# mindspore-lab/minddiffusion

Measured on AMD Instinct MI355X. Metric: 512x512 txt2img latents/sec (50-step DDIM), higher is better.
Workload: dtype f16; 1 GPU; SDv2 txt2img 512x512 (64x64 latent), 50-step DDIM, CFG 9.0, batch 1 per GPU (BASELINE.json configs[1]); synthetic seeded weights + synthetic text conditioning; global_batch=1, parallelism=batch-shard x1, hip_graph=True, rccl_world_size=1, broadcast_bytes=0, ddim_steps=50, unet_batch_per_gpu=2, sampler=ddim, cfg_dup_prefix=False

## Files before the change

### minddiffusion_amd/csrc/dense.hip

```cpp
#include "mdx_common.h"
#include "gemm_internal.h"

#include <algorithm>

namespace {

#ifndef MDX_LEAN_EPI
#define MDX_LEAN_EPI 1
#endif
constexpr bool LEAN_EPI = MDX_LEAN_EPI != 0;
constexpr int LNR_MAX = 24;
typedef unsigned u32x2 __attribute__((ext_vector_type(2)));

template <int BM, class Restage>
__device__ __forceinline__ void xattn_tile_epilogue(const GemmParams& p, char* smem, const char* xs, const int m0, const int n0,
                                                    const Restage& restage) {
    constexpr int SLD = 72;
    const int tid = threadIdx.x, lane = tid & 63;
    const int wave = __builtin_amdgcn_readfirstlane(tid >> 6);
    const int ntile = (p.xa_len + 63) >> 6;
    if (wave * 32 >= BM) {
        for (int t0 = 2; t0 < ntile; t0 += 2) {
            __syncthreads();
            restage(t0);
            asm volatile("s_waitcnt vmcnt(0)" ::: "memory");
            __syncthreads();
        }
        return;
    }
    const int hi = lane >> 5, l31 = lane & 31;
    f16* stg = reinterpret_cast<f16*>(smem);
    f16x8 qf[4];
#pragma unroll
    for (int s4 = 0; s4 < 4; ++s4) qf[s4] = *reinterpret_cast<const f16x8*>(&stg[(wave * 32 + l31) * SLD + 16 * s4 + 8 * hi]);
    f32x16 acc_o[2];
#pragma unroll
    for (int d = 0; d < 2; ++d)
#pragma unroll
        for (int r = 0; r < 16; ++r) acc_o[d][r] = 0.f;
    float m_run = -INFINITY, l_run = 0.f;
    const int vswz = (lane >> 1) & 7;
    const int krow_l = (l31 & 0x13) | ((l31 & 4) << 1) | ((l31 & 8) >> 1);
    auto tile = [&](const int t, auto mask_c) {
        constexpr bool MASK = decltype(mask_c)::value;
        const char* sk = xs + (t & 1) * 16384;
        const char* sv = sk + 8192;
        f32x16 acc_s[2];
#pragma unroll
        for (int kt = 0; kt < 2; ++kt) {
#pragma unroll
            for (int r = 0; r < 16; ++r) acc_s[kt][r] = 0.f;
            const int krow = kt * 32 + krow_l;
#pragma unroll
            for (int s4 = 0; s4 < 4; ++s4) {
                const f16x8 kf = *reinterpret_cast<const f16x8*>(sk + krow * 128 + (((2 * s4 + hi) ^ ((krow >> 1) & 7)) << 4));
                acc_s[kt] = __builtin_amdgcn_mfma_f32_32x32x16_f16(kf, qf[s4], acc_s[kt], 0, 0, 0);
            }
        }
        if constexpr (MASK) {
            const int key0 = t * 64, kmax = p.xa_len - 1;
#pragma unroll
            for (int kt = 0; kt < 2; ++kt)
#pragma unroll
                for (int r = 0; r < 16; ++r) {
                    const int key = key0 + kt * 32 + (r & 3) + 4 * ((r >> 2) & 1) + 8 * hi + 16 * (r >> 3);
                    if (key > kmax) acc_s[kt][r] = -INFINITY;
                }
        }
        float mx = acc_s[0][0];
#pragma unroll
        for (int kt = 0; kt < 2; ++kt)
#pragma unroll
            for (int r = 0; r < 16; ++r) mx = fmaxf(mx, acc_s[kt][r]);
        {
            const auto sw = __builtin_amdgcn_permlane32_swap(__float_as_uint(mx), __float_as_uint(mx), false, false);
            mx = fmaxf(__uint_as_float(sw[0]), __uint_as_float(sw[1]));
        }
        const float m_cand = fmaxf(m_run, mx);
        if (__builtin_amdgcn_ballot_w64((m_cand - m_run) * p.xa_scale_log2 > 8.0f)) {
            const float alpha = __builtin_amdgcn_exp2f((m_run - m_cand) * p.xa_scale_log2);
            l_run *= alpha;
#pragma unroll
            for (int d = 0; d < 2; ++d)
#pragma unroll
                for (int r = 0; r < 16; ++r) acc_o[d][r] *= alpha;
            m_run = m_cand;
        }
        const float mb = m_run * p.xa_scale_log2;
        typedef float f32x2 __attribute__((ext_vector_type(2)));
        const f32x2 sc2 = {p.xa_scale_log2, p.xa_scale_log2}, nmb2 = {-mb, -mb};
        f32x2 psum2 = {0.f, 0.f};
        f16x8 pf[4];
#pragma unroll
        for (int kt = 0; kt < 2; ++kt)
#pragma unroll
            for (int r = 0; r < 16; r += 2) {
                const f32x2 x2 = {acc_s[kt][r], acc_s[kt][r + 1]};
                const f32x2 a2 = __builtin_elementwise_fma(x2, sc2, nmb2);
                const f32x2 pv2 = {__builtin_amdgcn_exp2f(a2.x), __builtin_amdgcn_exp2f(a2.y)};
                psum2 += pv2;
                pf[kt * 2 + (r >> 3)][r & 7] = (f16)pv2.x;
                pf[kt * 2 + (r >> 3)][(r & 7) + 1] = (f16)pv2.y;
            }
        l_run += psum2.x + psum2.y;
#pragma unroll
        for (int c = 0; c < 4; ++c)
#pragma unroll
            for (int d = 0; d < 2; ++d) {
                const f16x8 vf = *reinterpret_cast<const f16x8*>(sv + (d * 32 + l31) * 128 + (((2 * c + hi) ^ vswz) << 4));
                acc_o[d] = __builtin_amdgcn_mfma_f32_32x32x16_f16(vf, pf[c], acc_o[d], 0, 0, 0);
            }
    };
    for (int t = 0; t < ntile; ++t) {
        if (t >= 2 && !(t & 1)) {
            __syncthreads();
            restage(t);
            asm volatile("s_waitcnt vmcnt(0)" ::: "memory");
            __syncthreads();
        }
        if ((t + 1) * 64 > p.xa_len) tile(t, std::true_type{}); else tile(t, std::false_type{});
    }
    const float l_tot = l_run + __shfl_xor(l_run, 32, 64);
    const float inv = 1.0f / l_tot;
    f16* og = stg + wave * 32 * SLD;
#pragma unroll
    for (int d = 0; d < 2; ++d)
#pragma unroll
        for (int g = 0; g < 4; ++g) {
            f16x4 v;
#pragma unroll
            for (int e = 0; e < 4; ++e) v[e] = (f16)(acc_o[d][4 * g + e] * inv);
            *reinterpret_cast<f16x4*>(&og[l31 * SLD + d * 32 + 8 * g + 4 * hi]) = v;
        }
    asm volatile("s_waitcnt lgkmcnt(0)" ::: "memory");
    for (int idx = lane; idx < 32 * 8; idx += 64) {
        const int row = idx >> 3, chunk = idx & 7;
        const int m = m0 + wave * 32 + row;
        if (m < p.M) {
            const f16x8 v = *reinterpret_cast<const f16x8*>(&og[row * SLD + chunk * 8]);
            *reinterpret_cast<f16x8*>(p.out + (size_t)m * p.out_ld + n0 + chunk * 8) = v;
        }
    }
}

template <int BM, int BN>
__device__ __forceinline__ void epilogue_w41(const GemmParams& p, f32x16 (&acc)[BN / 32], char* smem, const int m0, const int n0,
                                             const float bias_pre, const float lns_pre) {
    constexpr int NT = 256, TN = BN / 32, SLD = BN + 8;
    const int tid = threadIdx.x, lane = tid & 63;
    const int wave = __builtin_amdgcn_readfirstlane(tid >> 6);
    const int hi = lane >> 5, l31 = lane & 31;
    f16* stg = reinterpret_cast<f16*>(smem);
    float* lnrow = reinterpret_cast<float*>(smem + (size_t)BM * SLD * 2);
    float* lns = lnrow + 2 * BM;
    float* bs = lns + BN;
    if (tid < BN) bs[tid] = bias_pre;
    const int m_l = wave * 32 + l31;
    if (p.ln_stats) {
        for (int r = tid; r < BM; r += NT) {
            float mr[2];
            gemm_ln_row_fold(p, m0 + r, mr);
            lnrow[2 * r] = mr[0];
            lnrow[2 * r + 1] = mr[1];
        }
        if (tid < BN) lns[tid] = lns_pre;
        __syncthreads();
        const float mean = lnrow[2 * m_l], rstd = lnrow[2 * m_l + 1];
#pragma unroll
        for (int j = 0; j < TN; ++j)
#pragma unroll
            for (int r = 0; r < 16; ++r) {
                const int n_l = j * 32 + 8 * (r >> 2) + 4 * hi + (r & 3);
                acc[j][r] = rstd * (acc[j][r] - mean * lns[n_l]);
            }
    }
    const bool geglu = p.epilogue == MDX_EPI_GEGLU;
    constexpr int CH = BN / 8, PASSES = BM * CH / NT;
    static_assert(BM * CH % NT == 0 && BM * (CH / 2) % NT == 0, "store loops: whole passes");
    const __amdgpu_buffer_rsrc_t rs_res = make_rsrc(p.residual, (p.residual && !geglu) ? p.res_bytes : 0u);
    f16x8 lres[PASSES];
#pragma unroll
    for (int pass = 0; pass < PASSES; ++pass) {
        const int idx = tid + pass * NT;
        const int row = idx / CH, c = idx - row * CH;
        const int m = m0 + row, n = n0 + c * 8;
        const unsigned off = (m < p.M && n < p.N) ? ((unsigned)m * (unsigned)p.residual_ld + (unsigned)n) * 2u : MDX_OOB;
        lres[pass] = __builtin_bit_cast(f16x8, __builtin_amdgcn_raw_buffer_load_b128(rs_res, off, 0, 0));
    }
#pragma unroll
    for (int j = 0; j < TN; ++j)
#pragma unroll
        for (int g = 0; g < 4; ++g) {
            const int n_l = j * 32 + 8 * g + 4 * hi;
            *reinterpret_cast<f16x4*>(&stg[m_l * SLD + n_l]) =
                cvt4(acc[j][4 * g], acc[j][4 * g + 1], acc[j][4 * g + 2], acc[j][4 * g + 3]);
        }
    __syncthreads();
    trace_mark(p, 5);
    if (geglu) {
        constexpr int U = BN / 2, GCH = U / 8, GP = BM * GCH / NT;
        const bool has_res = p.residual != nullptr;
        f16x8 va[GP], vg[GP];
        f32x4 ba[GP][2], bg[GP][2];
#pragma unroll
        for (int pass = 0; pass < GP; ++pass) {
            const int idx = tid + pass * NT;
            const int row = idx / GCH, c = idx - row * GCH;
            va[pass] = *reinterpret_cast<const f16x8*>(&stg[row * SLD + c * 8]);
            vg[pass] = *reinterpret_cast<const f16x8*>(&stg[row * SLD + U + c * 8]);
            ba[pass][0] = *reinterpret_cast<const f32x4*>(&bs[c * 8]);
            ba[pass][1] = *reinterpret_cast<const f32x4*>(&bs[c * 8 + 4]);
            bg[pass][0] = *reinterpret_cast<const f32x4*>(&bs[U + c * 8]);
            bg[pass][1] = *reinterpret_cast<const f32x4*>(&bs[U + c * 8 + 4]);
        }
#pragma unroll
        for (int pass = 0; pass < GP; ++pass) {
            const int idx = tid + pass * NT;
            const int row = idx / GCH, c = idx - row * GCH;
            const int m = m0 + row;
            const int pn = n0 + c * 8;
            const int on = (n0 >> 1) + c * 8;
            if (m < p.M && pn < p.N) {
                float f[8];
#pragma unroll
                for (int e = 0; e < 8; ++e)
                    f[e] = ((float)va[pass][e] + ba[pass][e >> 2][e & 3]) * gelu_tanh_f((float)vg[pass][e] + bg[pass][e >> 2][e & 3]);
                if (has_res) {
                    const f16x8 rr = *reinterpret_cast<const f16x8*>(p.residual + (size_t)m * p.residual_ld + on);
#pragma unroll
                    for (int e = 0; e < 8; ++e) f[e] += (float)rr[e];
                }
                f16x8 o;
#pragma unroll
                for (int e = 0; e < 8; ++e) o[e] = (f16)f[e];
                *reinterpret_cast<f16x8*>(p.out + (size_t)m * p.out_ld + on) = o;
            }
        }
        return;
    }
    const bool has_res = p.residual != nullptr;
    f16x8 sv[PASSES];
    f32x4 bb[PASSES][2];
#pragma unroll
    for (int pass = 0; pass < PASSES; ++pass) {
        const int idx = tid + pass * NT;
        const int row = idx / CH, c = idx - row * CH;
        sv[pass] = *reinterpret_cast<const f16x8*>(&stg[row * SLD + c * 8]);
        bb[pass][0] = *reinterpret_cast<const f32x4*>(&bs[c * 8]);
        bb[pass][1] = *reinterpret_cast<const f32x4*>(&bs[c * 8 + 4]);
    }
#pragma unroll
    for (int pass = 0; pass < PASSES; ++pass) {
        const int idx = tid + pass * NT;
        const int row = idx / CH, c = idx - row * CH;
        const int m = m0 + row, n = n0 + c * 8;
        float f[8];
#pragma unroll
        for (int e = 0; e < 8; ++e) f[e] = (float)sv[pass][e] + bb[pass][e >> 2][e & 3];
        if (has_res) {
#pragma unroll
            for (int e = 0; e < 8; ++e) f[e] += (float)lres[pass][e];
        }
        f16x8 o;
#pragma unroll
        for (int e = 0; e < 8; ++e) o[e] = (f16)f[e];
        if (m < p.M && n < p.N) *reinterpret_cast<f16x8*>(p.out + (size_t)m * p.out_ld + n) = o;
    }
}

template <int BM, int BN, int NS, int PF, bool XA = false>
__global__ __launch_bounds__(256, 2) void dense_kernel(const GemmParams p) {
    mdx_kernarg_touch<sizeof(GemmParams)>();
    constexpr int NW = 4;
    constexpr bool W41 = BN % 64 != 0;
    static_assert(!W41 || (BM == 128 && BN % 32 == 0 && !XA && PF <= 1), "4 x 1 wave layout: 128-row tiles, prefetch level 0 / 1");
    constexpr int WROWS = W41 ? BM / 4 : BM / 2;
    constexpr int TM = WROWS / 32;
    constexpr int TN = W41 ? BN / 32 : BN / 64;
    constexpr int ROWB = 128;
    constexpr int KS = 4;
    constexpr int A_BYTES = BM * ROWB;
    constexpr int B_BYTES = BN * ROWB;
    constexpr int STAGE = A_BYTES + B_BYTES;
    constexpr int AJ = BM / 8 / NW;
    constexpr int BJ = BN / 8 / NW;
    constexpr int LPT = AJ + BJ;
    extern __shared__ __attribute__((aligned(16))) char smem[];

    const int tid = threadIdx.x;
    const int lane = tid & 63;
    const int wave = __builtin_amdgcn_readfirstlane(tid >> 6);
    const int wm = W41 ? wave : wave >> 1, wn = W41 ? 0 : wave & 1;
    const int hi = lane >> 5;
    const int l31 = lane & 31;

    const int ntiles = p.tiles_m * p.tiles_n;
    const int tile_id = p.spread ? (int)blockIdx.x : (int)((blockIdx.x & 7) * p.tiles_per_xcd + (blockIdx.x >> 3));
    if (tile_id >= ntiles) return;
    trace_mark(p, 0);
    int tile_m, tile_n;
    if (p.n_fastest) {
        tile_m = p.inv_tiles_n ? (int)__umulhi((unsigned)tile_id, p.inv_tiles_n) : tile_id;
        tile_n = tile_id - tile_m * p.tiles_n;
    } else {
        tile_n = p.inv_tiles_m ? (int)__umulhi((unsigned)tile_id, p.inv_tiles_m) : tile_id;
        tile_m = tile_id - tile_n * p.tiles_m;
    }
    const int m0 = tile_m * BM, n0 = tile_n * BN;
    const int split = (int)blockIdx.y;
    const int kt_begin = split * p.ktiles_per_split;
    const int kt_end = min(p.ktiles, kt_begin + p.ktiles_per_split);
    const int nt = kt_end - kt_begin;

    const __amdgpu_buffer_rsrc_t rs_a = make_rsrc(p.a, p.a_bytes);
    const __amdgpu_buffer_rsrc_t rs_w = make_rsrc(p.w, p.w_bytes);

    const int lrow = lane >> 3, lchk = lane & 7;
    const unsigned row_bytes = (unsigned)p.c1 * 2u;
    unsigned a_voff[AJ], b_off[BJ];
#pragma unroll
    for (int j = 0; j < AJ; ++j) {
        const int row = (wave * AJ + j) * 8 + lrow;
        const int m = m0 + row;
        a_voff[j] = m < p.M ? (unsigned)m * row_bytes + (unsigned)((lchk ^ ((row >> 1) & 7)) * 16) : MDX_OOB;
    }
#pragma unroll
    for (int j = 0; j < BJ; ++j) {
        const int row = (wave * BJ + j) * 8 + lrow;
        if constexpr (W41) {
            const int grow = n0 + row;
            b_off[j] = (unsigned)(grow >> 6) * (unsigned)p.kt64 * 8192u + (unsigned)(((grow & 63) * 8 + lchk) * 16);
        } else {
            const int panel = (n0 >> 6) + (row >> 6);
            b_off[j] = (unsigned)panel * (unsigned)p.kt64 * 8192u + (unsigned)(((row & 63) * 8 + lchk) * 16);
        }
    }
    auto stage_tile = [&](int kt, int buf) {
        char* sbase = smem + buf * STAGE;
#pragma unroll
        for (int j = 0; j < AJ; ++j) dma16s(rs_a, sbase + (wave * AJ + j) * 1024, a_voff[j], (unsigned)kt * 128u);
#pragma unroll
        for (int j = 0; j < BJ; ++j) dma16s(rs_w, sbase + A_BYTES + (wave * BJ + j) * 1024, b_off[j], (unsigned)kt * 8192u);
    };
#pragma unroll
    for (int i = 0; i < NS - 1; ++i)
        if (i < nt) stage_tile(kt_begin + i, i);
    __builtin_amdgcn_sched_barrier(0);
    trace_mark(p, 1);

    constexpr int CPR = BN / 8, RPP = 256 / CPR, PASSES = BM / RPP;
    constexpr int NX = (PF >= 2 && !W41) ? (PASSES < 4 ? PASSES : 4) : 0;
    constexpr int LNR = PF >= 3 ? LNR_MAX : 0;
    constexpr int NT = PF == 1 || PF == 2 ? 2 : 0;
    constexpr int NB = BN == 128 ? 4 : 2;
    constexpr int E = NB + NX + LNR + (PF >= 2 ? 1 : 0) + NT;
    const bool geglu = p.epilogue == MDX_EPI_GEGLU;
    const __amdgpu_buffer_rsrc_t rs_bias = make_rsrc(p.bias, p.bias ? (unsigned)p.N * 4u : 0u);
    const __amdgpu_buffer_rsrc_t rs_res = make_rsrc(p.residual, (p.residual && !geglu) ? p.res_bytes : 0u);
    const bool ln_regs = PF >= 3 && p.ln_stats != nullptr && p.ln_nt <= LNR;
    const bool lns_regs = PF >= 2 && p.ln_stats != nullptr;
    const __amdgpu_buffer_rsrc_t rs_ln = make_rsrc(p.ln_stats, p.ln_stats ? (unsigned)p.M * (unsigned)p.ln_nt * 8u : 0u);
    const __amdgpu_buffer_rsrc_t rs_lns = make_rsrc(p.ln_s, p.ln_stats ? (unsigned)p.N * 4u : 0u);
    u32x4 braw[4] = {};
    if constexpr (W41) {
        const unsigned off = (tid < BN && n0 + tid < p.N) ? (unsigned)(n0 + tid) * 4u : MDX_OOB;
        braw[0][0] = __builtin_amdgcn_raw_buffer_load_b32(rs_bias, off, 0, 0);
        braw[1][0] = __builtin_amdgcn_raw_buffer_load_b32(rs_lns, off, 0, 0);
    } else {
        const int n = n0 + (geglu ? (tid & 7) : (tid % CPR)) * 8;
        const unsigned off = n < p.N ? (unsigned)n * 4u : MDX_OOB;
        braw[0] = __builtin_amdgcn_raw_buffer_load_b128(rs_bias, off, 0, 0);
        braw[1] = __builtin_amdgcn_raw_buffer_load_b128(rs_bias, off, 16, 0);
        if constexpr (NB == 4) {
            const unsigned goff = geglu ? off : MDX_OOB;
            braw[2] = __builtin_amdgcn_raw_buffer_load_b128(rs_bias, goff, 256, 0);
            braw[3] = __builtin_amdgcn_raw_buffer_load_b128(rs_bias, goff, 272, 0);
        }
    }
    u32x4 xraw[NX > 0 ? NX : 1];
    if constexpr (NX > 0) {
        const int n = n0 + (tid % CPR) * 8;
#pragma unroll
        for (int q = 0; q < NX; ++q) {
            const int m = m0 + tid / CPR + q * RPP;
            const unsigned off = (m < p.M && n < p.N) ? ((unsigned)m * (unsigned)p.residual_ld + (unsigned)n) * 2u : MDX_OOB;
            xraw[q] = __builtin_amdgcn_raw_buffer_load_b128(rs_res, off, 0, 0);
        }
    }
    u32x2 lnraw[LNR > 0 ? LNR : 1];
    if constexpr (LNR > 0) {
        const unsigned base = (tid < BM && m0 + tid < p.M) ? (unsigned)(m0 + tid) * (unsigned)p.ln_nt * 8u : MDX_OOB;
#pragma unroll
        for (int j = 0; j < LNR; ++j)
            lnraw[j] = __builtin_amdgcn_raw_buffer_load_b64(rs_ln, (base != MDX_OOB && j < p.ln_nt) ? base : MDX_OOB, j * 8, 0);
    }
    unsigned lns_raw = 0u;
    if constexpr (PF >= 2)
        lns_raw = __builtin_amdgcn_raw_buffer_load_b32(rs_lns, (tid < BN && n0 + tid < p.N) ? (unsigned)(n0 + tid) * 4u : MDX_OOB, 0, 0);
    unsigned touch[2] = {0u, 0u};
    if constexpr (NT > 0) {
        const int rows = min(BM, p.M - m0);
        const unsigned bytes = (unsigned)rows * (unsigned)p.ln_nt * 8u;
        const unsigned base = (unsigned)m0 * (unsigned)p.ln_nt * 8u;
        touch[0] = __builtin_amdgcn_raw_buffer_load_b32(rs_ln, (unsigned)tid * 128u < bytes ? base + (unsigned)tid * 128u : MDX_OOB, 0, 0);
        touch[1] = __builtin_amdgcn_raw_buffer_load_b32(rs_lns, (PF < 2 && tid < BN / 32 && n0 + tid * 32 < p.N) ? (unsigned)(n0 + tid * 32) * 4u : MDX_OOB, 0, 0);
    }
    __builtin_amdgcn_sched_barrier(0);

    f32x16 acc[TM][TN];
#pragma unroll
    for (int i = 0; i < TM; ++i)
#pragma unroll
        for (int j = 0; j < TN; ++j)
#pragma unroll
            for (int r = 0; r < 16; ++r) acc[i][j][r] = 0.f;

    const int swz = (l31 >> 1) & 7;
    const int a_row_off = (wm * WROWS + l31) * ROWB;
    const int b_row_off = A_BYTES + (wn * (BN / 2) + l31) * ROWB;

    int rd = 0, wr = NS - 1;
    for (int t = 0; t < nt; ++t) {
        const int ahead = min(NS - 2, nt - 1 - t);
        if (t == 0) {
            if (NS >= 6 && ahead >= 4)
                asm volatile("s_waitcnt vmcnt(%0)" ::"n"(4 * LPT + E) : "memory");
            else if (NS >= 5 && ahead == 3)
                asm volatile("s_waitcnt vmcnt(%0)" ::"n"(3 * LPT + E) : "memory");
            else if (NS >= 4 && ahead == 2)
                asm volatile("s_waitcnt vmcnt(%0)" ::"n"(2 * LPT + E) : "memory");
            else if (NS >= 3 && ahead == 1)
                asm volatile("s_waitcnt vmcnt(%0)" ::"n"(LPT + E) : "memory");
            else
                asm volatile("s_waitcnt vmcnt(%0)" ::"n"(E) : "memory");
        } else if (NS >= 6 && ahead >= 4)
            asm volatile("s_waitcnt vmcnt(%0)" ::"n"(4 * LPT) : "memory");
        else if (NS >= 5 && ahead == 3)
            asm volatile("s_waitcnt vmcnt(%0)" ::"n"(3 * LPT) : "memory");
        else if (NS >= 4 && ahead == 2)
            asm volatile("s_waitcnt vmcnt(%0)" ::"n"(2 * LPT) : "memory");
        else if (NS >= 3 && ahead == 1)
            asm volatile("s_waitcnt vmcnt(%0)" ::"n"(LPT) : "memory");
        else
            asm volatile("s_waitcnt vmcnt(0)" ::: "memory");
        __builtin_amdgcn_s_barrier();
        if (t == 0) trace_mark(p, 2);
        const char* sb = smem + rd * STAGE;
        constexpr bool ALLK = TM * TN <= 2;
        constexpr int FD = ALLK ? KS : 2;
        f16x8 af[FD][TM], bf[FD][TN];
        auto rdfrag = [&](auto slot_c, const int ks) {
            constexpr int slot = decltype(slot_c)::value;
            const int coff = (((2 * ks + hi) ^ swz) << 4);
#pragma unroll
            for (int i = 0; i < TM; ++i) af[slot][i] = *reinterpret_cast<const f16x8*>(sb + a_row_off + i * 32 * ROWB + coff);
#pragma unroll
            for (int j = 0; j < TN; ++j) bf[slot][j] = *reinterpret_cast<const f16x8*>(sb + b_row_off + j * 32 * ROWB + coff);
        };
        auto mfmas = [&](auto slot_c) {
            constexpr int slot = decltype(slot_c)::value;
#pragma unroll
            for (int i = 0; i < TM; ++i)
#pragma unroll
                for (int j = 0; j < TN; ++j)
                    acc[i][j] = __builtin_amdgcn_mfma_f32_32x32x16_f16(bf[slot][j], af[slot][i], acc[i][j], 0, 0, 0);
        };
        using I0 = std::integral_constant<int, 0>;
        using I1 = std::integral_constant<int, 1>;
        if (t + NS - 1 < nt) stage_tile(kt_begin + t + NS - 1, wr);
        __builtin_amdgcn_sched_barrier(0);
        if constexpr (ALLK) {
            using I2 = std::integral_constant<int, 2>;
            using I3 = std::integral_constant<int, 3>;
            rdfrag(I0{}, 0); rdfrag(I1{}, 1); rdfrag(I2{}, 2); rdfrag(I3{}, 3);
            __builtin_amdgcn_sched_barrier(0);
            mfmas(I0{}); mfmas(I1{}); mfmas(I2{}); mfmas(I3{});
        } else {
            rdfrag(I0{}, 0);
            __builtin_amdgcn_sched_barrier(0);
#pragma unroll
            for (int ks = 0; ks < KS; ks += 2) {
                rdfrag(I1{}, ks + 1);
                __builtin_amdgcn_sched_barrier(0);
                mfmas(I0{});
                __builtin_amdgcn_sched_barrier(0);
                if (ks + 2 < KS) {
                    rdfrag(I0{}, ks + 2);
                    __builtin_amdgcn_sched_barrier(0);
                }
                mfmas(I1{});
                __builtin_amdgcn_sched_barrier(0);
            }
        }
        rd = (rd + 1 == NS) ? 0 : rd + 1;
        wr = (wr + 1 == NS) ? 0 : wr + 1;
    }

    __syncthreads();
    trace_mark(p, 3);
#pragma unroll
    for (int q = 0; q < NB; ++q) asm volatile("" ::"v"(braw[q]));
#pragma unroll
    for (int q = 0; q < NX; ++q) asm volatile("" ::"v"(xraw[q]));
#pragma unroll
    for (int j = 0; j < LNR; ++j) asm volatile("" ::"v"(lnraw[j]));
    if constexpr (PF >= 2) asm volatile("" ::"v"(lns_raw));
#pragma unroll
    for (int q = 0; q < NT; ++q) asm volatile("" ::"v"(touch[q]));
    float bpre[16];
#pragma unroll
    for (int q = 0; q < 4; ++q) {
        const f32x4 f = __builtin_bit_cast(f32x4, braw[q]);
        bpre[4 * q] = f[0]; bpre[4 * q + 1] = f[1]; bpre[4 * q + 2] = f[2]; bpre[4 * q + 3] = f[3];
    }
    Row8Extras xpre[NX > 0 ? NX : 1];
#pragma unroll
    for (int q = 0; q < NX; ++q) xpre[q].res = __builtin_bit_cast(f16x8, xraw[q]);
    float ln_pre[2];
    {
        float su = 0.f, sq = 0.f;
#pragma unroll
        for (int j = 0; j < LNR; ++j) {
            const float2 v = __builtin_bit_cast(float2, lnraw[j]);
            su += v.x;
            sq += v.y;
        }
        const float inv = 1.0f / (float)p.K;
        const float mean = su * inv;
        float var = sq * inv - mean * mean;
        var = var < 0.f ? 0.f : var;
        ln_pre[0] = mean;
        ln_pre[1] = rsqrtf(var + p.ln_eps);
    }
    const float lns_pre = __builtin_bit_cast(float, lns_raw);
    if constexpr (XA) {
        static_assert(BN == 64, "cross-attention epilogue: one 64-wide head per tile");
        constexpr int XOFF = ((BM * 72 * 2 + 2 * BM * 4 + BN * 4 + 1023) / 1024) * 1024;
        char* xs = smem + XOFF;
        const int bsamp = m0 / p.HoWo, head = n0 >> 6;
        const f16* kb = p.xa_k + (size_t)bsamp * p.xa_cap * p.N + head * 64;
        const f16* vb = p.xa_vt + ((size_t)bsamp * p.N + head * 64) * p.xa_cap;
        const __amdgpu_buffer_rsrc_t rs_k = make_rsrc(kb, (unsigned)(((size_t)(p.xa_len - 1) * p.N + 64) * 2));
        const __amdgpu_buffer_rsrc_t rs_v = make_rsrc(vb, (unsigned)((size_t)64 * p.xa_cap * 2));
        const int ntile = (p.xa_len + 63) >> 6;
        auto stage_pair = [&](const int t0) {
            const int t1 = t0 + 2 < ntile ? t0 + 2 : ntile;
            for (int t = t0; t < t1; ++t) {
                char* slot = xs + (t & 1) * 16384;
#pragma unroll
                for (int j = 0; j < 2; ++j) {
                    const int inst = wave * 2 + j;
                    const int krow = inst * 8 + (lane >> 3);
                    const int kchunk = (lane & 7) ^ ((krow >> 1) & 7);
                    const int key = t * 64 + krow;
                    dma16(rs_k, slot + inst * 1024, key < p.xa_len ? (unsigned)(((size_t)key * p.N + kchunk * 8) * 2) : MDX_OOB);
                    const int vrow = inst * 8 + (lane >> 3);
                    const unsigned vchunk = (unsigned)((lane & 7) ^ ((vrow >> 1) & 7));
                    const int kc = t * 64 + (int)vchunk * 8;
                    dma16(rs_v, slot + 8192 + inst * 1024, kc < p.xa_cap ? (unsigned)(((size_t)vrow * p.xa_cap + kc) * 2) : MDX_OOB);
                }
            }
        };
        stage_pair(0);
        gemm_epilogue<BM, BN, true, NW, LinearRows, NX, 3>(p, acc, smem, LinearRows{m0}, n0, split, bpre, tile_m, tile_id, ln_pre, &lns_pre, xpre,
                                                           ln_regs, lns_regs);
        asm volatile("s_waitcnt vmcnt(0)" ::: "memory");
        __syncthreads();
        xattn_tile_epilogue<BM>(p, smem, xs, m0, n0, stage_pair);
    } else if constexpr (W41) {
        epilogue_w41<BM, BN>(p, acc[0], smem, m0, n0, bpre[0], bpre[4]);
    } else {
        gemm_epilogue<BM, BN, true, NW, LinearRows, NX, LEAN_EPI ? 1 : 0>(p, acc, smem, LinearRows{m0}, n0, split, bpre, tile_m, tile_id, ln_pre,
                                                                  &lns_pre, xpre, ln_regs, lns_regs);
    }
    trace_mark(p, 4);
}

template <int BM, int BN, int NS, int PF>
void launch_dense_one(const GemmParams& p, dim3 grid, hipStream_t st) {
    constexpr size_t ring = (size_t)NS * (BM + BN) * 64 * 2;
    constexpr size_t epi = (size_t)(BM > BN ? BM : BN) * ((BM > BN ? BN : BM) + 8) * 2 + 4096;
    constexpr size_t lds = ring > epi ? ring : epi;
    static MdxPerDeviceOnce attr_once;
    if (attr_once.first())
        (void)hipFuncSetAttribute(reinterpret_cast<const void*>(&dense_kernel<BM, BN, NS, PF>),
                                  hipFuncAttributeMaxDynamicSharedMemorySize, (int)lds);
    hipLaunchKernelGGL((dense_kernel<BM, BN, NS, PF>), grid, dim3(256), lds, st, p);
}

template <int BM, int NS>
void launch_dense_xa(const GemmParams& p, dim3 grid, hipStream_t st) {
    constexpr size_t ring = (size_t)NS * (BM + 64) * 64 * 2;
    constexpr size_t xa = (size_t)((BM * 72 * 2 + 2 * BM * 4 + 64 * 4 + 1023) / 1024) * 1024 + 2 * 16384;
    constexpr size_t lds = ring > xa ? ring : xa;
    static MdxPerDeviceOnce attr_once;
    if (attr_once.first())
        (void)hipFuncSetAttribute(reinterpret_cast<const void*>(&dense_kernel<BM, 64, NS, 1, true>),
                                  hipFuncAttributeMaxDynamicSharedMemorySize, (int)lds);
    hipLaunchKernelGGL((dense_kernel<BM, 64, NS, 1, true>), grid, dim3(256), lds, st, p);
}

template <int BM, int BN, int NS>
void launch_dense_pf(const GemmParams& p, int pf, dim3 grid, hipStream_t st) {
    if constexpr (BM * BN < 128 * 128) {
        if (pf >= 3) return launch_dense_one<BM, BN, NS, 3>(p, grid, st);
        if (pf == 2) return launch_dense_one<BM, BN, NS, 2>(p, grid, st);
    }
    if (pf >= 1) return launch_dense_one<BM, BN, NS, 1>(p, grid, st);
    launch_dense_one<BM, BN, NS, 0>(p, grid, st);
}

template <int BM, int BN>
bool launch_dense_ns(const GemmParams& p, int ns, int pf, dim3 grid, hipStream_t st) {
    switch (ns) {
        case 2: launch_dense_pf<BM, BN, 2>(p, pf, grid, st); return true;
        case 3: launch_dense_pf<BM, BN, 3>(p, pf, grid, st); return true;
        case 4: if constexpr (BM == 64 || BN == 64) { launch_dense_pf<BM, BN, 4>(p, pf, grid, st); return true; } return false;
        case 5: if constexpr (BM == 64) { launch_dense_pf<BM, BN, 5>(p, pf, grid, st); return true; } return false;
        case 6: if constexpr (BM == 64) { launch_dense_pf<BM, BN, 6>(p, pf, grid, st); return true; } return false;
        default: return false;
    }
}

}

bool mdx_dense_takes_desc(const GemmParams& p, int bn) {
    if (!mdx_opt(MDX_OPT_GEMM_LEAN_DENSE) || !p.dense_issue) return false;
    if (!(p.ksize == 1 && p.stride == 1 && !p.upsample && p.c2 == 0 && p.cin % 64 == 0 && p.out_mode == MDX_OUT_ROWMAJOR)) return false;
    if (p.gn_cs || p.rowbias || p.out_bs || p.skip_w || p.d2s_c) return false;
    if (p.epilogue != MDX_EPI_NONE && p.epilogue != MDX_EPI_GEGLU) return false;
    if (p.xa_k && bn != 64) return false;
    if (bn == 160) {
        if (p.stats_out || p.colstats_out || p.n_split || p.xa_k) return false;
        if (p.epilogue == MDX_EPI_GEGLU && p.geglu_unit != 80) return false;
    }
    return true;
}

bool mdx_dense_takes(const GemmParams& p, int bm, int bn, int ring, int nsplit, bool fixup, bool nw8) {
    if (!mdx_dense_takes_desc(p, bn)) return false;
    if (!(nsplit == 1 || (fixup && bn != 160)) || nw8) return false;
    int built = (bm == 64 && (bn == 64 || bn == 128)) ? 6 : (bm == 128 && bn == 64) ? 4 : (bm == 128 && (bn == 128 || bn == 160)) ? 3 : 0;
    if (p.xa_k) built = std::min(built, 4);
    if (ring < 2 || ring > built) return false;
    if ((size_t)p.M * (size_t)(p.residual ? p.residual_ld : 0) * 2 >= 0x80000000ull) return false;
    if (p.ln_stats && (size_t)p.M * (size_t)p.ln_nt * 8 >= 0x80000000ull) return false;
    return (long)((p.M + bm - 1) / bm) * ((p.N + bn - 1) / bn) < 65536;
}

int mdx_dense_launch(const GemmParams& p, const GemmPlan& pl, hipStream_t st) {
    const int bm = pl.bm, bn = pl.bn, ns = pl.ring;
    const dim3 g = p.spread ? dim3((unsigned)(p.tiles_m * p.tiles_n), (unsigned)p.nsplit) : pl.grid;
    const int opt = mdx_opt(MDX_OPT_GEMM_LEAN_DENSE);
    const bool small = (long)g.x * g.y <= 512;
    const int pf = opt == 2 ? 0 : (opt == 3 && small ? 2 : (opt == 4 && small ? 3 : 1));
    bool ok = false;
    if (pl.form == GEMM_LEAN_XA) {
        ok = bn == 64 && ns >= 2 && ns <= 4 && (bm == 64 || bm == 128);
        if (ok && bm == 64) { if (ns == 2) launch_dense_xa<64, 2>(p, g, st); else if (ns == 3) launch_dense_xa<64, 3>(p, g, st); else launch_dense_xa<64, 4>(p, g, st); }
        if (ok && bm == 128) { if (ns == 2) launch_dense_xa<128, 2>(p, g, st); else if (ns == 3) launch_dense_xa<128, 3>(p, g, st); else launch_dense_xa<128, 4>(p, g, st); }
    }
    else if (bm == 64 && bn == 64) ok = launch_dense_ns<64, 64>(p, ns, pf, g, st);
    else if (bm == 64 && bn == 128) ok = launch_dense_ns<64, 128>(p, ns, pf, g, st);
    else if (bm == 128 && bn == 64) ok = launch_dense_ns<128, 64>(p, ns, pf, g, st);
    else if (bm == 128 && bn == 128) ok = launch_dense_ns<128, 128>(p, ns, pf, g, st);
    else if (bm == 128 && bn == 160) ok = launch_dense_ns<128, 160>(p, ns, pf, g, st);
    MDX_REQUIRE(ok, "mdx_gemm_f16: internal error: the plan names a lean dense tile %d x %d at ring depth %d that is not built", bm, bn, ns);
    return MDX_OK;
}
```

### minddiffusion_amd/csrc/gemm_tuned.inc

```
    {160, 320, 1024, 1, 64, 0, 8},
    {512, 1280, 2560, 1, 64, 0, 3},
    {512, 1280, 5120, 1, 128, 0, 6},
    {512, 1280, 5760, 3, 128, 0, 10},
    {2048, 640, 2560, 1, 128, 0, 3},
    {2048, 640, 2880, 3, 128, 0, 5},
    {2048, 640, 17280, 3, 128, 0, 6},
    {8192, 320, 72, 3, 64, 0, 1},
    {8192, 320, 320, 1, 64, 0, 1},
    {8192, 320, 640, 1, 64, 0, 1},
    {1024, 1280, 2560, 1, 128, 0, 3},
    {1024, 1280, 11520, 3, 128, 0, 6},
    {16384, 640, 320, 1, 64, 0, 1},
    {16384, 640, 960, 1, 64, 0, 1},
    {16384, 640, 1280, 1, 64, 0, 1},
    {16384, 640, 1920, 1, 64, 0, 1},
    {16384, 640, 2560, 1, 64, 0, 1},
    {640, 320, 1024, 1, 64, 0, 4},
    {1152, 1280, 5120, 1, 128, 0, 5},
    {1152, 3840, 1280, 1, 64, 0, 1},
    {4608, 1280, 1280, 1, 64, 0, 1},
    {4608, 3840, 1280, 1, 64, 0, 1},
    {18432, 640, 640, 1, 64, 0, 1},
    {73728, 8, 2880, 3, 128, 0, 2},
    {128, 1280, 1280, 1, 64, 64, 4},
// ... 56 lines not shown
    {16384, 640, 8640, 3, 128, 128, 1},
    {16384, 640, 11520, 3, 128, 128, 1},
    {65536, 960, 320, 1, 64, 128, 1},
    {640, 640, 1024, 1, 64, 64, 1},
    {640, 1280, 1024, 1, 64, 64, 1},
    {4608, 1280, 5760, 3, 64, 128, 1},
    {4608, 1280, 11520, 3, 64, 128, 1},
    {18432, 640, 320, 1, 64, 128, 1},
    {18432, 640, 960, 1, 64, 128, 1},
    {18432, 640, 2560, 1, 64, 128, 1},
    {18432, 640, 11520, 3, 128, 128, 1},
    {73728, 320, 72, 3, 64, 128, 1},
    {73728, 320, 8640, 3, 128, 128, 1},
    {128, 1280, 11520, 3, 128, 64, 20},
    {128, 1280, 23040, 3, 128, 64, 20},
    {160, 1280, 1024, 1, 64, 64, 1, 65},
    {8192, 320, 960, 1, 64, 64, 1, 2},
    {640, 320, 1024, 1, 64, 64, 1, 65},
    {18432, 640, 8640, 3, 128, 128, 2, 641},
    {18432, 640, 11520, 3, 128, 128, 2, 641},
    {1024, 768, 512, 1, 64, 64, 1, 1},
    {1024, 768, 512, 1, 64, 64, 1, 65},
    {1024, 768, 576, 1, 64, 64, 1, 1},
    {2048, 384, 512, 1, 64, 64, 1, 1},
    {2048, 384, 512, 1, 64, 64, 1, 65},
    {8192, 384, 384, 1, 64, 64, 1, 1},
    {8192, 384, 384, 1, 64, 64, 1, 65},
    {8192, 384, 384, 1, 64, 64, 1, 257},
    {8192, 384, 768, 1, 64, 64, 1, 2},
    {128, 1280, 11520, 3, 128, 64, 14, 257, 3},
    {512, 1280, 1920, 1, 64, 64, 3, 2, 3},
    {2048, 640, 320, 1, 64, 64, 1, 1, 3},
    {2048, 640, 640, 1, 64, 64, 1, 17, 3},
    {2048, 640, 640, 1, 64, 64, 1, 33, 3},
    {2048, 640, 640, 1, 64, 64, 1, 257, 3},
    {2048, 640, 640, 1, 64, 64, 1, 289, 3},
    {2048, 640, 640, 1, 64, 64, 1, 385, 3},
    {2048, 640, 960, 1, 64, 64, 1, 2, 3},
    {2048, 640, 1280, 1, 64, 64, 1, 2, 3},
    {2048, 640, 1920, 1, 64, 64, 1, 2, 3},
    {2048, 640, 2560, 1, 128, 64, 2, 257, 3},
    {2048, 640, 8640, 3, 128, 64, 3, 641, 3},
    {2048, 1920, 640, 1, 64, 128, 1, 25, 3},
    {8192, 8, 2880, 3, 128, 64, 5, 1, 3},
    {8192, 320, 320, 1, 64, 64, 1, 385, 3},
    {8192, 320, 1280, 1, 64, 128, 1, 257, 3},
    {8192, 320, 2880, 3, 128, 64, 1, 641, 3},
    {8192, 320, 8640, 3, 128, 64, 3, 641, 3},
    {1024, 1280, 1280, 1, 64, 64, 1, 33, 3},
    {1024, 1280, 1280, 1, 64, 64, 1, 257, 3},
    {1024, 1280, 1280, 1, 64, 64, 1, 289, 3},
    {1024, 1280, 2560, 1, 64, 128, 2, 2, 3},
    {1024, 1280, 11520, 3, 128, 64, 3, 257, 3},
    {1024, 1280, 11520, 3, 128, 64, 3, 513, 3},
    {16384, 640, 2880, 3, 128, 64, 1, 641, 3},
    {16384, 640, 5760, 3, 128, 64, 1, 385, 3},
    {16384, 640, 5760, 3, 128, 64, 1, 641, 3},
    {16384, 640, 8640, 3, 128, 64, 1, 641, 3},
    {16384, 640, 11520, 3, 128, 64, 1, 641, 3},
    {16384, 640, 17280, 3, 128, 64, 1, 641, 3},
    {16384, 1920, 640, 1, 64, 128, 1, 25, 2},
    {65536, 8, 2880, 3, 128, 64, 1, 1, 3},
    {65536, 320, 1280, 1, 128, 64, 1, 257, 2},
    {65536, 320, 2880, 3, 128, 64, 1, 641, 3},
    {1152, 1280, 1280, 1, 64, 64, 1, 257, 3},
    {1152, 1280, 2560, 1, 64, 128, 2, 2, 3},
    {4608, 1280, 17280, 3, 128, 128, 4, 513, 2},
    {18432, 640, 1920, 1, 64, 128, 1, 2, 2},
    {18432, 640, 5760, 3, 128, 64, 1, 385, 3},
    {18432, 640, 5760, 3, 128, 64, 1, 641, 3},
    {73728, 320, 2880, 3, 128, 64, 1, 257, 3},
    {73728, 320, 2880, 3, 128, 64, 1, 513, 3},
    {73728, 320, 5760, 3, 128, 64, 1, 513, 3},
    {512, 768, 1536, 1, 64, 64, 3, 2, 3},
    {512, 768, 6912, 3, 128, 64, 8, 1, 3},
    {512, 768, 6912, 3, 128, 64, 8, 257, 3},
    {512, 768, 13824, 3, 128, 64, 10, 1, 3},
    {1024, 768, 1536, 1, 64, 64, 3, 2, 3},
    {1024, 768, 5184, 3, 128, 64, 6, 1, 3},
    {1024, 768, 6912, 3, 128, 64, 5, 1, 3},
    {1024, 768, 6912, 3, 128, 64, 5, 257, 3},
    {1024, 768, 12096, 3, 128, 64, 6, 1, 3},
    {2048, 576, 512, 1, 64, 64, 1, 1, 3},
    {2048, 576, 512, 1, 64, 64, 1, 65, 3},
    {2048, 768, 384, 1, 64, 64, 1, 1, 3},
    {2048, 768, 512, 1, 64, 64, 1, 65, 3},
    {2048, 768, 768, 1, 64, 64, 1, 1, 3},
    {2048, 768, 768, 1, 64, 64, 1, 65, 3},
    {2048, 768, 768, 1, 64, 64, 1, 257, 3},
    {2048, 768, 3456, 3, 128, 64, 2, 1, 3},
    {2048, 768, 6912, 3, 128, 64, 2, 257, 3},
    {4096, 384, 3456, 3, 128, 64, 2, 257, 3},
    {4096, 576, 576, 1, 64, 64, 1, 257, 3},
    {4096, 576, 576, 1, 64, 64, 1, 385, 3},
    {4096, 576, 960, 1, 128, 64, 1, 2, 3},
    {4096, 576, 1152, 1, 128, 64, 1, 2, 3},
    {4096, 576, 1344, 1, 128, 64, 1, 2, 3},
    {8192, 384, 384, 1, 64, 64, 1, 385, 3},
    {8192, 384, 3456, 3, 128, 64, 1, 257, 3},
    {8192, 384, 6912, 3, 128, 64, 1, 1, 3},
    {16384, 384, 1728, 3, 128, 64, 1, 1, 3},
    {16384, 384, 3456, 3, 128, 64, 1, 1, 3},
    {16384, 384, 5184, 3, 128, 64, 1, 1, 3},
    {16384, 384, 8640, 3, 128, 64, 1, 1, 3},
    {16384, 576, 5184, 3, 128, 64, 1, 385, 3},
    {32768, 192, 1728, 3, 128, 64, 1, 385, 3},
    {32768, 384, 3456, 3, 128, 64, 1, 129, 3},
    {32768, 384, 3456, 3, 128, 64, 1, 385, 3},
    {32768, 384, 5184, 3, 128, 64, 1, 129, 3},
    {32768, 384, 6912, 3, 128, 64, 1, 129, 3},
    {65536, 8, 1728, 3, 128, 64, 1, 1, 3},
    {65536, 192, 1728, 3, 128, 64, 1, 129, 3},
    {65536, 192, 1728, 3, 128, 64, 1, 385, 3},
    {65536, 192, 3456, 3, 128, 64, 1, 129, 3},
    {65536, 192, 5184, 3, 128, 64, 1, 129, 3},
    {131072, 192, 1728, 3, 128, 64, 1, 257, 3},
    {131072, 192, 3456, 3, 128, 64, 1, 1, 3},
    {131072, 192, 5184, 3, 128, 64, 1, 1, 3},
    {524288, 192, 1728, 3, 128, 64, 1, 1, 3},
    {524288, 192, 1728, 3, 128, 64, 1, 257, 3},
    {524288, 192, 3456, 3, 128, 64, 1, 1, 3},
    {128, 1280, 11520, 3, 128, 64, 14, 513, 3},
    {512, 1280, 2560, 1, 64, 64, 3, 2, 3},
    {8192, 960, 320, 1, 128, 128, 1, 25, 2},
    {1024, 1280, 1280, 1, 64, 64, 1, 17, 3},
    {4096, 1280, 640, 1, 64, 128, 1, 1, 2},
    {4096, 1280, 1920, 1, 64, 128, 1, 2, 2},
    {4096, 1280, 2560, 1, 64, 128, 1, 2, 2},
    {16384, 640, 320, 1, 64, 128, 1, 1, 2},
    {16384, 640, 640, 1, 64, 128, 1, 289, 2},
    {65536, 320, 320, 1, 128, 64, 1, 17, 2},
    {65536, 320, 320, 1, 64, 64, 1, 33, 2},
    {65536, 320, 320, 1, 128, 64, 1, 289, 2},
    {65536, 320, 320, 1, 128, 64, 1, 385, 2},
    {65536, 320, 2880, 3, 128, 64, 1, 385, 3},
    {65536, 320, 5760, 3, 128, 64, 1, 641, 3},
    {65536, 960, 320, 1, 64, 128, 1, 25, 2},
    {1152, 3840, 1280, 1, 64, 128, 1, 25, 2},
    {4608, 1280, 1280, 1, 64, 128, 1, 33, 2},
    {4608, 1280, 1280, 1, 64, 128, 1, 385, 2},
    {4608, 1280, 2560, 1, 128, 128, 1, 2, 2},
    {4608, 1280, 5760, 3, 64, 128, 1, 513, 2},
    {4608, 1280, 11520, 3, 64, 128, 1, 257, 2},
    {4608, 1280, 11520, 3, 64, 128, 1, 513, 2},
    {18432, 640, 320, 1, 64, 128, 1, 1, 2},
    {18432, 640, 960, 1, 64, 128, 1, 2, 2},
    {18432, 640, 1280, 1, 64, 128, 1, 2, 2},
    {73728, 320, 320, 1, 128, 64, 1, 17, 2},
    {73728, 320, 320, 1, 128, 64, 1, 257, 2},
    {73728, 320, 320, 1, 128, 64, 1, 289, 2},
    {73728, 320, 640, 1, 128, 64, 1, 2, 2},
    {73728, 320, 1280, 1, 128, 64, 1, 257, 2},
    {73728, 960, 320, 1, 128, 64, 1, 25, 2},
    {1024, 768, 1344, 1, 64, 64, 3, 2, 3},
    {16384, 384, 192, 1, 64, 128, 1, 1, 2},
    {16384, 384, 384, 1, 64, 128, 1, 1, 2},
    {16384, 384, 384, 1, 128, 64, 1, 65, 2},
    {16384, 384, 384, 1, 64, 128, 1, 257, 2},
    {16384, 384, 384, 1, 128, 64, 1, 385, 2},
    {16384, 384, 576, 1, 64, 128, 1, 2, 2},
    {16384, 384, 768, 1, 64, 128, 1, 2, 2},
    {16384, 384, 960, 1, 64, 128, 1, 2, 2},
    {32768, 384, 576, 1, 64, 128, 1, 2, 2},
    {32768, 384, 1728, 3, 128, 64, 1, 129, 3},
    {65536, 192, 384, 1, 128, 64, 1, 2, 2},
    {131072, 192, 384, 1, 128, 64, 1, 2, 2},
    {524288, 192, 384, 1, 128, 64, 1, 2, 2},
    {128, 1280, 23040, 3, 128, 64, 10, 513, 3},
    {512, 1280, 11520, 3, 256, 64, 6, 513, 3},
    {512, 1280, 17280, 3, 256, 64, 6, 513, 3},
    {512, 1280, 23040, 3, 256, 64, 6, 513, 3},
    {8192, 320, 640, 1, 128, 128, 1, 2, 11},
    {4096, 1280, 5760, 3, 256, 128, 1, 513, 3},
    {4096, 1280, 11520, 3, 256, 128, 3, 257, 3},
    {4096, 1280, 11520, 3, 256, 128, 1, 513, 3},
    {4096, 1280, 17280, 3, 256, 128, 3, 513, 3},
    {4096, 1280, 23040, 3, 256, 128, 3, 513, 3},
    {16384, 640, 640, 1, 64, 128, 1, 17, 2},
    {65536, 320, 72, 3, 128, 128, 1, 129, 10},
    {65536, 320, 640, 1, 128, 128, 1, 2, 10},
    {65536, 320, 960, 1, 128, 128, 1, 2, 10},
    {65536, 320, 8640, 3, 256, 128, 1, 641, 2},
    {18432, 640, 640, 1, 128, 64, 1, 257, 2},
    {18432, 640, 640, 1, 128, 64, 1, 385, 2},
    {73728, 320, 72, 3, 128, 128, 1, 1, 10},
    {73728, 320, 320, 1, 64, 64, 1, 33, 2},
    {2048, 768, 512, 1, 64, 64, 1, 1, 3},
    {2048, 768, 1152, 1, 128, 64, 1, 2, 11},
    {2048, 768, 13824, 3, 256, 128, 5, 1, 3},
    {2048, 2048, 512, 1, 128, 128, 1, 5, 11},
    {4096, 384, 3456, 3, 128, 64, 2, 1, 3},
    {8192, 384, 1152, 1, 128, 128, 1, 2, 11},
    {8192, 768, 6912, 3, 256, 128, 1, 385, 3},
    {16384, 384, 6912, 3, 256, 128, 1, 1, 3},
    {32768, 384, 192, 1, 128, 128, 1, 1, 10},
    {32768, 384, 768, 1, 128, 128, 1, 2, 10},
    {65536, 192, 72, 3, 128, 128, 1, 129, 10},
    {65536, 192, 576, 1, 128, 64, 1, 2, 11},
    {65536, 384, 3456, 3, 256, 128, 1, 385, 3},
    {1024, 1280, 5120, 1, 128, 128, 3, 257, 11},
    {1024, 1280, 11520, 3, 128, 64, 3, 1, 3},
    {1280, 640, 768, 1, 64, 64, 1, 1, 4},
    {1280, 1280, 768, 1, 64, 64, 1, 1, 3},
    {4096, 1280, 1280, 1, 64, 128, 1, 33, 2},
    {4096, 10240, 1280, 1, 128, 128, 1, 19, 10},
    {16384, 640, 640, 1, 64, 128, 1, 33, 2},
    {640, 1280, 1024, 1, 64, 64, 1, 65, 4},
    {1152, 1280, 1280, 1, 64, 64, 1, 33, 3},
    {1152, 1280, 1280, 1, 64, 64, 1, 289, 3},
    {512, 1280, 11520, 3, 256, 64, 6, 1, 3},
    {512, 1280, 11520, 3, 256, 64, 5, 257, 3},
    {2048, 5120, 640, 1, 64, 128, 1, 19, 2},
    {160, 1280, 1024, 1, 64, 64, 3, 1, 4},
    {512, 1280, 1280, 1, 64, 64, 1, 257, 4},
    {512, 1280, 1280, 1, 64, 64, 1, 289, 4},
    {512, 10240, 1280, 1, 64, 128, 1, 19, 2},
    {1024, 3840, 1280, 1, 128, 128, 1, 25, 11},
    {1024, 10240, 1280, 1, 64, 128, 1, 19, 2},
    {1280, 1280, 768, 1, 64, 64, 1, 65, 3},
    {16384, 640, 2560, 1, 64, 128, 1, 257, 2},
    {640, 320, 1024, 1, 64, 64, 3, 1, 4},
    {640, 640, 1024, 1, 64, 64, 2, 1, 4},
    {1152, 1280, 1280, 1, 64, 64, 1, 17, 3},
    {1152, 1280, 11520, 3, 128, 128, 5, 257, 2},
    {4608, 1280, 1280, 1, 128, 128, 1, 289, 10},
    {4608, 1280, 5120, 1, 128, 128, 1, 257, 10},
    {18432, 640, 640, 1, 64, 128, 1, 289, 2},
    {18432, 640, 2560, 1, 128, 128, 1, 257, 10},
    {512, 768, 768, 1, 64, 64, 3, 1, 4},
    {512, 768, 768, 1, 64, 64, 1, 65, 3},
    {1024, 768, 768, 1, 64, 64, 1, 1, 3},
    {1024, 768, 768, 1, 64, 64, 1, 65, 3},
    {1024, 768, 13824, 3, 128, 128, 5, 1, 3},
    {1024, 2048, 512, 1, 128, 64, 1, 5, 11},
    {2048, 384, 3456, 3, 128, 64, 3, 1, 3},
    {2048, 384, 3456, 3, 128, 64, 5, 257, 3},
    {2048, 512, 512, 1, 64, 64, 1, 257, 4},
    {2048, 512, 2048, 1, 64, 64, 1, 257, 6},
    {4096, 576, 576, 1, 128, 64, 1, 1, 11},
    {4096, 576, 8640, 3, 256, 128, 3, 1, 3},
    {524288, 192, 72, 3, 128, 128, 1, 1, 10},
    {1024, 1280, 23040, 3, 128, 128, 3, 513, 4},
    {4096, 1280, 1280, 1, 128, 128, 1, 17, 2},
    {4096, 1280, 1280, 1, 128, 128, 1, 257, 2},
    {4096, 1280, 1280, 1, 128, 128, 1, 289, 2},
    {4096, 1280, 5120, 1, 128, 128, 3, 257, 2},
    {16384, 640, 640, 1, 128, 64, 1, 257, 2},
    {16384, 640, 640, 1, 64, 128, 1, 385, 2},
    {640, 1280, 1024, 1, 64, 64, 1, 1, 3},
    {4608, 1280, 640, 1, 128, 128, 1, 1, 2},
    {4608, 1280, 1280, 1, 128, 128, 1, 17, 2},
    {4608, 1280, 1280, 1, 128, 128, 1, 257, 2},
    {4608, 3840, 1280, 1, 128, 128, 1, 25, 2},
    {18432, 640, 640, 1, 128, 128, 1, 17, 2},
    {18432, 640, 640, 1, 128, 128, 1, 33, 2},
    {18432, 640, 2880, 3, 128, 128, 1, 641, 2},
    {18432, 1920, 640, 1, 128, 128, 1, 25, 2},
    {73728, 8, 2880, 3, 128, 64, 1, 1, 4},
    {512, 2304, 768, 1, 64, 64, 1, 9, 3},
    {1024, 512, 2048, 1, 64, 64, 2, 257, 6},
    {1024, 576, 5184, 3, 128, 64, 6, 1, 3},
    {1024, 576, 5184, 3, 128, 64, 6, 257, 3},
    {1024, 2304, 768, 1, 64, 64, 1, 9, 3},
    {2048, 768, 6912, 3, 128, 64, 2, 1, 4},
    {2048, 768, 10368, 3, 128, 64, 2, 1, 4},
    {2048, 2304, 768, 1, 64, 128, 1, 9, 2},
    {4096, 576, 3456, 3, 128, 64, 1, 1, 4},
    {4096, 576, 5184, 3, 128, 64, 1, 1, 4},
    {4096, 576, 5184, 3, 128, 64, 1, 257, 4},
    {4096, 576, 10368, 3, 256, 128, 3, 1, 3},
    {4096, 576, 12096, 3, 256, 128, 3, 1, 3},
    {4096, 768, 6912, 3, 128, 64, 1, 385, 4},
    {4096, 1728, 576, 1, 128, 128, 1, 9, 10},
    {8192, 384, 3456, 3, 128, 64, 1, 1, 4},
    {8192, 384, 10368, 3, 256, 128, 2, 1, 3},
    {8192, 1152, 384, 1, 64, 128, 1, 9, 2},
    {16384, 192, 1728, 3, 128, 64, 1, 1, 4},
    {16384, 192, 1728, 3, 128, 64, 1, 385, 4},
    {16384, 384, 3456, 3, 256, 128, 1, 257, 3},
    {16384, 1152, 384, 1, 64, 128, 1, 9, 2},
    {131072, 384, 3456, 3, 256, 128, 1, 385, 3},
    {524288, 8, 1728, 3, 128, 64, 1, 1, 4},
    {128, 1280, 1280, 1, 64, 64, 3, 257, 5},
    {128, 1280, 5120, 1, 64, 64, 4, 257, 5},
    {128, 1280, 11520, 3, 128, 64, 16, 1, 4},
    {128, 3840, 1280, 1, 64, 64, 2, 25, 5},
    {160, 320, 1024, 1, 64, 64, 3, 1, 5},
    {160, 640, 1024, 1, 64, 64, 3, 1, 4},
    {160, 640, 1024, 1, 64, 64, 1, 65, 4},
    {512, 1280, 1280, 1, 64, 64, 1, 17, 4},
    {512, 1280, 1280, 1, 64, 64, 1, 33, 5},
    {512, 1280, 5120, 1, 128, 64, 3, 257, 4},
    {512, 1280, 5760, 3, 128, 64, 4, 513, 4},
    {512, 3840, 1280, 1, 64, 128, 1, 25, 4},
    {2048, 640, 2880, 3, 128, 64, 3, 641, 4},
    {2048, 640, 5760, 3, 128, 64, 3, 129, 4},
    {2048, 640, 5760, 3, 128, 64, 3, 385, 4},
    {2048, 640, 5760, 3, 128, 64, 3, 641, 4},
    {2048, 640, 11520, 3, 128, 64, 3, 641, 4},
    {2048, 640, 17280, 3, 128, 64, 3, 641, 4},
    {8192, 320, 2880, 3, 128, 64, 1, 129, 4},
    {8192, 320, 2880, 3, 128, 64, 1, 385, 4},
    {8192, 320, 5760, 3, 128, 64, 1, 641, 4},
```

### minddiffusion_amd/ldm/modules/diffusionmodules/openaimodel.py

```python
import ctypes
import math
import os
import re
import weakref

import torch

from .... import ops
from ...._lib import MdxError
from ....planner import PlanBuilder, round_up, capture_or_eager
from ....loader import WeightLoader, named_layers

f16, f32 = torch.float16, torch.float32

LORA_PREFIXES = ("tk_delta_", "mindpet_delta_")
_LORA_KEY = re.compile(r"^(.*)\.(" + "|".join(LORA_PREFIXES) + r")lora_([ab])$")
_LORA_TARGETS = ("to_q", "to_k", "to_v", "to_out.0")


def is_lora_key(name):
    return _LORA_KEY.match(name) is not None


class UNetModel:
# ... 6 lines not shown
                 max_context_len=80, device="cuda:0"):
        if use_spatial_transformer:
            assert context_dim is not None, "context_dim is required with use_spatial_transformer"
        if context_dim is not None:
            assert use_spatial_transformer, "context_dim requires use_spatial_transformer"
        if num_heads == -1:
            assert num_head_channels != -1, "Either num_heads or num_head_channels has to be set"
        if num_head_channels == -1:
            assert num_heads != -1, "Either num_heads or num_head_channels has to be set"
        if not use_spatial_transformer:
            raise NotImplementedError("AttentionBlock is an empty stub in the reference (openaimodel.py:208-242)")
        if dims != 2:
            raise NotImplementedError("dims != 2: the image UNet is the only instantiation on the denoising path")
        self.conv_resample = bool(conv_resample)
        self.num_classes = num_classes
        self.use_scale_shift_norm = bool(use_scale_shift_norm)
        self.resblock_updown = bool(resblock_updown)
        self.transformer_depth = int(transformer_depth)
        self.n_embed = n_embed
        assert self.transformer_depth >= 1
        self.image_size = image_size
        self.in_channels = in_channels
        self.model_channels = model_channels
        self.out_channels = out_channels
        self.num_res_blocks = num_res_blocks
        self.attention_resolutions = list(attention_resolutions)
        self.channel_mult = list(channel_mult)
        self.num_heads = num_heads
        self.num_head_channels = num_head_channels
        self.context_dim = int(context_dim)
        self.legacy = legacy
        self.use_linear = use_linear_in_transformer
        self.use_fp16 = use_fp16
        self.device = torch.device(device)
        self.time_embed_dim = model_channels * 4
        self.input_blocks, self.middle_block, self.output_blocks = self._structure()
        self.cin_pad = round_up(in_channels, 8)
        self.final_channels = out_channels if n_embed is None else int(n_embed)
        self.cout_pad = round_up(self.final_channels, 8)
        self.w = None
        self._plans = {}
        self._ctx_key = None
        self._ctx_ref = None
        self.use_graph = True
        self.max_context_len = self._check_context_cap(max_context_len)
        self.last_launch_count = 0
        self.enable_lora = bool(enable_lora)
        self.lora_rank = int(lora_rank)
        self.lora_alpha = float(lora_alpha)
        if self.enable_lora and not (1 <= self.lora_rank <= 64 and self.lora_alpha != 0):
            raise ValueError(f"UNetModel: lora_rank must be in [1, 64] and lora_alpha non-zero (got {lora_rank}, {lora_alpha})")
        self._lora_base = {}
        self._lora_sites = {}
        self._lora = None
        self._lora_mult = 1.0

    @staticmethod
    def _check_context_cap(n):
        n = int(n)
        if not 1 <= n <= 1024:
            raise MdxError(f"UNetModel: max_context_len must be in [1, 1024] (got {n})")
        return round_up(n, 8)

    def set_max_context_len(self, n):
        n = self._check_context_cap(n)
        if n != self.max_context_len:
            self.max_context_len = n
            self._plans = {}
            self._ctx_key = None
            self._ctx_ref = None
        return self

    def _heads(self, ch, num_heads):
        if self.num_head_channels == -1:
            dim_head = ch // num_heads
        else:
            num_heads = ch // self.num_head_channels
            dim_head = self.num_head_channels
        if self.legacy:
            dim_head = ch // num_heads
        return num_heads, dim_head

    def _structure(self):
        mc = self.model_channels
        nh = self.num_heads
        inb = [[("conv", self.in_channels, mc)]]
        chans = [mc]
        ch, ds = mc, 1
        for level, mult in enumerate(self.channel_mult):
            for _ in range(self.num_res_blocks):
                layers = [("res", ch, mult * mc)]
                ch = mult * mc
                if ds in self.attention_resolutions:
                    nh, dh = self._heads(ch, nh)
                    layers.append(("st", ch, nh, dh))
                inb.append(layers)
                chans.append(ch)
            if level != len(self.channel_mult) - 1:
                inb.append([("resdown", ch, ch) if self.resblock_updown else ("down", ch)])
                chans.append(ch)
                ds *= 2
        nh, dh = self._heads(ch, nh)
        mid = [("res", ch, ch), ("st", ch, nh, dh), ("res", ch, ch)]
        outb = []
        for level, mult in list(enumerate(self.channel_mult))[::-1]:
            for i in range(self.num_res_blocks + 1):
                ich = chans.pop()
                layers = [("res", ch + ich, mc * mult)]
                ch = mc * mult
                if ds in self.attention_resolutions:
                    nh, dh = self._heads(ch, nh)
                    layers.append(("st", ch, nh, dh))
                if level and i == self.num_res_blocks:
                    layers.append(("resup", ch, ch) if self.resblock_updown else ("up", ch))
                    ds //= 2
                outb.append(layers)
        return inb, mid, outb

    def parameter_shapes(self):
        mc, ted, ctx = self.model_channels, self.time_embed_dim, self.context_dim
        s = {"time_embed.0.weight": (ted, mc), "time_embed.0.bias": (ted,),
             "time_embed.2.weight": (ted, ted), "time_embed.2.bias": (ted,)}
        if self.num_classes is not None:
            s["label_emb.embedding_table"] = (self.num_classes, ted)
        ssn = 2 if self.use_scale_shift_norm else 1
        for pre, layer in named_layers(self):
            kind = layer[0]
            if kind == "conv":
                s[pre + "conv.weight"] = (layer[2], layer[1], 3, 3)
                s[pre + "conv.bias"] = (layer[2],)
            elif kind in ("res", "resdown", "resup"):
                cin, cout = layer[1], layer[2]
                s[pre + "in_layers_norm.gamma"] = (cin,)
                s[pre + "in_layers_norm.beta"] = (cin,)
                s[pre + "in_layers_conv.conv.weight"] = (cout, cin, 3, 3)
                s[pre + "in_layers_conv.conv.bias"] = (cout,)
                s[pre + "emb_layers.1.weight"] = (ssn * cout, ted)
                s[pre + "emb_layers.1.bias"] = (ssn * cout,)
                s[pre + "out_layers_norm.gamma"] = (cout,)
                s[pre + "out_layers_norm.beta"] = (cout,)
                s[pre + "out_layers_conv.conv.weight"] = (cout, cout, 3, 3)
                s[pre + "out_layers_conv.conv.bias"] = (cout,)
                if cin != cout:
                    s[pre + "skip_connection.conv.weight"] = (cout, cin, 1, 1)
                    s[pre + "skip_connection.conv.bias"] = (cout,)
            elif kind == "st":
                ch, inner = layer[1], layer[2] * layer[3]
                s[pre + "norm.gamma"] = (ch,)
                s[pre + "norm.beta"] = (ch,)
                s[pre + "proj_in.weight"] = (inner, ch) if self.use_linear else (inner, ch, 1, 1)
                s[pre + "proj_in.bias"] = (inner,)
                s[pre + "proj_out.weight"] = (ch, inner) if self.use_linear else (ch, inner, 1, 1)
                s[pre + "proj_out.bias"] = (ch,)
                for k in range(self.transformer_depth):
                    t = pre + f"transformer_blocks.{k}."
                    for a, cd in (("attn1.", inner), ("attn2.", ctx)):
                        s[t + a + "to_q.weight"] = (inner, inner)
                        s[t + a + "to_k.weight"] = (inner, cd)
                        s[t + a + "to_v.weight"] = (inner, cd)
                        s[t + a + "to_out.0.weight"] = (inner, inner)
                        s[t + a + "to_out.0.bias"] = (inner,)
                    s[t + "ff.net.0.proj.weight"] = (inner * 8, inner)
                    s[t + "ff.net.0.proj.bias"] = (inner * 8,)
                    s[t + "ff.net.2.weight"] = (inner, inner * 4)
                    s[t + "ff.net.2.bias"] = (inner,)
                    for n in ("norm1", "norm2", "norm3"):
                        s[t + n + ".gamma"] = (inner,)
                        s[t + n + ".beta"] = (inner,)
            elif kind == "down" and self.conv_resample:
                s[pre + "op.conv.weight"] = (layer[1], layer[1], 3, 3)
                s[pre + "op.conv.bias"] = (layer[1],)
            elif kind == "up" and self.conv_resample:
                s[pre + "conv.conv.weight"] = (layer[1], layer[1], 3, 3)
                s[pre + "conv.conv.bias"] = (layer[1],)
        s["out.0.gamma"] = (mc,)
        s["out.0.beta"] = (mc,)
        s["out.2.conv.weight"] = (self.out_channels, mc, 3, 3)
        s["out.2.conv.bias"] = (self.out_channels,)
        if self.n_embed is not None:
            s["id_predictor.0.gamma"] = (mc,)
            s["id_predictor.0.beta"] = (mc,)
            s["id_predictor.1.conv.weight"] = (self.n_embed, mc, 1, 1)
            s["id_predictor.1.conv.bias"] = (self.n_embed,)
        return s

    def _lora_targets(self):
        for pre, layer in named_layers(self):
            if layer[0] != "st":
                continue
            inner = layer[2] * layer[3]
            for k in range(self.transformer_depth):
                t = pre + f"transformer_blocks.{k}."
                for a, cd in (("attn1.", inner), ("attn2.", self.context_dim)):
                    for n in _LORA_TARGETS:
                        yield t + a + n, inner, (inner if n in ("to_q", "to_out.0") else cd)

    def lora_parameter_shapes(self, prefix=LORA_PREFIXES[0]):
        if prefix not in LORA_PREFIXES:
            raise ValueError(f"lora_parameter_shapes: prefix must be one of {LORA_PREFIXES}")
        s = {}
        for name, nout, nin in self._lora_targets():
            s[f"{name}.{prefix}lora_a"] = (self.lora_rank, nin)
            s[f"{name}.{prefix}lora_b"] = (nout, self.lora_rank)
        return s

    def load_state_dict(self, params, strict=True):
        shapes = self.parameter_shapes()
        who = "UNetModel.load_state_dict"
        lora_params = {}
        if self.enable_lora:
            lora_params = {k: v for k, v in params.items() if is_lora_key(k)}
            params = {k: v for k, v in params.items() if k not in lora_params}
        L = WeightLoader(params, self.device, who)
        L.check(shapes, unexpected=strict)
        if lora_params:
            lora_params = self._check_lora(lora_params, strict, who)
        ln_fold = os.environ.get("MDX_UNET_LN_FOLD", "1") != "0"
        qkv_merge = os.environ.get("MDX_UNET_QKV_MERGE", "1") != "0"
        w = L.w
        w["te0.w"], w["te0.b"] = L.raw("time_embed.0.weight", f16), L.vec("time_embed.0.bias")
        w["te2.w"], w["te2.b"] = L.raw("time_embed.2.weight", f16), L.vec("time_embed.2.bias")
        if self.num_classes is not None:
            w["label_emb"] = L.raw("label_emb.embedding_table", f32)
        emb_w, emb_b, self._emb_off = [], [], {}
        off = 0
        for pre, layer in named_layers(self):
            kind = layer[0]
            if kind == "conv":
                w[pre + "w"], w[pre + "b"] = L.conv(pre + "conv.weight", cin_pad=self.cin_pad), L.vec(pre + "conv.bias")
            elif kind in ("res", "resdown", "resup"):
                cin, cout = layer[1], layer[2]
                for n in ("in_layers_norm", "out_layers_norm"):
                    L.norm(pre + n, pre + n)
                w[pre + "conv1.w"], w[pre + "conv1.b"] = L.conv(pre + "in_layers_conv.conv.weight"), L.vec(pre + "in_layers_conv.conv.bias")
                w[pre + "conv2.w"], w[pre + "conv2.b"] = L.conv(pre + "out_layers_conv.conv.weight"), L.vec(pre + "out_layers_conv.conv.bias")
                if cin != cout:
                    w[pre + "skip.w"], w[pre + "skip.b"] = L.conv(pre + "skip_connection.conv.weight"), L.vec(pre + "skip_connection.conv.bias")
                emb_w.append(L.raw(pre + "emb_layers.1.weight", f16))
                emb_b.append(L.vec(pre + "emb_layers.1.bias"))
                self._emb_off[pre] = off
                off += cout * (2 if self.use_scale_shift_norm else 1)
            elif kind == "st":
                inner = layer[2] * layer[3]
                L.norm(pre + "norm", pre + "norm")
                proj = {}
                for n in ("proj_in", "proj_out"):
                    wt = L.raw(pre + n + ".weight", f16)
                    proj[n] = wt.reshape(wt.shape[0], wt.shape[1])
                    w[pre + n + ".w"], w[pre + n + ".b"] = L.dense(proj[n]), L.vec(pre + n + ".bias")
                for k in range(self.transformer_depth):
                    t = pre + f"transformer_blocks.{k}."
                    wq, wk, wv = (L.raw(t + f"attn1.to_{n}.weight", f16) for n in "qkv")
                    for n in ("norm1", "norm2", "norm3"):
                        L.norm(t + n, t + n)
                    fold = inner % 64 == 0 and ln_fold

                    def put(name, wt, norm, bias=None):
                        if fold:
                            wt, w[name + ".s"], w[name + ".cb"] = ops.fold_layernorm(wt, w[t + norm + ".g"], w[t + norm + ".b"], bias)
                        w[name + ".w"] = L.dense(wt)
                    if (2 * wq.shape[0]) % 128 == 0 and qkv_merge:
                        put(t + "attn1.qkv", torch.cat([wq, wk, wv], 0), "norm1")
                    else:
                        w[t + "attn1.qk.w"] = L.dense(torch.cat([wq, wk], 0))
                        w[t + "attn1.v.w"] = L.dense(wv)
                    wq2 = L.raw(t + "attn2.to_q.weight", f16)
                    put(t + "attn2.q", wq2, "norm2")
                    w[t + "attn2.k.w"] = L.dense(t + "attn2.to_k.weight")
                    w[t + "attn2.v.w"] = L.dense(t + "attn2.to_v.weight")
                    wo = {a: L.raw(t + a + ".to_out.0.weight", f16) for a in ("attn1", "attn2")}
                    for a in ("attn1", "attn2"):
                        w[t + a + ".o.w"], w[t + a + ".o.b"] = L.dense(wo[a]), L.vec(t + a + ".to_out.0.bias")
                    gw, gb = L.raw(t + "ff.net.0.proj.weight", f16), L.vec(t + "ff.net.0.proj.bias")
                    half = 4 * inner
                    w[t + "ff1.b"] = ops.geglu_interleave(gb[:half], gb[half:], 64)
                    put(t + "ff1", ops.geglu_interleave(gw[:half], gw[half:], 64), "norm3", w[t + "ff1.b"])
                    w2 = L.raw(t + "ff.net.2.weight", f16)
                    w[t + "ff2.w"], w[t + "ff2.b"] = L.dense(w2), L.vec(t + "ff.net.2.bias")
                    if (self.transformer_depth == 1 and inner == layer[1]
                            and ops.st_tail_supported(inner, layer[2], layer[3], 64, 64)):
                        w[t + "tail.stream"], w[t + "tail.vec"] = ops.pack_st_tail(
                            wo["attn1"], wq2, wo["attn2"], gw, w2, proj["proj_out"],
                            w[t + "attn1.o.b"], w[t + "norm2.g"], w[t + "norm2.b"], w[t + "attn2.o.b"], w[t + "norm3.g"],
                            w[t + "norm3.b"], gb, w[t + "ff2.b"], w[pre + "proj_out.b"])
                        if ops.st_head_supported(inner, 64, 64):
                            w[t + "head.stream"], w[t + "head.vec"] = ops.pack_st_head(
                                proj["proj_in"], wq, wk, wv, w[pre + "norm.g"], w[pre + "norm.b"],
                                w[pre + "proj_in.b"], w[t + "norm1.g"], w[t + "norm1.b"])
            elif kind == "down" and self.conv_resample:
                w[pre + "w"], w[pre + "b"] = L.conv(pre + "op.conv.weight"), L.vec(pre + "op.conv.bias")
            elif kind == "up" and self.conv_resample:
                w[pre + "w"], w[pre + "b"] = L.conv(pre + "conv.conv.weight"), L.vec(pre + "conv.conv.bias")
                if layer[1] % 64 == 0 and ops.get_option("unet_subpixel_upsample"):
                    w[pre + "wsub"] = ops.pack_subpixel_conv_weight(L.raw(pre + "conv.conv.weight", f32))
        w["emb.w"] = torch.cat(emb_w, 0).contiguous()
        w["emb.b"] = torch.cat(emb_b, 0).contiguous()
        self._emb_total = off
        norm, conv = ("out.0", "out.2.conv") if self.n_embed is None else ("id_predictor.0", "id_predictor.1.conv")
        w["out.g"], w["out.b"] = L.vec(norm + ".gamma"), L.vec(norm + ".beta")
        w["out.w"] = L.conv(conv + ".weight", cout_pad=self.cout_pad)
        w["out.cb"] = L.vec(conv + ".bias", pad=self.cout_pad)
        self._frag_w = {}
        self._geglu80 = {}
        self._plans = {}
        self._ctx_key = None
        self._ctx_ref = None
        self._lora = None
        self._lora_base, self._lora_sites = {}, {}
        if self.enable_lora:
            for name, _, _ in self._lora_targets():
                self._lora_base[name] = L.own(name + ".weight", f32)
        self.w = L.finish(shapes, unused=() if self.n_embed is None else [k for k in shapes if k.startswith("out.")])
        if self.enable_lora:
            self._lora_sites = self._find_lora_sites()
            if lora_params:
                self._set_lora(lora_params)
        return self

    def weight_bytes(self):
        n = sum(t.numel() * t.element_size() for t in self.w.values())
        n += sum(t.numel() * t.element_size() for t in self._lora_base.values())
        if self._lora:
            n += sum(a.numel() * 4 + b.numel() * 4 for a, b in self._lora.values())
        return n

    def _find_lora_sites(self):
        w = self.w
        T, F = ops.LORA_TILED, ops.LORA_FRAG
        sites = {}
        for pre, layer in named_layers(self):
            if layer[0] != "st":
                continue
            inner = layer[2] * layer[3]
            ks = inner // 16
            for k in range(self.transformer_depth):
                t = pre + f"transformer_blocks.{k}."

                def tiled(key, n0=0, dst_n=inner, norm=None):
                    kw = dict(dst=w[key + ".w"], layout=T, dst_n0=n0, dst_N=dst_n)
                    if norm is not None and (key + ".s") in w:
                        kw.update(gamma=w[t + norm + ".g"], beta=w[t + norm + ".b"], S=w[key + ".s"][n0:], cb=w[key + ".cb"][n0:])
                    return kw

                def frag(key, slot, per_wave):
                    return dict(dst=w[t + key], layout=F, dst_N=inner, piece_stride=per_wave * ks, piece_offset=slot * ks)
                merged = (t + "attn1.qkv.w") in w
                for i, n in enumerate("qkv"):
                    if merged:
                        here = [tiled(t + "attn1.qkv", i * inner, 3 * inner, "norm1")]
                    elif n == "v":
                        here = [tiled(t + "attn1.v")]
                    else:
                        here = [tiled(t + "attn1.qk", i * inner, 2 * inner)]
                    if (t + "head.stream") in w:
                        here.append(frag("head.stream", 1 + i, 4))
                    sites[t + f"attn1.to_{n}"] = here
                sites[t + "attn2.to_q"] = [tiled(t + "attn2.q", norm="norm2")]
                sites[t + "attn2.to_k"] = [tiled(t + "attn2.k")]
                sites[t + "attn2.to_v"] = [tiled(t + "attn2.v")]
                sites[t + "attn1.to_out.0"] = [tiled(t + "attn1.o")]
                sites[t + "attn2.to_out.0"] = [tiled(t + "attn2.o")]
                if (t + "tail.stream") in w:
                    for slot, name in enumerate(("attn1.to_out.0", "attn2.to_q", "attn2.to_out.0")):
                        sites[t + name].append(frag("tail.stream", slot, 16))
        assert set(sites) == set(self._lora_base)
        return sites

    def _check_lora(self, params, strict, who):
        found = {m.group(2) for m in map(_LORA_KEY.match, params) if m}
        if len(found) > 1:
            raise KeyError(f"{who}: adapter keys mix the prefixes {sorted(found)}")
        prefix = found.pop() if found else LORA_PREFIXES[0]
        shapes = self.lora_parameter_shapes(prefix)
        WeightLoader(params, self.device, who).check(shapes, unexpected=strict)
        return {k.replace("." + prefix, "." + LORA_PREFIXES[0]): params[k] for k in shapes}

    def _set_lora(self, checked):
        p, L = LORA_PREFIXES[0], WeightLoader(checked, self.device, "UNetModel.load_lora_state_dict")
        self._lora = {name: (L.own(f"{name}.{p}lora_a", f32), L.own(f"{name}.{p}lora_b", f32)) for name in self._lora_base}
        self._merge_lora()

    def _merge_lora(self):
        scale = self._lora_mult * self.lora_alpha / self.lora_rank
        for name, base in self._lora_base.items():
            a, b = self._lora[name] if self._lora else (None, None)
            for site in self._lora_sites[name]:
                ops.lora_merge(base, A=a, B=b, scale=scale, **site)
        self._ctx_key = None
        self._ctx_ref = None

    def _need_lora(self, who):
        if not self.enable_lora:
            raise MdxError(f"UNetModel.{who}: the model was built without enable_lora=True")
        if self.w is None:
            raise MdxError(f"UNetModel.{who}: load_state_dict() must be called first (the adapter is merged into the base weights)")

    def load_lora_state_dict(self, params, strict=True):
        self._need_lora("load_lora_state_dict")
        self._set_lora(self._check_lora(dict(params), strict, "UNetModel.load_lora_state_dict"))
        return self

    def set_lora_scale(self, m=1.0):
        self._need_lora("set_lora_scale")
        m = float(m)
        if not math.isfinite(m):
            raise ValueError("set_lora_scale: the multiplier must be finite")
        self._lora_mult = m
        if self._lora:
            self._merge_lora()
        return self

    def unload_lora(self):
        self._need_lora("unload_lora")
        if self._lora:
            self._lora = None
            self._merge_lora()
        return self

    @property
    def lora_loaded(self):
        return self._lora is not None

    class _Plan:
        pass

    def _plan(self, B, H, W, _selfctx=False):
        key = (B, H, W, "selfctx") if _selfctx else (B, H, W)
        if key in self._plans:
            return self._plans[key]
        if self.w is None:
            raise MdxError("UNetModel: load_state_dict() must be called before the first forward")
        for lvl in range(len(self.channel_mult) - 1):
            if (H >> lvl) % 2 or (W >> lvl) % 2:
                raise MdxError(f"UNetModel: latent {H}x{W} is not divisible by 2^{len(self.channel_mult) - 1}")
        try:
            P = _UNetPlanner(self, B, H, W, True, _selfctx).build()
        except _HeadNotWired:
            P = _UNetPlanner(self, B, H, W, False, _selfctx).build()
        self._plans[key] = P
        return P

    def _ensure_context(self, P, context):
        key = (context.data_ptr(), context._version, tuple(context.shape), context.dtype, id(P))
        alive = self._ctx_ref() if self._ctx_ref is not None else None
        if key == self._ctx_key and alive is context:
            return
        Bc, T, Dc = context.shape
        if Bc != P.B or Dc != self.context_dim:
            raise MdxError(f"context shape {tuple(context.shape)} does not match batch {P.B} / context_dim {self.context_dim}")
        if T > self.max_context_len:
            raise MdxError(f"context length {T} > max_context_len={self.max_context_len}")
        P.ctx_pad.zero_()
        P.ctx_pad[:, :T].copy_(context)
        P.ctx_len = T
        for d in getattr(P, "xattn_descs", ()):
            d.xattn_len = T
        for op in P.ctxops:
            op()
        self._ctx_key = key
        self._ctx_ref = weakref.ref(context)
        if getattr(P, "graph_ctx_len", None) != T:
            P.graph = None
            P.dup_graph = None

    def time_embedding_table(self, t):
        if self.w is None:
            raise MdxError("UNetModel: load_state_dict() must be called before time_embedding_table()")
        if self.num_classes is not None:
            raise MdxError("UNetModel: a class-conditional UNet adds label_emb(y) before the ResBlock projections; "
                           "there is no timestep-only table")
        t = torch.as_tensor(t, dtype=f32).to(self.device).reshape(-1).contiguous()
        w = self.w
        e0 = ops.timestep_embedding(t, self.model_channels)
        e1 = ops.dense_small(e0, w["te0.w"], w["te0.b"], act_out=True)
        e2 = ops.dense_small(e1, w["te2.w"], w["te2.b"])
        return ops.dense_small(e2, w["emb.w"], w["emb.b"], act_in=True)

    def forward_nhwc(self, x, timesteps, context=None, temb=None, y=None, cfg_dup=False):
        if (y is not None) != (self.num_classes is not None):
            raise MdxError("UNetModel: must specify y if and only if the model is class-conditional")
        if y is not None and temb is not None:
            raise MdxError("UNetModel: time_embedding_table() rows do not carry the label embedding; pass timesteps with y")
        if not (isinstance(x, torch.Tensor) and x.is_cuda):
            raise MdxError("UNetModel: x must be a CUDA(HIP) tensor (no CPU fallback)")
        B, C, H, W = x.shape
        if C != self.in_channels:
            raise MdxError(f"UNetModel: expected {self.in_channels} input channels, got {C}")
        if context is None:
            if getattr(self, "_selfctx_bad", None) is None:
                self._selfctx_bad = sorted({l[2] * l[3] for _, l in named_layers(self)
                                            if l[0] == "st" and l[2] * l[3] != self.context_dim})
            bad = self._selfctx_bad
            if bad:
                raise MdxError(f"UNetModel: context=None makes attn2 attend to its own input (attention.py:133), which needs "
                               f"context_dim == transformer width; context_dim={self.context_dim}, widths {bad}")
            P = self._plan(B, H, W, _selfctx=True)
        else:
            P = self._plan(B, H, W)
            self._ensure_context(P, context)
        P.x_static.copy_(x)
        if temb is not None:
            if temb.shape[-1] != self._emb_total or temb.dtype != f32:
                raise MdxError(f"UNetModel: temb must be fp32 [.., {self._emb_total}] rows of time_embedding_table()")
            P.emb_all.copy_(temb)
        else:
            P.t_static.copy_(timesteps.to(device=self.device, dtype=f32) if isinstance(timesteps, torch.Tensor)
                             else torch.as_tensor(timesteps, dtype=f32, device=self.device))
            if y is not None:
                yy = torch.as_tensor(y).to(device=self.device, dtype=torch.long).reshape(-1)
                if yy.shape[0] != B:
                    raise MdxError(f"UNetModel: y has {yy.shape[0]} labels for a batch of {B}")
                if int(yy.min()) < 0 or int(yy.max()) >= self.num_classes:
                    raise MdxError(f"UNetModel: class label outside [0, {self.num_classes})")
                P.y_static.copy_(yy)
            for op in P.main[:P.temb_ops]:
                op()
        dup = self._dup_body(P) if (cfg_dup and context is not None and y is None) else None
        if dup is not None and ops.get_option("unet_cfg_dup_check"):
            hb = B // 2
            same = torch.equal(P.x_static[:hb], P.x_static[hb:]) and torch.equal(P.emb_all[:hb], P.emb_all[hb:])
            if not same:
                raise MdxError("UNetModel: cfg_dup=True, but the two halves of the batch do not carry the same x / timesteps")
        if self.use_graph and not P.graph_failed:
            if dup is not None:
                if P.dup_graph is None:
                    self._capture(P, dup)
                if P.dup_graph is not None:
                    P.dup_graph.replay()
                    return P.eps_nhwc
            if P.graph is None:
                self._capture(P)
            if P.graph is not None:
                P.graph.replay()
                return P.eps_nhwc
        body = dup if dup is not None else P.main[P.temb_ops:]
        for op in body:
            op()
        self.last_launch_count = P.temb_ops + len(body)
        return P.eps_nhwc

    def _dup_body(self, P):
        mn = ops.get_option("unet_cfg_dup")
        if not mn or P.B < mn or P.B % 2 or P.ck is None:
            return None
        if hasattr(P, "dup_body"):
            return P.dup_body
        P.dup_body = None
        h = P.B // 2
        PA = self._plan(h, P.H, P.W)
        if PA.ck is None:
            return None
        late = "op2" in P.ck and "op2" in PA.ck and len(P.ck["live2"]) == len(PA.ck["live2"])
        ko, kl = ("op2", "live2") if late else ("op", "live")
        ib, ic = P.main.index(P.ck[ko]), P.main.index(P.ck["conv_in"])
        ja, jc = PA.main.index(PA.ck[ko]), PA.main.index(PA.ck["conv_in"])
        xin_a, xin_b = PA.ck["xin"], P.ck["xin"]
        copies = [lambda: xin_a.copy_(xin_b[:h]), lambda: PA.emb_all.copy_(P.emb_all[:h])]
        spread = []
        for src, dst in zip(PA.ck[kl], P.ck[kl]):
            if not (dst.shape[0] == 2 * src.shape[0] and dst.shape[1:] == src.shape[1:] and dst.dtype == src.dtype):
                raise MdxError(f"UNetModel: guidance-duplicate prefix: live tensors of the two plans do not pair up "
                               f"({tuple(src.shape)} vs {tuple(dst.shape)})")
            spread.append(lambda src=src, dst=dst, k=src.shape[0]: (dst[:k].copy_(src), dst[k:].copy_(src)))
        P.dup_half = PA
        P.dup_body = P.main[P.temb_ops:ic + 1] + copies + PA.main[jc:ja + 1] + spread + P.main[ib + 1:]
        small = {"kind": "small", "flops": 0, "launches": 1, "info": "guidance-duplicate prefix: copy"}
        P.dup_meta = (P.meta[P.temb_ops:ic + 1] + [dict(small) for _ in copies] + PA.meta[jc:ja + 1]
                      + [dict(small, launches=2) for _ in spread] + P.meta[ib + 1:])
        return P.dup_body

    def _capture(self, P, dup=None):
        body = dup if dup is not None else P.main[P.temb_ops:]
        graphs = capture_or_eager([body])
        if graphs is None:
            P.graph, P.graph_failed = None, True
        elif dup is not None:
            P.dup_graph = graphs[0]
        else:
            P.graph = graphs[0]
        if graphs is not None:
            P.graph_ctx_len = P.ctx_len

    def construct(self, x, timesteps=None, context=None, y=None):
        eps = self.forward_nhwc(x, timesteps, context, y=y)
        B, _, H, W = x.shape
        return ops.nhwc_to_nchw(eps, self.final_channels, H, W)

    __call__ = construct
    forward = construct


class _HeadNotWired(Exception):
    """A fused SpatialTransformer head / GroupNorm-in-conv launch did not get its column statistics (UNetModel._plan)."""


class _UNetPlanner(PlanBuilder):

    def __init__(self, net, B, H, W, fuse_head, selfctx):
        super().__init__(net.device, B, track_producers=True)
        self.net, self.w, self.H, self.W = net, net.w, H, W
        self.fuse_head, self.selfctx = fuse_head, selfctx
        self.TC = net.max_context_len
        self.ctx_flops = 77 if self.TC == 80 else self.TC
        self.mod_ld = net._emb_total
        self.P = UNetModel._Plan()
        self.ctxops = []
        self.ck = {}
        self.hs = []
        self.ctx_kv = {}
        self.xattn_descs, self.ln_stats, self.tails, self.heads_fused, self.ragged_vt = [], {}, [], [], []

    def build(self):
        P, net, B = self.P, self.net, self.B
        dev = self.dev
        P.B, P.H, P.W = B, self.H, self.W
        P.x_static = torch.zeros((B, net.in_channels, self.H, self.W), dtype=f32, device=dev)
        P.t_static = torch.zeros((B,), dtype=f32, device=dev)
        self.time_embedding()
        xin = self.get((B, self.H * self.W, net.cin_pad))
        self.emit(lambda: ops.nchw_to_nhwc(P.x_static, net.cin_pad, out=xin), "small")
        self.ck["xin"] = xin
        P.ctx_pad = torch.zeros((B, self.TC, net.context_dim), dtype=f16, device=dev)
        P.ctx_len = 0
        self.walk(xin)
        for t, (kc, vtc) in self.ctx_kv.items():
            inner = kc.shape[2]
            self.dense(P.ctx_pad, B, self.TC, net.context_dim, inner, self.w[t + "attn2.k.w"], out=kc, out_ld=inner,
                       oplist=self.ctxops)
            self.dense(P.ctx_pad, B, self.TC, net.context_dim, inner, self.w[t + "attn2.v.w"], out=vtc, out_ld=self.TC,
                       out_mode=ops.OUT_TRANSPOSED, oplist=self.ctxops)
        self.finish(P)
        P.ctxops, P.attn_ws, P.colstats = self.ctxops, self.attn_ws, self.colstats
        P.arena_bytes = self.A.total
        P.ln_stats = self.ln_stats
        P.tails = self.tails
        P.ragged_vt = self.ragged_vt
        P.heads_fused = self.heads_fused
        P.ctx_kv = self.ctx_kv
        P.xattn_descs = self.xattn_descs
        P.ck = self.ck if (self.ck.get("op") is not None and not self.selfctx) else None
        P.graph = None
        P.dup_graph = None
        P.graph_failed = False
        return P

    def time_embedding(self):
        P, net, w, B, dev = self.P, self.net, self.w, self.B, self.dev
        mc, ted = net.model_channels, net.time_embed_dim
        t_emb = torch.empty((B, mc), dtype=f32, device=dev)
        e1 = torch.empty((B, ted), dtype=f32, device=dev)
        emb = torch.empty((B, ted), dtype=f32, device=dev)
        P.emb_all = torch.empty((B, net._emb_total), dtype=f32, device=dev)
        self.emit(lambda: ops.timestep_embedding(P.t_static, mc, out=t_emb), "small")
        self.emit(lambda: ops.dense_small(t_emb, w["te0.w"], w["te0.b"], act_out=True, out=e1), "small", 2 * B * mc * ted)
        self.emit(lambda: ops.dense_small(e1, w["te2.w"], w["te2.b"], out=emb), "small", 2 * B * ted * ted)
        if net.num_classes is not None:
            P.y_static = torch.zeros((B,), dtype=torch.long, device=dev)
            self.emit(lambda: emb.add_(w["label_emb"].index_select(0, P.y_static)), "small")
        self.emit(lambda: ops.dense_small(emb, w["emb.w"], w["emb.b"], act_in=True, out=P.emb_all), "small",
                  2 * B * ted * net._emb_total)
        P.temb_ops = len(self.main)

    def held(self, t):
        return any(t is s_[0] for s_ in self.hs)

    def walk(self, xin):
        net, w, B = self.net, self.w, self.B
        h, wd = self.H, self.W
        cur = None
        for i, blk in enumerate(net.input_blocks):
            for j, layer in enumerate(blk):
                pre = f"input_blocks.{i}.{j}."
                if layer[0] == "conv":
                    cur, h, wd = self.conv3(xin, net.cin_pad, layer[2], w[pre + "w"], w[pre + "b"], h, wd)
                    self.ck["conv_in"] = self.main[-1]
                    self.release(xin)
                    continue
                new, h2, w2 = self.layer_op(pre, layer, cur, None, h, wd)
                if not self.held(cur):
                    self.release(cur)
                cur, h, wd = new, h2, w2
            self.hs.append((cur, h, wd))
        self.ck.setdefault("op", None)
        for j, layer in enumerate(net.middle_block):
            new, h, wd = self.layer_op(f"middle_block.{j}.", layer, cur, None, h, wd)
            if not self.held(cur):
                self.release(cur)
            cur = new
        for i, blk in enumerate(net.output_blocks):
            skip, sh, sw = self.hs.pop()
            assert (sh, sw) == (h, wd)
            for j, layer in enumerate(blk):
                new, h, wd = self.layer_op(f"output_blocks.{i}.{j}.", layer, cur, skip if j == 0 else None, h, wd)
                self.release(cur)
                if j == 0:
                    self.release(skip)
                cur = new
        mc = net.model_channels
        a = self.get((B, h * wd, mc))
        self.gn(cur, None, w["out.g"], w["out.b"], 1e-5, net.n_embed is None, a)
        self.P.eps_nhwc = torch.empty((B, h * wd, net.cout_pad), dtype=f16, device=self.dev)
        self.gemm(a=a, w=w["out.w"], N=net.cout_pad, B=B, H=h, W=wd, c1=mc, out=self.P.eps_nhwc, out_ld=net.cout_pad,
                  bias=w["out.cb"], ksize=3 if net.n_embed is None else 1)

    def layer_op(self, pre, layer, cur, skip, h, wd):
        net, w, B = self.net, self.w, self.B
        kind = layer[0]
        if kind == "res":
            return self.resblock(pre, cur, skip, layer[1], layer[2], h, wd)
        if kind in ("resdown", "resup"):
            return self.resblock(pre, cur, None, layer[1], layer[2], h, wd, mode=kind[3:])
        if kind == "st":
            return self.transformer(pre, cur, layer[1], layer[2], layer[3], h, wd), h, wd
        if kind == "down":
            if net.conv_resample:
                return self.conv3(cur, layer[1], layer[1], w[pre + "w"], w[pre + "b"], h, wd, stride=2)
            new = self.get((B, (h // 2) * (wd // 2), layer[1]))
            self.emit(lambda cur=cur, new=new: ops.avgpool2x2(cur, B, h, wd, layer[1], out=new), "small")
            return new, h // 2, wd // 2
        if kind == "up":
            if net.conv_resample:
                return self.conv3(cur, layer[1], layer[1], w[pre + "w"], w[pre + "b"], h, wd, upsample=1, wsub=w.get(pre + "wsub"))
            new = self.get((B, 4 * h * wd, layer[1]))
            self.emit(lambda cur=cur, new=new: ops.upsample_nearest2x(cur, B, h, wd, layer[1], out=new), "small")
            return new, 2 * h, 2 * wd
        raise ValueError(kind)

    def gn_conv_ok(self, src, c_in, c_out, hh, ww, wt):
        B = self.B
        mrows = ops.get_option("unet_gn_conv_fuse")
        if not self.fuse_head or not mrows or B * hh * ww < mrows or c_in % 64 or c_in > 640 or (hh == 8 and ww == 8):
            return False
        if self.producer.get(src.data_ptr()) is None:
            return False
        probe = ops.make_gemm_desc(a=src, w=wt, N=c_out, B=B, H=hh, W=ww, c1=c_in, out=src, out_ld=c_out, ksize=3)
        q = ops.gemm_query(probe)
        return q[3] == 1 and q[1] == 64

    def conv2(self, pre, src, x, x2, xs, cin, cout, c2, ho, wo, fusable, gn=None):
        w, B = self.w, self.B
        if cin != cout and fusable and self.skip_fusable(src, cin - c2, c2, cout, ho, wo, w[pre + "conv2.w"]):
            if (pre + "conv2skip.b") not in w:
                w[pre + "conv2skip.b"] = (w[pre + "conv2.b"] + w[pre + "skip.b"]).contiguous()
            out, _, _ = self.conv3(src, cout, cout, w[pre + "conv2.w"], w[pre + "conv2skip.b"], ho, wo, gn=gn,
                                   skip=(x, x2, cin - c2, c2, w[pre + "skip.w"]))
            self.release(src)
            return out
        if cin != cout:
            skip = self.dense(x, B, x.shape[1], cin, cout, w[pre + "skip.w"], bias=w[pre + "skip.b"], src2=x2, c2=c2)
        else:
            assert x2 is None
            skip = xs
        out, _, _ = self.conv3(src, cout, cout, w[pre + "conv2.w"], w[pre + "conv2.b"], ho, wo, residual=skip, gn=gn)
        self.release(src)
        if skip is not x:
            self.release(skip)
        return out

    def resblock(self, pre, x, x2, cin, cout, h, wd, mode=None):
        net, w, B, P = self.net, self.w, self.B, self.P
        c2 = 0 if x2 is None else x2.shape[2]
        hw = h * wd
        eoff = net._emb_off[pre]
        film = net.use_scale_shift_norm
        rowbias = None if film else P.emb_all[:, eoff:eoff + cout]
        gn1 = x2 is None and mode is None and self.gn_conv_ok(x, cin, cout, h, wd, w[pre + "conv1.w"])
        a = None
        if not gn1:
            a = self.get((B, hw, cin))
            self.gn(x, x2, w[pre + "in_layers_norm.g"], w[pre + "in_layers_norm.b"], 1e-5, True, a)
        if mode == "up":
            assert x2 is None and cin == cout
            hbuf, ho, wo = self.conv3(a, cin, cout, w[pre + "conv1.w"], w[pre + "conv1.b"], h, wd, upsample=1, rowbias=rowbias)
            xs = self.get((B, ho * wo, cin))
            self.emit(lambda x=x, xs=xs: ops.upsample_nearest2x(x, B, h, wd, cin, out=xs), "small")
        elif mode == "down":
            assert x2 is None and cin == cout
            ap = self.get((B, hw // 4, cin))
            self.emit(lambda a=a, ap=ap: ops.avgpool2x2(a, B, h, wd, cin, out=ap), "small")
            hbuf, ho, wo = self.conv3(ap, cin, cout, w[pre + "conv1.w"], w[pre + "conv1.b"], h // 2, wd // 2, rowbias=rowbias)
            self.release(ap)
            xs = self.get((B, hw // 4, cin))
            self.emit(lambda x=x, xs=xs: ops.avgpool2x2(x, B, h, wd, cin, out=xs), "small")
        elif gn1:
            hbuf, ho, wo = self.conv3(x, cin, cout, w[pre + "conv1.w"], w[pre + "conv1.b"], h, wd, rowbias=rowbias,
                                      gn=(w[pre + "in_layers_norm.g"], w[pre + "in_layers_norm.b"], 1e-5))
            xs = x
        else:
            hbuf, ho, wo = self.conv3(a, cin, cout, w[pre + "conv1.w"], w[pre + "conv1.b"], h, wd, rowbias=rowbias)
            xs = x
        if a is not None:
            self.release(a)
        if (not film and mode is None) and self.gn_conv_ok(hbuf, cout, cout, ho, wo, w[pre + "conv2.w"]):
            gnp = (w[pre + "out_layers_norm.g"], w[pre + "out_layers_norm.b"], 1e-5)
            return self.conv2(pre, hbuf, x, x2, xs, cin, cout, c2, ho, wo, True, gn=gnp), ho, wo
        a2 = self.get((B, ho * wo, cout))
        if film:
            self.gn(hbuf, None, w[pre + "out_layers_norm.g"], w[pre + "out_layers_norm.b"], 1e-5, True, a2,
                    scale=P.emb_all[:, eoff:eoff + cout], shift=P.emb_all[:, eoff + cout:eoff + 2 * cout])
        else:
            self.gn(hbuf, None, w[pre + "out_layers_norm.g"], w[pre + "out_layers_norm.b"], 1e-5, True, a2)
        self.release(hbuf)
        return self.conv2(pre, a2, x, x2, xs, cin, cout, c2, ho, wo, mode is None), ho, wo

    def geglu_tile160(self, d, t, inner):
        w, g80 = self.w, self.net._geglu80
        if (8 * inner) % 160 or inner % 64:
            return
        d.geglu_unit = 80
        ok = ops.gemm_check(d) and ops.gemm_query(d)[1] == 160
        if not ok:
            d.geglu_unit = 0
            return
        for k in ("ff1.w", "ff1.b", "ff1.s", "ff1.cb"):
            if (t + k) in w and (t + k) not in g80:
                src = w[t + k]
                if k == "ff1.w":
                    src = ops.pack_gemm_weight(ops.geglu_repack(ops.unpack_gemm_weight(src, 8 * inner, inner), 64, 80))
                else:
                    src = ops.geglu_repack(src, 64, 80)
                g80[t + k] = src
        d.w = g80[t + "ff1.w"].data_ptr()
        d._w_tensor = g80[t + "ff1.w"]
        if d.ln_stats:
            d.bias, d.ln_s = g80[t + "ff1.cb"].data_ptr(), g80[t + "ff1.s"].data_ptr()
        else:
            d.bias = g80[t + "ff1.b"].data_ptr()

    def tail_rows(self, t, n, heads, dh):
        TC = self.TC
        if (t + "tail.stream") not in self.w or self.net.transformer_depth != 1 or self.selfctx:
            return 0
        if TC > 1024 or TC % 8:
            return 0
        forced = ops.get_option("unet_st_tail")
        cands = [forced] if forced in (32, 64) else ([] if forced == 0 else [64, 32])
        for r in cands:
            if not ops.st_tail_supported(heads * dh, heads, dh, n, r):
                continue
            blocks = self.B * n // r
            if forced in (32, 64) or (r == 64 and blocks >= 512) or (r == 32 and blocks >= 192):
                return r
        return 0

    def head_rows(self, t, x, n, heads, dh):
        if not self.fuse_head or (t + "head.stream") not in self.w or ops.get_option("unet_st_head") == 0:
            return 0
        r = self.tail_rows(t, n, heads, dh)
        if not r or not ops.st_head_supported(heads * dh, n, r) or self.producer.get(x.data_ptr()) is None:
            return 0
        return r

    def context_kv(self, t, inner):
        kc = torch.zeros((self.B, self.TC, inner), dtype=f16, device=self.dev)
        vtc = torch.zeros((self.B, inner, self.TC), dtype=f16, device=self.dev)
        self.ctx_kv[t] = (kc, vtc)
        return kc, vtc

    def fused_tail(self, t, rows_t, o, tok, x, ch, inner, heads, dh, n):
        w, B, P, TC = self.w, self.B, self.P, self.TC
        kc, vtc = self.context_kv(t, inner)
        out = self.get((B, n, ch))
        td = ops.make_st_tail_desc(o, tok, x, out, kc, vtc, w[t + "tail.stream"], w[t + "tail.vec"], B, n, ch, heads,
                                   dh, 1, TC, tile_rows=rows_t)
        self.tails.append(td)
        td._bufs = (o, tok, x, out, kc, vtc)
        self.producer[out.data_ptr()] = td

        def run_tail(td=td):
            td.ctx_len = P.ctx_len
            ops.st_tail_run(td)
        self.emit(run_tail, "gemm", 2 * B * n * 16 * inner * inner + 4 * B * heads * n * self.ctx_flops * dh, 1,
                  f"st_tail M={B * n} C={inner} rows={rows_t} (to_out1..proj_out fused)")
        return out

    def stats_buf(self, rows, width):
        if (rows, width) not in self.ln_stats:
            self.ln_stats[(rows, width)] = torch.zeros((rows, width // 64, 2), dtype=f32, device=self.dev)
        return self.ln_stats[(rows, width)]

    def vt_buffer(self, n, inner):
        if n % 8 == 0:
            return self.get((self.B, inner, n))
        t_ = torch.zeros((self.B, inner, round_up(n, 8)), dtype=f16, device=self.dev)
        self.ragged_vt.append(t_)
        return t_

    def vt_release(self, t_):
        if not any(t_ is r for r in self.ragged_vt):
            self.release(t_)

    def first_self_attention(self):
        return "op" not in self.ck and "conv_in" in self.ck and len(self.hs) == 1

    def fused_transformer(self, t0, rows_h, x, ch, heads, dh, n):
        w, B = self.w, self.B
        inner = heads * dh
        tok = self.get((B, n, inner))
        qk = self.get((B, n, 2 * inner))
        vt = self.get((B, inner, n))
        hd = ops.make_st_head_desc(x, x, 1, w[t0 + "head.stream"], w[t0 + "head.vec"], tok, qk, vt, n, B, n, ch,
                                   tile_rows=rows_h)
        hd.colstats = 0
        self.heads_fused.append(hd)
        hd._bufs = (x, tok, qk, vt)
        self.gn_calls.append(dict(x1=x, x2=None, head=hd, meta=len(self.meta), film=False,
                                  prod=(self.producer.get(x.data_ptr()), None)))
        self.emit(lambda hd=hd: ops.st_head_run(hd), "gemm", 2 * B * n * 4 * inner * inner, 1,
                  f"st_head M={B * n} C={inner} rows={rows_h} (GroupNorm..q|k|v fused)")
        o = self.get((B, n, inner))
        self.attention(qk, vt, o, heads, dh, f"self B={B} h={heads} N={n} d={dh}", split_kv=True)
        if self.first_self_attention():
            self.ck.update(op=self.main[-1], live=(x, tok, o))
        out = self.fused_tail(t0, self.tail_rows(t0, n, heads, dh), o, tok, x, ch, inner, heads, dh, n)
        self.release(qk, vt, tok, o)
        return out

    def transformer(self, pre, x, ch, heads, dh, h, wd):
        net, w, B, P, TC = self.net, self.w, self.B, self.P, self.TC
        dense, emit, selfctx = self.dense, self.emit, self.selfctx
        n = h * wd
        inner = heads * dh
        scale = dh ** -0.5
        t0 = pre + "transformer_blocks.0."
        rows_h = self.head_rows(t0, x, n, heads, dh)
        if rows_h:
            return self.fused_transformer(t0, rows_h, x, ch, heads, dh, n)
        a = self.get((B, n, ch))
        self.gn(x, None, w[pre + "norm.g"], w[pre + "norm.b"], 1e-6, False, a)
        st = self.stats_buf(B * n, inner) if (t0 + "attn2.q.s") in w else None
        fold1 = st is not None and (t0 + "attn1.qkv.s") in w

        def consumer(name):
            return dict(bias=w[name + ".cb"], ln_stats=st, ln_s=w[name + ".s"], ln_eps=1e-5)

        def layernorm(src, t, norm, ln):
            emit(lambda: ops.layernorm(src, w[t + norm + ".g"], w[t + norm + ".b"], 1e-5, out=ln), "layernorm")
        tok = dense(a, B, n, ch, inner, w[pre + "proj_in.w"], bias=w[pre + "proj_in.b"], stats_out=st if fold1 else None)
        pf = ops.get_option("unet_gn_proj_fuse")
        if (self.fuse_head and pf and n >= pf and n % 64 == 0 and ch % 64 == 0 and ch <= 2560
                and self.producer.get(x.data_ptr()) is not None):
            self.gn_calls[-1]["proj"] = dict(desc=self.descs[-1], meta=len(self.meta) - 1)
        self.release(a)
        for k in range(net.transformer_depth):
            t = pre + f"transformer_blocks.{k}."
            last = k == net.transformer_depth - 1
            ln = self.get((B, n, inner))
            if not fold1:
                layernorm(tok, t, "norm1", ln)
            vt = self.vt_buffer(n, inner)
            nv = vt.shape[2]
            if (t + "attn1.qkv.w") in w:
                qk = self.get((B, n, 2 * inner))
                self.gemm(a=tok if fold1 else ln, w=w[t + "attn1.qkv.w"], N=3 * inner, B=B, H=n, W=1, c1=inner, out=qk,
                          out_ld=2 * inner, out2=vt, out2_ld=nv, n_split=2 * inner,
                          **(consumer(t + "attn1.qkv") if fold1 else {}))
            else:
                qk = dense(ln, B, n, inner, 2 * inner, w[t + "attn1.qk.w"])
                dense(ln, B, n, inner, inner, w[t + "attn1.v.w"], out=vt, out_ld=nv, out_mode=ops.OUT_TRANSPOSED)
            o = ln
            self.attention(qk, vt, o, heads, dh, f"self B={B} h={heads} N={n} d={dh}", split_kv=True)
            first = self.first_self_attention()
            rows_t = self.tail_rows(t, n, heads, dh)
            if first:
                self.ck.update(op=self.main[-1], live=(x, tok, o))
            if rows_t:
                out = self.fused_tail(t, rows_t, o, tok, x, ch, inner, heads, dh, n)
                self.release(qk); self.vt_release(vt); self.release(tok, ln)
                return out
            tok2 = dense(o, B, n, inner, inner, w[t + "attn1.o.w"], bias=w[t + "attn1.o.b"], residual=tok, stats_out=st)
            if first:
                self.ck.update(op2=self.main[-1], live2=(x, tok2) + (() if st is None else (st,)))
            self.release(qk); self.vt_release(vt); self.release(tok)
            xfuse = (ops.get_option("unet_xattn_fuse") and not selfctx and dh == 64 and TC <= 1024 and TC % 8 == 0
                     and n % 64 == 0)
            xkw = {}
            if xfuse:
                kc, vtc = self.context_kv(t, inner)
                xkw = dict(tile_n=64, splitk=1, tile_m=0 if n % 128 == 0 else 64, xattn_k=kc, xattn_vt=vtc, xattn_len=TC,
                           xattn_cap=TC, xattn_scale=scale, out=o, out_ld=inner)
            if st is None:
                layernorm(tok2, t, "norm2", ln)
                q2 = dense(ln, B, n, inner, inner, w[t + "attn2.q.w"], **xkw)
            else:
                q2 = dense(tok2, B, n, inner, inner, w[t + "attn2.q.w"], **consumer(t + "attn2.q"), **xkw)
                if selfctx:
                    layernorm(tok2, t, "norm2", ln)
            if xfuse:
                self.xattn_descs.append(self.descs[-1])
                self.meta[-1]["flops"] += 4 * B * heads * n * self.ctx_flops * dh
                self.meta[-1]["info"] += f" +cross-attention h={heads} d={dh}"
                q2 = None
            if selfctx:
                k2 = dense(ln, B, n, inner, inner, w[t + "attn2.k.w"])
                v2t = self.vt_buffer(n, inner)
                nv2 = v2t.shape[2]
                dense(ln, B, n, inner, inner, w[t + "attn2.v.w"], out=v2t, out_ld=nv2, out_mode=ops.OUT_TRANSPOSED)
                self.attn_ws_need = max(self.attn_ws_need, ops.attention_ws_bytes(B, heads, dh, n, n))
                emit(lambda q2=q2, k2=k2, v2t=v2t, o=o, nv2=nv2: ops.attention(
                    q2.data_ptr(), k2.data_ptr(), v2t.data_ptr(), o.data_ptr(), B, heads, dh, n, n, scale,
                    n * inner, inner, n * inner, inner, inner * nv2, nv2, n * inner, inner, ws=self.attn_ws),
                    "attention", 4 * B * heads * n * n * dh, 1, f"attn2-self B={B} h={heads} N={n} d={dh}")
                self.release(k2); self.vt_release(v2t)
            elif not xfuse:
                kc, vtc = self.context_kv(t, inner)
                emit(lambda q2=q2, kc=kc, vtc=vtc, o=o: ops.attention(
                    q2.data_ptr(), kc.data_ptr(), vtc.data_ptr(), o.data_ptr(), B, heads, dh, n, P.ctx_len, scale,
                    n * inner, inner, TC * inner, inner, inner * TC, TC, n * inner, inner),
                    "attention", 4 * B * heads * n * self.ctx_flops * dh, 1, f"cross B={B} h={heads} N={n} d={dh}")
            tok3 = dense(o, B, n, inner, inner, w[t + "attn2.o.w"], bias=w[t + "attn2.o.b"], residual=tok2, stats_out=st)
            if q2 is not None:
                self.release(q2)
            self.release(tok2)
            if st is None:
                layernorm(tok3, t, "norm3", ln)
                g = dense(ln, B, n, inner, 8 * inner, w[t + "ff1.w"], bias=w[t + "ff1.b"], epilogue=ops.EPI_GEGLU)
            else:
                g = dense(tok3, B, n, inner, 8 * inner, w[t + "ff1.w"], epilogue=ops.EPI_GEGLU, **consumer(t + "ff1"))
            self.geglu_tile160(self.descs[-1], t, inner)
            tok = dense(g, B, n, 4 * inner, inner, w[t + "ff2.w"], bias=w[t + "ff2.b"], residual=tok3,
                        stats_out=st if (fold1 and not last) else None)
            self.release(g, tok3, ln)
        out = dense(tok, B, n, inner, ch, w[pre + "proj_out.w"], bias=w[pre + "proj_out.b"], residual=x)
        self.release(tok)
        return out

    def before_wiring(self):
        self.stream_small_convs()
        self.fuse_splitk_into_groupnorm()

    def stream_small_convs(self):
        max_m = ops.get_option("unet_conv_stream")
        if not max_m:
            return
        frag_w = self.net._frag_w
        for d in self.descs:
            M = d.B * d.H * d.W
            if not (d.ksize == 3 and d.stride == 1 and not d.upsample and d.c2 == 0 and d.c1 % 64 == 0 and d.N % 64 == 0
                    and M <= max_m and d.out_mode == ops.OUT_ROWMAJOR and not d.skip_w and not d.gn_gamma):
                continue
            q = ops.gemm_query(d)
            w4 = ops.get_option("unet_conv_stream_w4")
            if w4 and q[3] == 1 and d.N % 128 == 0 and d.c1 // 64 >= 5 and not d.colstats_out and not d.defer_reduce:
                keep = (d.tile_m, d.tile_n, d.splitk)
                d.tile_m, d.tile_n, d.splitk = 128, 128, min(d.c1 // 64, w4)
                q = ops.gemm_query(d)
                if not (q[0] == 128 and q[1] == 128 and q[3] == 1 and q[2] > 4 and not q[6]):
                    d.tile_m, d.tile_n, d.splitk = keep
                    q = ops.gemm_query(d)
            if not (q[0] == 128 and q[1] in (64, 128) and q[3] == 1):
                continue
            if q[1] == 128 and not (q[2] > 1 and not q[6]):
                continue
            wkey = d._w_tensor.data_ptr()
            if wkey not in frag_w:
                frag_w[wkey] = ops.pack_frag_weight(ops.unpack_gemm_weight(d._w_tensor, d.N, 9 * d.c1)).reshape(-1)
            d.w, d.w_frag = frag_w[wkey].data_ptr(), 1

    def fuse_splitk_into_groupnorm(self):
        fuse_hw = ops.get_option("unet_gn_splitk_fuse")
        if not fuse_hw:
            return
        for c in self.gn_calls:
            if c.get("head") is not None or c.get("conv") is not None or c.get("proj") is not None:
                continue
            _, HW, C1 = c["x1"].shape
            if HW > fuse_hw:
                continue
            cpg = C1 // 32
            L = cpg // math.gcd(cpg, 8)
            d = c["prod"][0]
            if (c["x2"] is None and not c["film"] and L <= 64 and HW * L * 16 <= (64 << 10) and isinstance(d, ops.GemmDesc)
                    and d.N == C1
                    and d.out_ld == C1 and self.op_index.get(ctypes.addressof(d)) == c["meta"] - 1
                    and ops.gemm_query(d)[2] > 1 and ops.groupnorm_from_splitk_ok(d)):
                d.defer_reduce = 1
                c["fs"] = d
                self.meta[c["meta"] - 1]["launches"] = 1

    def after_wiring(self):
        if any(not hd.colstats for hd in self.heads_fused) or any(not dd.gn_colstats for dd in self.gn_convs):
            raise _HeadNotWired()
        if ops.get_option("unet_tune_first_use"):
            tws = ops.new_gemm_workspace(256 << 20, self.dev)
            self.patch_workspace(tws)
            self.P.tuned_shapes = ops.tune_untuned(self.descs)
            torch.cuda.synchronize()
            del tws
            ops.release_tune_scratch()
            self.patch_workspace(self.gemm_ws)
```

### minddiffusion_amd/ops.py

```python
import ctypes
import math
import os

import numpy as np
import torch

from . import _lib
from ._lib import GemmDesc, EPI_NONE, EPI_GEGLU, EPI_GELU, EPI_QUICKGELU, OUT_ROWMAJOR, OUT_TRANSPOSED
from ._lib import EPI_PRELU, OUT_D2S2

f16 = torch.float16
f32 = torch.float32


_OPTIONS = {"unet_st_tail": int(os.environ.get("MDX_UNET_ST_TAIL", "-1")),
            "unet_st_head": int(os.environ.get("MDX_UNET_ST_HEAD", "-1")),
            "unet_conv_stream": int(os.environ.get("MDX_UNET_CONV_STREAM", "128")),
            "gn_colstats_fold": int(os.environ.get("MDX_GN_COLSTATS_FOLD", "0")),
            "unet_gn_splitk_fuse": int(os.environ.get("MDX_UNET_GN_SPLITK_FUSE", "256")),
            "unet_conv_stream_w4": int(os.environ.get("MDX_UNET_CONV_STREAM_W4", "0")),
            "unet_skip_fuse": int(os.environ.get("MDX_UNET_SKIP_FUSE", "1")),
            "unet_gn_conv_fuse": int(os.environ.get("MDX_UNET_GN_CONV_FUSE", "0")),
            "unet_tune_first_use": int(os.environ.get("MDX_UNET_TUNE_FIRST_USE", "0")),
            "unet_subpixel_upsample": int(os.environ.get("MDX_UNET_SUBPIXEL_UPSAMPLE", "1")),
            "unet_gn_proj_fuse": int(os.environ.get("MDX_UNET_GN_PROJ_FUSE", "0")),
            "unet_xattn_fuse": int(os.environ.get("MDX_UNET_XATTN_FUSE", "1")),
            "unet_cfg_dup": int(os.environ.get("MDX_UNET_CFG_DUP", "4")),
            "unet_cfg_dup_check": int(os.environ.get("MDX_UNET_CFG_DUP_CHECK", "0")),
            "glide_qkv_merge": int(os.environ.get("MDX_GLIDE_QKV_MERGE", "1")),
            "glide_gn_qkv_fuse": int(os.environ.get("MDX_GLIDE_GN_QKV_FUSE", "0"))}


def set_option(name, value):
    if name in _OPTIONS:
        _OPTIONS[name] = int(value)
        return
    _lib.check(_lib.load().mdx_set_option(name.encode(), int(value)), "mdx_set_option")


def get_option(name):
    if name in _OPTIONS:
        return _OPTIONS[name]
    out = ctypes.c_int(0)
    _lib.check(_lib.load().mdx_get_option(name.encode(), ctypes.byref(out)), "mdx_get_option")
    return int(out.value)


def capture_graph(ops_list):
    import gc
    g = torch.cuda.CUDAGraph()
    gc.collect()
    was_enabled = gc.isenabled()
    gc.disable()
    try:
        with torch.cuda.graph(g):
            for op in ops_list:
                op()
    finally:
        if was_enabled:
            gc.enable()
    return g


def _stream():
    return ctypes.c_void_p(torch.cuda.current_stream().cuda_stream)


def _ptr(t):
    return None if t is None else ctypes.c_void_p(t.data_ptr())


def _chk(t, dtype, name):
    if t is None:
        return
    if not t.is_cuda:
        raise _lib.MdxError(f"{name}: tensor must live on the GPU (no CPU fallback)")
    if t.dtype != dtype:
        raise _lib.MdxError(f"{name}: expected {dtype}, got {t.dtype}")
    if not t.is_contiguous():
        raise _lib.MdxError(f"{name}: tensor must be contiguous")


def nchw_to_nhwc(x, cpad, out=None):
    _chk(x, f32, "x")
    B, C, H, W = x.shape
    if out is None:
        out = torch.empty((B, H * W, cpad), dtype=f16, device=x.device)
    _lib.check(_lib.load().mdx_nchw_to_nhwc_f16(_ptr(x), _ptr(out), B, C, H, W, cpad, _stream()), "mdx_nchw_to_nhwc_f16")
    return out


def nhwc_to_nchw(x, C, H, W, out=None):
    _chk(x, f16, "x")
    B, HW, Cs = x.shape
    assert HW == H * W
    if out is None:
        out = torch.empty((B, C, H, W), dtype=f32, device=x.device)
    _lib.check(_lib.load().mdx_nhwc_to_nchw_f32(_ptr(x), _ptr(out), B, C, H, W, Cs, _stream()), "mdx_nhwc_to_nchw_f32")
    return out


def groupnorm_ws_floats(B, HW, C, groups=32):
    return int(_lib.load().mdx_groupnorm_ws_floats(B, HW, C, groups))


def groupnorm(x1, x2, gamma, beta, eps, silu, ws=None, out=None, groups=32):
    _chk(x1, f16, "x1"); _chk(x2, f16, "x2"); _chk(gamma, f32, "gamma"); _chk(beta, f32, "beta")
    B, HW, C1 = x1.shape
    C2 = 0 if x2 is None else x2.shape[2]
    C = C1 + C2
    if ws is None:
        ws = torch.empty(groupnorm_ws_floats(B, HW, C, groups), dtype=f32, device=x1.device)
    if out is None:
        out = torch.empty((B, HW, C), dtype=f16, device=x1.device)
    _lib.check(_lib.load().mdx_groupnorm_f16(_ptr(x1), C1, _ptr(x2), C2, _ptr(gamma), _ptr(beta), _ptr(out), B, HW,
                                             groups, float(eps), int(bool(silu)), _ptr(ws), _stream()),
               "mdx_groupnorm_f16")
    return out


GN_FORMS = ("two_launch", "fused", "fused_one_pass", "fused_256", "colstats")


def groupnorm_query(C1, C2, B, HW, groups=32, colstats_nrb=0):
    out = (ctypes.c_int * 6)()
    _lib.check(_lib.load().mdx_groupnorm_query(int(C1), int(C2), int(B), int(HW), int(groups), int(colstats_nrb), out),
               "mdx_groupnorm_query")
    return dict(form=GN_FORMS[out[0]], cw=out[1], ncb=out[2], nblk=out[3], pix=out[4], threads=out[5])


class FoldedColStats:

    def __init__(self, raw, nrb, batch):
        f = (nrb + 63) // 64
        self.raw, self.nrb, self.batch = raw, nrb, batch
        self.nrb2 = (nrb + f - 1) // f
        self.folded = torch.zeros((batch * self.nrb2, raw.shape[1], 2), dtype=f32, device=raw.device)

    def data_ptr(self):
        return self.raw.data_ptr()

    def fold(self):
        _lib.check(_lib.load().mdx_colstats_fold_f32(_ptr(self.raw), self.nrb, _ptr(self.folded), self.nrb2, self.batch,
                                                     self.raw.shape[1], _stream()), "mdx_colstats_fold_f32")
        return self.folded, self.nrb2


def groupnorm_colstats(x1, cs1, nrb1, x2, cs2, nrb2, gamma, beta, eps, silu, out=None, groups=32, scale=None, shift=None,
                       mod_ld=0):
    if isinstance(cs1, FoldedColStats):
        cs1, nrb1 = cs1.fold()
    if isinstance(cs2, FoldedColStats):
        cs2, nrb2 = cs2.fold()
    B, HW, C1 = x1.shape
    C2 = 0 if x2 is None else x2.shape[2]
    if out is None:
        out = torch.empty((B, HW, C1 + C2), dtype=f16, device=x1.device)
    _lib.check(_lib.load().mdx_groupnorm_colstats_f16(_ptr(x1), C1, _ptr(cs1), int(nrb1), _ptr(x2), C2, _ptr(cs2), int(nrb2),
                                                      _ptr(gamma), _ptr(beta), _ptr(scale), _ptr(shift), int(mod_ld),
                                                      _ptr(out), B, HW, groups, float(eps), int(bool(silu)), _stream()),
               "mdx_groupnorm_colstats_f16")
    return out


def groupnorm_from_splitk_ok(desc, groups=32):
    return bool(_lib.load().mdx_groupnorm_from_splitk_ok(ctypes.byref(desc), groups))


def groupnorm_from_splitk(desc, gamma, beta, eps, silu, out, groups=32):
    _lib.check(_lib.load().mdx_groupnorm_from_splitk_f16(ctypes.byref(desc), _ptr(gamma), _ptr(beta), _ptr(out), groups,
                                                         float(eps), int(bool(silu)), _stream()),
               "mdx_groupnorm_from_splitk_f16")
    return out


def groupnorm_scaleshift(x1, x2, gamma, beta, scale, shift, mod_ld, eps, silu, ws=None, out=None, groups=32):
    _chk(x1, f16, "x1"); _chk(x2, f16, "x2")
    B, HW, C1 = x1.shape
    C2 = 0 if x2 is None else x2.shape[2]
    C = C1 + C2
    if ws is None:
        ws = torch.empty(groupnorm_ws_floats(B, HW, C, groups), dtype=f32, device=x1.device)
    if out is None:
        out = torch.empty((B, HW, C), dtype=f16, device=x1.device)
    _lib.check(_lib.load().mdx_groupnorm_scaleshift_f16(
        _ptr(x1), C1, _ptr(x2), C2, _ptr(gamma), _ptr(beta), _ptr(scale), _ptr(shift), int(mod_ld), _ptr(out), B, HW,
        groups, float(eps), int(bool(silu)), _ptr(ws), _stream()), "mdx_groupnorm_scaleshift_f16")
    return out


def avgpool2x2(x, B, H, W, C, out=None):
    if out is None:
        out = torch.empty((B, (H // 2) * (W // 2), C), dtype=f16, device=x.device)
    _lib.check(_lib.load().mdx_avgpool2x2_f16(_ptr(x), _ptr(out), B, H, W, C, _stream()), "mdx_avgpool2x2_f16")
    return out


def upsample_nearest2x(x, B, H, W, C, out=None):
    if out is None:
        out = torch.empty((B, 4 * H * W, C), dtype=f16, device=x.device)
    _lib.check(_lib.load().mdx_upsample_nearest2x_f16(_ptr(x), _ptr(out), B, H, W, C, _stream()),
               "mdx_upsample_nearest2x_f16")
    return out


def glide_text_embed(tokens, mask, tok_emb, pos, pad, out=None):
    B, T = tokens.shape
    width = pos.shape[1]
    if out is None:
        out = torch.empty((B, T, width), dtype=f16, device=tokens.device)
    _lib.check(_lib.load().mdx_glide_text_embed_f16(_ptr(tokens), _ptr(mask), _ptr(tok_emb), _ptr(pos), _ptr(pad),
                                                    _ptr(out), B, T, width, tok_emb.shape[0], _stream()),
               "mdx_glide_text_embed_f16")
    return out


def glide_superres_input(x, low, out=None):
    B, _, S, _ = x.shape
    if out is None:
        out = torch.empty((B, S * S, 8), dtype=f16, device=x.device)
    _lib.check(_lib.load().mdx_glide_superres_input_f16(_ptr(x), _ptr(low), _ptr(out), B, S, low.shape[2], _stream()),
               "mdx_glide_superres_input_f16")
    return out


def glide_step(x, out_c, out_u, ld, scale, coef8, mode, noise_scale, noise, x_next, pred_x0):
    B, _, H, W = x.shape
    c8 = (ctypes.c_float * 8)(*[float(v) for v in coef8])
    _lib.check(_lib.load().mdx_glide_step_f32(_ptr(x), _ptr(out_c), _ptr(out_u), int(ld), float(scale),
                                              ctypes.cast(c8, ctypes.c_void_p), int(mode), float(noise_scale),
                                              _ptr(noise), _ptr(x_next), _ptr(pred_x0), B, H, W, _stream()),
               "mdx_glide_step_f32")


def glide_kv_slots(entries, device):
    import numpy as np
    rows = []
    for src, dst, seb, dbb, sp, dp, r, rb in entries:
        for v in (src.data_ptr(), dst.data_ptr(), seb, dbb, sp, dp, rb):
            if v % 16:
                raise _lib.MdxError("glide_kv_slots: pointers and byte counts must be multiples of 16")
        rows.append([src.data_ptr(), dst.data_ptr(), seb, dbb, sp, dp, (int(r) & 0xffffffff) | (int(rb) << 32)])
    return torch.from_numpy(np.asarray(rows, dtype=np.int64)).to(device), len(rows)


def glide_kv_select(slots, nslots, entry0, entry_per_b, b0, nb, blocks_per_copy=8):
    _lib.check(_lib.load().mdx_glide_kv_select_f16(_ptr(slots), int(nslots), int(entry0), int(entry_per_b), int(b0), int(nb),
                                                   int(blocks_per_copy), _stream()), "mdx_glide_kv_select_f16")


def layernorm(x, gamma, beta, eps, out=None):
    _chk(x, f16, "x"); _chk(gamma, f32, "gamma"); _chk(beta, f32, "beta")
    C = x.shape[-1]
    rows = x.numel() // C
    if out is None:
        out = torch.empty_like(x)
    _lib.check(_lib.load().mdx_layernorm_f16(_ptr(x), _ptr(gamma), _ptr(beta), _ptr(out), rows, C, float(eps), _stream()),
               "mdx_layernorm_f16")
    return out


def pack_gemm_weight(w2d):
    N, K = w2d.shape
    dev = w2d.device
    Np, Kp = (N + 63) // 64 * 64, (K + 63) // 64 * 64
    wp = torch.zeros((Np, Kp), dtype=f16, device=dev)
    wp[:N, :K] = w2d
    t = wp.view(Np // 64, 64, Kp // 64, 8, 8).permute(0, 2, 1, 3, 4)
    r = torch.arange(64, device=dev)
    src = torch.arange(8, device=dev)[None, :] ^ ((r >> 1) & 7)[:, None]
    idx = src[None, None, :, :, None].expand(Np // 64, Kp // 64, 64, 8, 8)
    return torch.gather(t, 3, idx).contiguous().view(-1)


def conv_weight_k_order(w4d, cin_pad=None, cout_pad=None):
    w4d = w4d.to(torch.float32)
    co, ci, kh, kw = w4d.shape
    cip = cin_pad or ci
    cop = cout_pad or co
    if cip % 64 == 0:
        assert cip == ci
        p = torch.zeros((cop, ci // 64, kh * kw, 64), dtype=torch.float32, device=w4d.device)
        p[:co] = w4d.reshape(co, ci // 64, 64, kh * kw).permute(0, 1, 3, 2)
        return p.reshape(cop, kh * kw * ci)
    p = torch.zeros((cop, kh * kw, cip), dtype=torch.float32, device=w4d.device)
    p[:co, :, :ci] = w4d.permute(0, 2, 3, 1).reshape(co, kh * kw, ci)
    return p.reshape(cop, kh * kw * cip)


def pack_conv_weight(w4d, cin_pad=None, cout_pad=None):
    return pack_gemm_weight(conv_weight_k_order(w4d, cin_pad, cout_pad))


def subpixel_conv_weight(w4d):
    w = w4d.to(torch.float32)
    rows = {0: (w[:, :, 0], w[:, :, 1] + w[:, :, 2]), 1: (w[:, :, 0] + w[:, :, 1], w[:, :, 2])}
    out = []
    for dy in (0, 1):
        for dx in (0, 1):
            taps = []
            for a in (0, 1):
                r = rows[dy][a]
                cols = (r[:, :, 0], r[:, :, 1] + r[:, :, 2]) if dx == 0 else (r[:, :, 0] + r[:, :, 1], r[:, :, 2])
                taps.append(torch.stack(cols, -1))
            out.append(torch.stack(taps, 2))
    return torch.cat(out, 0)


def pack_subpixel_conv_weight(w4d):
    assert w4d.shape[0] % 64 == 0 and w4d.shape[1] % 64 == 0
    return pack_conv_weight(subpixel_conv_weight(w4d))


def pack_conv_weight_frag(w4d):
    co, ci = w4d.shape[0], w4d.shape[1]
    assert co % 64 == 0 and ci % 64 == 0
    return pack_frag_weight(conv_weight_k_order(w4d).to(f16)).reshape(-1)


def unpack_gemm_weight(packed, N, K):
    Np, Kp = (N + 63) // 64 * 64, (K + 63) // 64 * 64
    t = packed.view(Np // 64, Kp // 64, 64, 8, 8)
    r = torch.arange(64, device=packed.device)
    src = torch.arange(8, device=packed.device)[None, :] ^ ((r >> 1) & 7)[:, None]
    inv = torch.argsort(src, 1)
    idx = inv[None, None, :, :, None].expand(Np // 64, Kp // 64, 64, 8, 8)
    return torch.gather(t, 3, idx).permute(0, 2, 1, 3, 4).reshape(Np, Kp)[:N, :K].contiguous()


def geglu_interleave(a, g, unit=64):
    half = a.shape[0]
    assert g.shape == a.shape and half % unit == 0
    nt = half // unit
    return torch.stack([a.reshape(nt, unit, *a.shape[1:]), g.reshape(nt, unit, *a.shape[1:])], 1).reshape(2 * half, *a.shape[1:]).contiguous()


def geglu_deinterleave(t, unit=64):
    half = t.shape[0] // 2
    assert t.shape[0] % (2 * unit) == 0
    x = t.reshape(half // unit, 2, unit, *t.shape[1:])
    return x[:, 0].reshape(half, *t.shape[1:]).contiguous(), x[:, 1].reshape(half, *t.shape[1:]).contiguous()


def geglu_repack(t, unit_from, unit_to):
    return geglu_interleave(*geglu_deinterleave(t, unit_from), unit_to)


def make_gemm_desc(a, w, N, B, H, W, c1, out, out_ld, a2=None, c2=0, bias=None, rowbias=None, rowbias_ld=0,
                   residual=None, residual_ld=0, ksize=1, stride=1, upsample=0, epilogue=EPI_NONE,
                   out_mode=OUT_ROWMAJOR, splitk=0, workspace=None, out_bs=0, out2=None, out2_ld=0, n_split=0, asym_pad=0,
                   stats_out=None, ln_stats=None, ln_s=None, ln_eps=1e-5, tile_m=0, tile_n=0, colstats_out=None, stages=0,
                   w_frag=0, skip_a=None, skip_a2=None, skip_c1=0, skip_c2=0, skip_w=None, gn_colstats=None, gn_nrb=0,
                   gn_gamma=None, gn_beta=None, gn_eps=1e-5, gn_silu=1, w_sub=None, xattn_k=None, xattn_vt=None, xattn_len=0,
                   xattn_cap=0, xattn_scale=0.0, act_slope=None, geglu_unit=0):
    d = GemmDesc()
    d.a = a.data_ptr()
    d.a2 = 0 if a2 is None else a2.data_ptr()
    d.c1, d.c2 = int(c1), int(c2)
    d.w = w.data_ptr()
    d.bias = 0 if bias is None else bias.data_ptr()
    d.rowbias = 0 if rowbias is None else rowbias.data_ptr()
    d.rowbias_ld = int(rowbias_ld)
    d.residual = 0 if residual is None else residual.data_ptr()
    d.residual_ld = int(residual_ld)
    d.out = out.data_ptr()
    d.out_ld = int(out_ld)
    d.B, d.H, d.W, d.N = int(B), int(H), int(W), int(N)
    d.ksize, d.stride, d.upsample = int(ksize), int(stride), int(upsample)
    d.epilogue, d.out_mode, d.splitk = int(epilogue), int(out_mode), int(splitk)
    d.workspace = 0 if workspace is None else workspace.data_ptr()
    d.workspace_bytes = 0 if workspace is None else workspace.numel() * workspace.element_size()
    d.out_bs = int(out_bs)
    d.out2 = 0 if out2 is None else out2.data_ptr()
    d.out2_ld, d.n_split, d.asym_pad = int(out2_ld), int(n_split), int(asym_pad)
    d.stats_out = 0 if stats_out is None else stats_out.data_ptr()
    d.ln_stats = 0 if ln_stats is None else ln_stats.data_ptr()
    d.ln_s = 0 if ln_s is None else ln_s.data_ptr()
    d.ln_nt = 0 if ln_stats is None else (int(c1) + int(c2)) // 64
    d.ln_eps = float(ln_eps)
    d.tile_m, d.tile_n, d.stages, d.w_frag = int(tile_m), int(tile_n), int(stages), int(w_frag)
    d.gn_colstats = 0 if gn_colstats is None else gn_colstats.data_ptr()
    d.gn_gamma = 0 if gn_gamma is None else gn_gamma.data_ptr()
    d.gn_beta = 0 if gn_beta is None else gn_beta.data_ptr()
    d.gn_nrb, d.gn_silu, d.gn_eps = int(gn_nrb), int(gn_silu), float(gn_eps)
    d.skip_a = 0 if skip_a is None else skip_a.data_ptr()
    d.skip_a2 = 0 if skip_a2 is None else skip_a2.data_ptr()
    d.skip_c1, d.skip_c2 = int(skip_c1), int(skip_c2)
    d.skip_w = 0 if skip_w is None else skip_w.data_ptr()
    d.colstats_out = 0 if colstats_out is None else colstats_out.data_ptr()
    d.colstats_cap = 0 if colstats_out is None else int(colstats_out.shape[0])
    d.w_sub = 0 if w_sub is None else w_sub.data_ptr()
    if xattn_k is not None:
        d.xattn_k, d.xattn_vt = xattn_k.data_ptr(), xattn_vt.data_ptr()
        d.xattn_len, d.xattn_cap, d.xattn_scale = int(xattn_len), int(xattn_cap), float(xattn_scale)
    if act_slope is not None:
        d.act_slope, d.act_slope_n = act_slope.data_ptr(), int(act_slope.numel())
    d.geglu_unit = int(geglu_unit)
    d._tensors = tuple(t for t in (a, a2, w, bias, rowbias, residual, out, workspace, out2, stats_out, ln_stats, ln_s,
                                   colstats_out, skip_a, skip_a2, skip_w, gn_colstats, gn_gamma, gn_beta, w_sub, xattn_k,
                                   xattn_vt, act_slope) if t is not None)
    return d


def fold_layernorm(wt, gamma, beta, bias=None):
    w32 = wt.to(torch.float64)
    wg = (w32 * gamma.to(torch.float64)[None, :]).to(f16)
    s = wg.to(torch.float64).sum(1).to(f32).contiguous()
    cb = w32 @ beta.to(torch.float64)
    if bias is not None:
        cb = cb + bias.to(torch.float64)
    return wg.contiguous(), s, cb.to(f32).contiguous()


def gemm_workspace_bytes(desc):
    return int(_lib.load().mdx_gemm_workspace_bytes(ctypes.byref(desc)))


_WS_HEAD = 16384


def new_gemm_workspace(nbytes, device):
    import weakref
    base = torch.zeros((_WS_HEAD + max(int(nbytes), 16)) // 4 + 1, dtype=f32, device=device)
    ws = base[_WS_HEAD // 4:]
    lib = _lib.load()
    _lib.check(lib.mdx_gemm_bind_counters(ctypes.c_void_p(ws.data_ptr()), ctypes.c_void_p(base.data_ptr())),
               "mdx_gemm_bind_counters")
    weakref.finalize(ws, lib.mdx_gemm_release_workspace, ctypes.c_void_p(ws.data_ptr()))
    return ws


def gemm_check(desc):
    return _lib.load().mdx_gemm_check(ctypes.byref(desc)) == 0


def gemm_query(desc):
    out = (ctypes.c_int * 7)()
    _lib.check(_lib.load().mdx_gemm_query(ctypes.byref(desc), out), "mdx_gemm_query")
    return tuple(int(v) for v in out)


tune_cache = {}
_tune_flush = {}


def gemm_shape_key(d):
    var = ((1 if d.c2 > 0 else 0) | (d.epilogue << 1) | (8 if d.n_split else 0) | (16 if d.ln_stats else 0)
           | (32 if d.stats_out else 0) | (64 if d.out_mode == 1 else 0) | (128 if d.colstats_out else 0)
           | (256 if d.residual else 0) | (512 if d.rowbias else 0) | (1024 if d.skip_w else 0) | (2048 if d.gn_gamma else 0)
           | (4096 if d.w_sub else 0))
    return (d.B * d.H * d.W, d.N, d.ksize * d.ksize * (d.c1 + d.c2), d.ksize, d.stride, d.upsample, var, d.B, d.H, d.W)


def gemm_tune(desc, reps=5, cold=True):
    flush, nbytes = None, 0
    if cold:
        dev = torch.cuda.current_device()
        if dev not in _tune_flush:
            _tune_flush[dev] = torch.empty(512 << 20, dtype=torch.uint8, device=f"cuda:{dev}")
        flush, nbytes = ctypes.c_void_p(_tune_flush[dev].data_ptr()), _tune_flush[dev].numel()
    best, us = (ctypes.c_int * 4)(), (ctypes.c_float * 2)()
    _lib.check(_lib.load().mdx_gemm_tune(ctypes.byref(desc), _stream(), flush, nbytes, int(reps), best, us), "mdx_gemm_tune")
    return tuple(int(v) for v in best) + (float(us[0]), float(us[1]))


def tune_untuned(descs, reps=5):
    measured = 0
    for d in descs:
        if (d.colstats_out or d.defer_reduce or d.w_frag or d.skip_w or d.gn_gamma or d.tile_m or d.tile_n or d.splitk
                or d.stages or d.geglu_unit):
            continue
        key = gemm_shape_key(d)
        if key not in tune_cache:
            if gemm_query(d)[4]:
                continue
            tune_cache[key] = gemm_tune(d, reps)
            measured += 1
        tm, tn, sk, stg = tune_cache[key][:4]
        old = (d.tile_m, d.tile_n, d.splitk, d.stages)
        d.tile_m, d.tile_n, d.splitk, d.stages = tm, tn, sk, stg
        if _lib.load().mdx_gemm_check(ctypes.byref(d)) != 0:
            d.tile_m, d.tile_n, d.splitk, d.stages = old
    return measured


def release_tune_scratch():
    _tune_flush.clear()


TUNE_CACHE_VERSION = 2


def save_tune_cache(path):
    import json
    with open(path, "w") as f:
        json.dump({"version": TUNE_CACHE_VERSION, "key_fields": 10,
                   "entries": [[list(k), list(v)] for k, v in sorted(tune_cache.items())]}, f)


def load_tune_cache(path):
    import json
    import warnings
    with open(path) as f:
        data = json.load(f)
    if not isinstance(data, dict) or data.get("version") != TUNE_CACHE_VERSION:
        warnings.warn(f"load_tune_cache: {path} was written under another key layout (version "
                      f"{data.get('version') if isinstance(data, dict) else 'none'}, this build: {TUNE_CACHE_VERSION}); ignored")
        return 0
    n = 0
    for k, v in data["entries"]:
        if len(k) != 10:
            continue
        tune_cache[tuple(k)] = tuple(v)
        n += 1
    return n


def gemm_run(desc):
    _lib.check(_lib.load().mdx_gemm_f16(ctypes.byref(desc), _stream()), "mdx_gemm_f16")


def gemm(a, w, N, B, H, W, c1, out=None, **kw):
    _chk(a, f16, "a"); _chk(w, f16, "w")
    ksize, stride, upsample = kw.get("ksize", 1), kw.get("stride", 1), kw.get("upsample", 0)
    Hs, Ws = (2 * H, 2 * W) if upsample else (H, W)
    pad = 1 if ksize == 3 else 0
    Ho = (Hs + 2 * pad - ksize) // stride + 1
    Wo = (Ws + 2 * pad - ksize) // stride + 1
    M = B * Ho * Wo
    epi = kw.get("epilogue", EPI_NONE)
    out_mode = kw.get("out_mode", OUT_ROWMAJOR)
    if out is None:
        if out_mode == OUT_TRANSPOSED:
            ld = kw.pop("out_ld", Ho * Wo)
            out = torch.zeros((B, N, ld), dtype=f16, device=a.device)
        elif out_mode == OUT_D2S2:
            ld = kw.pop("out_ld", N // 4)
            out = torch.empty((B, 2 * Ho, 2 * Wo, ld), dtype=f16, device=a.device)
        else:
            cols = N // 2 if epi == EPI_GEGLU else N
            ld = kw.pop("out_ld", cols)
            out = torch.empty((M, ld), dtype=f16, device=a.device)
    else:
        ld = kw.pop("out_ld")
    d = make_gemm_desc(a, w, N, B, H, W, c1, out, ld, **kw)
    if not d.workspace:
        need = gemm_workspace_bytes(d)
        if need:
            ws = new_gemm_workspace(need, a.device)
            d.workspace = ws.data_ptr()
            d.workspace_bytes = need
    gemm_run(d)
    return out


def attention(q_ptr, k_ptr, vt_ptr, o_ptr, B, heads, D, Nq, Nk, scale, q_bs, q_ld, k_bs, k_ld, vt_bs, vt_ld, o_bs, o_ld,
              causal=False, ws=None, kv_splits=0):
    lib = _lib.load()
    if ws is not None and not causal:
        _lib.check(lib.mdx_attention_splitkv_f16(
            ctypes.c_void_p(q_ptr), q_bs, q_ld, ctypes.c_void_p(k_ptr), k_bs, k_ld, ctypes.c_void_p(vt_ptr), vt_bs, vt_ld,
            ctypes.c_void_p(o_ptr), o_bs, o_ld, B, heads, D, Nq, Nk, float(scale), int(kv_splits), ctypes.c_void_p(ws.data_ptr()),
            ws.numel() * ws.element_size(), _stream()), "mdx_attention_splitkv_f16")
        return
    fn = lib.mdx_attention_causal_f16 if causal else lib.mdx_attention_f16
    _lib.check(fn(ctypes.c_void_p(q_ptr), q_bs, q_ld, ctypes.c_void_p(k_ptr), k_bs, k_ld, ctypes.c_void_p(vt_ptr), vt_bs,
                  vt_ld, ctypes.c_void_p(o_ptr), o_bs, o_ld, B, heads, D, Nq, Nk, float(scale), _stream()),
               "mdx_attention_causal_f16" if causal else "mdx_attention_f16")


def attention_ws_bytes(B, heads, D, Nq, Nk):
    return int(_lib.load().mdx_attention_ws_bytes(B, heads, D, Nq, Nk))


def attention_workspace(nbytes, device):
    return torch.zeros(max(int(nbytes), 256), dtype=torch.uint8, device=device)


def timestep_embedding(t, dim, max_period=10000.0, out=None):
    _chk(t, f32, "t")
    M = t.shape[0]
    if out is None:
        out = torch.empty((M, dim), dtype=f32, device=t.device)
    _lib.check(_lib.load().mdx_timestep_embedding_f32(_ptr(t), _ptr(out), M, dim, float(max_period), _stream()),
               "mdx_timestep_embedding_f32")
    return out


def dense_small(x, w, b, act_in=False, act_out=False, out=None):
    _chk(x, f32, "x"); _chk(w, f16, "w"); _chk(b, f32, "b")
    M, K = x.shape
    N = w.shape[0]
    if out is None:
        out = torch.empty((M, N), dtype=f32, device=x.device)
    _lib.check(_lib.load().mdx_dense_small_f32(_ptr(x), x.stride(0), _ptr(w), _ptr(b), _ptr(out), out.stride(0), M, N, K,
                                               int(act_in), int(act_out), _stream()), "mdx_dense_small_f32")
    return out


def sampler_step(x, eps_u, eps_c, eps_ld, cfg_scale, olds, coef, sqrt_at, sqrt_one_minus_at, sqrt_a_prev, dir_coef,
                 sigma, noise, e_t_out, x_prev, pred_x0):
    B, C, H, W = x.shape
    c4 = (ctypes.c_float * 4)(*[float(v) for v in coef])
    o = list(olds) + [None] * (3 - len(olds))
    _lib.check(_lib.load().mdx_sampler_step_f32(
        _ptr(x), _ptr(eps_u), _ptr(eps_c), int(eps_ld), float(cfg_scale), _ptr(o[0]), _ptr(o[1]), _ptr(o[2]),
        ctypes.cast(c4, ctypes.c_void_p), float(sqrt_at), float(sqrt_one_minus_at), float(sqrt_a_prev), float(dir_coef),
        float(sigma), _ptr(noise), _ptr(e_t_out), _ptr(x_prev), _ptr(pred_x0), B, C, H, W, _stream()),
        "mdx_sampler_step_f32")


PRED_EPS, PRED_V = 0, 1


def sampler_step_pred(x, x_model, out_u, out_c, out_ld, cfg_scale, pred_type, sqrt_at_model, sqrt_one_minus_at_model,
                      olds, coef, sqrt_at, sqrt_one_minus_at, sqrt_a_prev, dir_coef, sigma, noise, e_t_out, x_prev,
                      pred_x0):
    B, C, H, W = x.shape
    c4 = (ctypes.c_float * 4)(*[float(v) for v in coef])
    o = list(olds) + [None] * (3 - len(olds))
    _lib.check(_lib.load().mdx_sampler_step_pred_f32(
        _ptr(x), _ptr(x_model), _ptr(out_u), _ptr(out_c), int(out_ld), float(cfg_scale), int(pred_type),
        float(sqrt_at_model), float(sqrt_one_minus_at_model), _ptr(o[0]), _ptr(o[1]), _ptr(o[2]),
        ctypes.cast(c4, ctypes.c_void_p), float(sqrt_at), float(sqrt_one_minus_at), float(sqrt_a_prev), float(dir_coef),
        float(sigma), _ptr(noise), _ptr(e_t_out), _ptr(x_prev), _ptr(pred_x0), B, C, H, W, _stream()),
        "mdx_sampler_step_pred_f32")


def sampler_step_rescale(x, x_model, out_u, out_c, out_ld, cfg_scale, pred_type, sqrt_at_model, sqrt_one_minus_at_model,
                         olds, coef, sqrt_at, sqrt_one_minus_at, sqrt_a_prev, dir_coef, sigma, noise, e_t_out, x_prev,
                         pred_x0, guidance_rescale, factor_out=None):
    B, C, H, W = x.shape
    c4 = (ctypes.c_float * 4)(*[float(v) for v in coef])
    o = list(olds) + [None] * (3 - len(olds))
    if factor_out is not None:
        _chk(factor_out, f32, "factor_out")
        if factor_out.numel() < B:
            raise _lib.MdxError(f"factor_out: needs {B} elements, has {factor_out.numel()}")
    _lib.check(_lib.load().mdx_sampler_step_rescale_f32(
        _ptr(x), _ptr(x_model), _ptr(out_u), _ptr(out_c), int(out_ld), float(cfg_scale), int(pred_type),
        float(sqrt_at_model), float(sqrt_one_minus_at_model), _ptr(o[0]), _ptr(o[1]), _ptr(o[2]),
        ctypes.cast(c4, ctypes.c_void_p), float(sqrt_at), float(sqrt_one_minus_at), float(sqrt_a_prev), float(dir_coef),
        float(sigma), _ptr(noise), _ptr(e_t_out), _ptr(x_prev), _ptr(pred_x0), float(guidance_rescale), _ptr(factor_out),
        B, C, H, W, _stream()), "mdx_sampler_step_rescale_f32")


def probe_mfma(a, b):
    c = torch.empty((64, 16), dtype=f32, device=a.device)
# ... 387 lines not shown
```

Measured before the change: 5.203 latents/s.

## Fold ff2 into proj_out via precomposed weights in a segmented dense GEMM

For the last transformer block, the ff2 linear and the proj_out linear are merged algebraically. The composed weight W_p·W_f2 is concatenated with W_p so that a single GEMM over [geglu output, tok3] produces the projected output plus residual, which removes one GEMM launch and the intermediate activation round trip. A new segmented dense kernel variant handles the two-source A operand, and tuned entries are added for the new shapes. The cost is a larger K dimension: proj_out's FLOPs over the 4×inner input go up because ch×4inner replaces inner×4inner work plus ch×inner. Folding two fp16 matrices into one may also change precision slightly.

```diff
diff --git a/minddiffusion_amd/csrc/dense.hip b/minddiffusion_amd/csrc/dense.hip
--- a/minddiffusion_amd/csrc/dense.hip
+++ b/minddiffusion_amd/csrc/dense.hip
@@ -268,324 +268,30 @@
     }
 }
 
-template <int BM, int BN, int NS, int PF, bool XA = false>
-__global__ __launch_bounds__(256, 2) void dense_kernel(const GemmParams p) {
-    mdx_kernarg_touch<sizeof(GemmParams)>();
-    constexpr int NW = 4;
-    constexpr bool W41 = BN % 64 != 0;
-    static_assert(!W41 || (BM == 128 && BN % 32 == 0 && !XA && PF <= 1), "4 x 1 wave layout: 128-row tiles, prefetch level 0 / 1");
-    constexpr int WROWS = W41 ? BM / 4 : BM / 2;
-    constexpr int TM = WROWS / 32;
-    constexpr int TN = W41 ? BN / 32 : BN / 64;
-    constexpr int ROWB = 128;
-    constexpr int KS = 4;
-    constexpr int A_BYTES = BM * ROWB;
-    constexpr int B_BYTES = BN * ROWB;
-    constexpr int STAGE = A_BYTES + B_BYTES;
-    constexpr int AJ = BM / 8 / NW;
-    constexpr int BJ = BN / 8 / NW;
-    constexpr int LPT = AJ + BJ;
-    extern __shared__ __attribute__((aligned(16))) char smem[];
-
-    const int tid = threadIdx.x;
-    const int lane = tid & 63;
-    const int wave = __builtin_amdgcn_readfirstlane(tid >> 6);
-    const int wm = W41 ? wave : wave >> 1, wn = W41 ? 0 : wave & 1;
-    const int hi = lane >> 5;
-    const int l31 = lane & 31;
-
-    const int ntiles = p.tiles_m * p.tiles_n;
-    const int tile_id = p.spread ? (int)blockIdx.x : (int)((blockIdx.x & 7) * p.tiles_per_xcd + (blockIdx.x >> 3));
-    if (tile_id >= ntiles) return;
-    trace_mark(p, 0);
-    int tile_m, tile_n;
-    if (p.n_fastest) {
-        tile_m = p.inv_tiles_n ? (int)__umulhi((unsigned)tile_id, p.inv_tiles_n) : tile_id;
-        tile_n = tile_id - tile_m * p.tiles_n;
-    } else {
-        tile_n = p.inv_tiles_m ? (int)__umulhi((unsigned)tile_id, p.inv_tiles_m) : tile_id;
-        tile_m = tile_id - tile_n * p.tiles_m;
-    }
-    const int m0 = tile_m * BM, n0 = tile_n * BN;
-    const int split = (int)blockIdx.y;
-    const int kt_begin = split * p.ktiles_per_split;
-    const int kt_end = min(p.ktiles, kt_begin + p.ktiles_per_split);
-    const int nt = kt_end - kt_begin;
-
-    const __amdgpu_buffer_rsrc_t rs_a = make_rsrc(p.a, p.a_bytes);
-    const __amdgpu_buffer_rsrc_t rs_w = make_rsrc(p.w, p.w_bytes);
-
-    const int lrow = lane >> 3, lchk = lane & 7;
-    const unsigned row_bytes = (unsigned)p.c1 * 2u;
-    unsigned a_voff[AJ], b_off[BJ];
-#pragma unroll
-    for (int j = 0; j < AJ; ++j) {
-        const int row = (wave * AJ + j) * 8 + lrow;
-        const int m = m0 + row;
-        a_voff[j] = m < p.M ? (unsigned)m * row_bytes + (unsigned)((lchk ^ ((row >> 1) & 7)) * 16) : MDX_OOB;
-    }
-#pragma unroll
-    for (int j = 0; j < BJ; ++j) {
-        const int row = (wave * BJ + j) * 8 + lrow;
-        if constexpr (W41) {
-            const int grow = n0 + row;
-            b_off[j] = (unsigned)(grow >> 6) * (unsigned)p.kt64 * 8192u + (unsigned)(((grow & 63) * 8 + lchk) * 16);
-        } else {
-            const int panel = (n0 >> 6) + (row >> 6);
-            b_off[j] = (unsigned)panel * (unsigned)p.kt64 * 8192u + (unsigned)(((row & 63) * 8 + lchk) * 16);
-        }
-    }
-    auto stage_tile = [&](int kt, int buf) {
-        char* sbase = smem + buf * STAGE;
-#pragma unroll
-        for (int j = 0; j < AJ; ++j) dma16s(rs_a, sbase + (wave * AJ + j) * 1024, a_voff[j], (unsigned)kt * 128u);
-#pragma unroll
-        for (int j = 0; j < BJ; ++j) dma16s(rs_w, sbase + A_BYTES + (wave * BJ + j) * 1024, b_off[j], (unsigned)kt * 8192u);
-    };
-#pragma unroll
-    for (int i = 0; i < NS - 1; ++i)
-        if (i < nt) stage_tile(kt_begin + i, i);
-    __builtin_amdgcn_sched_barrier(0);
-    trace_mark(p, 1);
-
-    constexpr int CPR = BN / 8, RPP = 256 / CPR, PASSES = BM / RPP;
-    constexpr int NX = (PF >= 2 && !W41) ? (PASSES < 4 ? PASSES : 4) : 0;
-    constexpr int LNR = PF >= 3 ? LNR_MAX : 0;
-    constexpr int NT = PF == 1 || PF == 2 ? 2 : 0;
-    constexpr int NB = BN == 128 ? 4 : 2;
-    constexpr int E = NB + NX + LNR + (PF >= 2 ? 1 : 0) + NT;
-    const bool geglu = p.epilogue == MDX_EPI_GEGLU;
-    const __amdgpu_buffer_rsrc_t rs_bias = make_rsrc(p.bias, p.bias ? (unsigned)p.N * 4u : 0u);
-    const __amdgpu_buffer_rsrc_t rs_res = make_rsrc(p.residual, (p.residual && !geglu) ? p.res_bytes : 0u);
-    const bool ln_regs = PF >= 3 && p.ln_stats != nullptr && p.ln_nt <= LNR;
-    const bool lns_regs = PF >= 2 && p.ln_stats != nullptr;
-    const __amdgpu_buffer_rsrc_t rs_ln = make_rsrc(p.ln_stats, p.ln_stats ? (unsigned)p.M * (unsigned)p.ln_nt * 8u : 0u);
-    const __amdgpu_buffer_rsrc_t rs_lns = make_rsrc(p.ln_s, p.ln_stats ? (unsigned)p.N * 4u : 0u);
-    u32x4 braw[4] = {};
-    if constexpr (W41) {
-        const unsigned off = (tid < BN && n0 + tid < p.N) ? (unsigned)(n0 + tid) * 4u : MDX_OOB;
-        braw[0][0] = __builtin_amdgcn_raw_buffer_load_b32(rs_bias, off, 0, 0);
-        braw[1][0] = __builtin_amdgcn_raw_buffer_load_b32(rs_lns, off, 0, 0);
-    } else {
-        const int n = n0 + (geglu ? (tid & 7) : (tid % CPR)) * 8;
-        const unsigned off = n < p.N ? (unsigned)n * 4u : MDX_OOB;
-        braw[0] = __builtin_amdgcn_raw_buffer_load_b128(rs_bias, off, 0, 0);
-        braw[1] = __builtin_amdgcn_raw_buffer_load_b128(rs_bias, off, 16, 0);
-        if constexpr (NB == 4) {
-            const unsigned goff = geglu ? off : MDX_OOB;
-            braw[2] = __builtin_amdgcn_raw_buffer_load_b128(rs_bias, goff, 256, 0);
-            braw[3] = __builtin_amdgcn_raw_buffer_load_b128(rs_bias, goff, 272, 0);
-        }
-    }
-    u32x4 xraw[NX > 0 ? NX : 1];
-    if constexpr (NX > 0) {
-        const int n = n0 + (tid % CPR) * 8;
-#pragma unroll
-        for (int q = 0; q < NX; ++q) {
-            const int m = m0 + tid / CPR + q * RPP;
-            const unsigned off = (m < p.M && n < p.N) ? ((unsigned)m * (unsigned)p.residual_ld + (unsigned)n) * 2u : MDX_OOB;
-            xraw[q] = __builtin_amdgcn_raw_buffer_load_b128(rs_res, off, 0, 0);
-        }
-    }
-    u32x2 lnraw[LNR > 0 ? LNR : 1];
-    if constexpr (LNR > 0) {
-        const unsigned base = (tid < BM && m0 + tid < p.M) ? (unsigned)(m0 + tid) * (unsigned)p.ln_nt * 8u : MDX_OOB;
-#pragma unroll
-        for (int j = 0; j < LNR; ++j)
-            lnraw[j] = __builtin_amdgcn_raw_buffer_load_b64(rs_ln, (base != MDX_OOB && j < p.ln_nt) ? base : MDX_OOB, j * 8, 0);
-    }
-    unsigned lns_raw = 0u;
-    if constexpr (PF >= 2)
-        lns_raw = __builtin_amdgcn_raw_buffer_load_b32(rs_lns, (tid < BN && n0 + tid < p.N) ? (unsigned)(n0 + tid) * 4u : MDX_OOB, 0, 0);
-    unsigned touch[2] = {0u, 0u};
-    if constexpr (NT > 0) {
-        const int rows = min(BM, p.M - m0);
-        const unsigned bytes = (unsigned)rows * (unsigned)p.ln_nt * 8u;
-        const unsigned base = (unsigned)m0 * (unsigned)p.ln_nt * 8u;
-        touch[0] = __builtin_amdgcn_raw_buffer_load_b32(rs_ln, (unsigned)tid * 128u < bytes ? base + (unsigned)tid * 128u : MDX_OOB, 0, 0);
-        touch[1] = __builtin_amdgcn_raw_buffer_load_b32(rs_lns, (PF < 2 && tid < BN / 32 && n0 + tid * 32 < p.N) ? (unsigned)(n0 + tid * 32) * 4u : MDX_OOB, 0, 0);
-    }
-    __builtin_amdgcn_sched_barrier(0);
-
-    f32x16 acc[TM][TN];
-#pragma unroll
-    for (int i = 0; i < TM; ++i)
-#pragma unroll
-        for (int j = 0; j < TN; ++j)
-#pragma unroll
-            for (int r = 0; r < 16; ++r) acc[i][j][r] = 0.f;
-
-    const int swz = (l31 >> 1) & 7;
-    const int a_row_off = (wm * WROWS + l31) * ROWB;
-    const int b_row_off = A_BYTES + (wn * (BN / 2) + l31) * ROWB;
-
-    int rd = 0, wr = NS - 1;
-    for (int t = 0; t < nt; ++t) {
-        const int ahead = min(NS - 2, nt - 1 - t);
-        if (t == 0) {
-            if (NS >= 6 && ahead >= 4)
-                asm volatile("s_waitcnt vmcnt(%0)" ::"n"(4 * LPT + E) : "memory");
-            else if (NS >= 5 && ahead == 3)
-                asm volatile("s_waitcnt vmcnt(%0)" ::"n"(3 * LPT + E) : "memory");
-            else if (NS >= 4 && ahead == 2)
-                asm volatile("s_waitcnt vmcnt(%0)" ::"n"(2 * LPT + E) : "memory");
-            else if (NS >= 3 && ahead == 1)
-                asm volatile("s_waitcnt vmcnt(%0)" ::"n"(LPT + E) : "memory");
-            else
-                asm volatile("s_waitcnt vmcnt(%0)" ::"n"(E) : "memory");
-        } else if (NS >= 6 && ahead >= 4)
-            asm volatile("s_waitcnt vmcnt(%0)" ::"n"(4 * LPT) : "memory");
-        else if (NS >= 5 && ahead == 3)
-            asm volatile("s_waitcnt vmcnt(%0)" ::"n"(3 * LPT) : "memory");
-        else if (NS >= 4 && ahead == 2)
-            asm volatile("s_waitcnt vmcnt(%0)" ::"n"(2 * LPT) : "memory");
-        else if (NS >= 3 && ahead == 1)
-            asm volatile("s_waitcnt vmcnt(%0)" ::"n"(LPT) : "memory");
-        else
-            asm volatile("s_waitcnt vmcnt(0)" ::: "memory");
-        __builtin_amdgcn_s_barrier();
-        if (t == 0) trace_mark(p, 2);
-        const char* sb = smem + rd * STAGE;
-        constexpr bool ALLK = TM * TN <= 2;
-        constexpr int FD = ALLK ? KS : 2;
-        f16x8 af[FD][TM], bf[FD][TN];
-        auto rdfrag = [&](auto slot_c, const int ks) {
-            constexpr int slot = decltype(slot_c)::value;
-            const int coff = (((2 * ks + hi) ^ swz) << 4);
-#pragma unroll
-            for (int i = 0; i < TM; ++i) af[slot][i] = *reinterpret_cast<const f16x8*>(sb + a_row_off + i * 32 * ROWB + coff);
-#pragma unroll
-            for (int j = 0; j < TN; ++j) bf[slot][j] = *reinterpret_cast<const f16x8*>(sb + b_row_off + j * 32 * ROWB + coff);
-        };
-        auto mfmas = [&](auto slot_c) {
-            constexpr int slot = decltype(slot_c)::value;
-#pragma unroll
-            for (int i = 0; i < TM; ++i)
-#pragma unroll
-                for (int j = 0; j < TN; ++j)
-                    acc[i][j] = __builtin_amdgcn_mfma_f32_32x32x16_f16(bf[slot][j], af[slot][i], acc[i][j], 0, 0, 0);
-        };
-        using I0 = std::integral_constant<int, 0>;
-        using I1 = std::integral_constant<int, 1>;
-        if (t + NS - 1 < nt) stage_tile(kt_begin + t + NS - 1, wr);
-        __builtin_amdgcn_sched_barrier(0);
-        if constexpr (ALLK) {
-            using I2 = std::integral_constant<int, 2>;
-            using I3 = std::integral_constant<int, 3>;
-            rdfrag(I0{}, 0); rdfrag(I1{}, 1); rdfrag(I2{}, 2); rdfrag(I3{}, 3);
-            __builtin_amdgcn_sched_barrier(0);
-            mfmas(I0{}); mfmas(I1{}); mfmas(I2{}); mfmas(I3{});
-        } else {
-            rdfrag(I0{}, 0);
-            __builtin_amdgcn_sched_barrier(0);
-#pragma unroll
-            for (int ks = 0; ks < KS; ks += 2) {
-                rdfrag(I1{}, ks + 1);
-                __builtin_amdgcn_sched_barrier(0);
-                mfmas(I0{});
-                __builtin_amdgcn_sched_barrier(0);
-                if (ks + 2 < KS) {
-                    rdfrag(I0{}, ks + 2);
-                    __builtin_amdgcn_sched_barrier(0);
-                }
-                mfmas(I1{});
-                __builtin_amdgcn_sched_barrier(0);
-            }
-        }
-        rd = (rd + 1 == NS) ? 0 : rd + 1;
-        wr = (wr + 1 == NS) ? 0 : wr + 1;
-    }
-
-    __syncthreads();
-    trace_mark(p, 3);
-#pragma unroll
-    for (int q = 0; q < NB; ++q) asm volatile("" ::"v"(braw[q]));
-#pragma unroll
-    for (int q = 0; q < NX; ++q) asm volatile("" ::"v"(xraw[q]));
-#pragma unroll
-    for (int j = 0; j < LNR; ++j) asm volatile("" ::"v"(lnraw[j]));
-    if constexpr (PF >= 2) asm volatile("" ::"v"(lns_raw));
-#pragma unroll
-    for (int q = 0; q < NT; ++q) asm volatile("" ::"v"(touch[q]));
-    float bpre[16];
-#pragma unroll
-    for (int q = 0; q < 4; ++q) {
-        const f32x4 f = __builtin_bit_cast(f32x4, braw[q]);
-        bpre[4 * q] = f[0]; bpre[4 * q + 1] = f[1]; bpre[4 * q + 2] = f[2]; bpre[4 * q + 3] = f[3];
-    }
-    Row8Extras xpre[NX > 0 ? NX : 1];
-#pragma unroll
-    for (int q = 0; q < NX; ++q) xpre[q].res = __builtin_bit_cast(f16x8, xraw[q]);
-    float ln_pre[2];
-    {
-        float su = 0.f, sq = 0.f;
-#pragma unroll
-        for (int j = 0; j < LNR; ++j) {
-            const float2 v = __builtin_bit_cast(float2, lnraw[j]);
-            su += v.x;
-            sq += v.y;
-        }
-        const float inv = 1.0f / (float)p.K;
-        const float mean = su * inv;
-        float var = sq * inv - mean * mean;
-        var = var < 0.f ? 0.f : var;
-        ln_pre[0] = mean;
-        ln_pre[1] = rsqrtf(var + p.ln_eps);
-    }
-    const float lns_pre = __builtin_bit_cast(float, lns_raw);
-    if constexpr (XA) {
-        static_assert(BN == 64, "cross-attention epilogue: one 64-wide head per tile");
-        constexpr int XOFF = ((BM * 72 * 2 + 2 * BM * 4 + BN * 4 + 1023) / 1024) * 1024;
-        char* xs = smem + XOFF;
-        const int bsamp = m0 / p.HoWo, head = n0 >> 6;
-        const f16* kb = p.xa_k + (size_t)bsamp * p.xa_cap * p.N + head * 64;
-        const f16* vb = p.xa_vt + ((size_t)bsamp * p.N + head * 64) * p.xa_cap;
-        const __amdgpu_buffer_rsrc_t rs_k = make_rsrc(kb, (unsigned)(((size_t)(p.xa_len - 1) * p.N + 64) * 2));
-        const __amdgpu_buffer_rsrc_t rs_v = make_rsrc(vb, (unsigned)((size_t)64 * p.xa_cap * 2));
-        const int ntile = (p.xa_len + 63) >> 6;
-        auto stage_pair = [&](const int t0) {
-            const int t1 = t0 + 2 < ntile ? t0 + 2 : ntile;
-            for (int t = t0; t < t1; ++t) {
-                char* slot = xs + (t & 1) * 16384;
-#pragma unroll
-                for (int j = 0; j < 2; ++j) {
-                    const int inst = wave * 2 + j;
-                    const int krow = inst * 8 + (lane >> 3);
-                    const int kchunk = (lane & 7) ^ ((krow >> 1) & 7);
-                    const int key = t * 64 + krow;
-                    dma16(rs_k, slot + inst * 1024, key < p.xa_len ? (unsigned)(((size_t)key * p.N + kchunk * 8) * 2) : MDX_OOB);
-                    const int vrow = inst * 8 + (lane >> 3);
-                    const unsigned vchunk = (unsigned)((lane & 7) ^ ((vrow >> 1) & 7));
-                    const int kc = t * 64 + (int)vchunk * 8;
-                    dma16(rs_v, slot + 8192 + inst * 1024, kc < p.xa_cap ? (unsigned)(((size_t)vrow * p.xa_cap + kc) * 2) : MDX_OOB);
-                }
-            }
-        };
-        stage_pair(0);
-        gemm_epilogue<BM, BN, true, NW, LinearRows, NX, 3>(p, acc, smem, LinearRows{m0}, n0, split, bpre, tile_m, tile_id, ln_pre, &lns_pre, xpre,
-                                                           ln_regs, lns_regs);
-        asm volatile("s_waitcnt vmcnt(0)" ::: "memory");
-        __syncthreads();
-        xattn_tile_epilogue<BM>(p, smem, xs, m0, n0, stage_pair);
-    } else if constexpr (W41) {
-        epilogue_w41<BM, BN>(p, acc[0], smem, m0, n0, bpre[0], bpre[4]);
-    } else {
-        gemm_epilogue<BM, BN, true, NW, LinearRows, NX, LEAN_EPI ? 1 : 0>(p, acc, smem, LinearRows{m0}, n0, split, bpre, tile_m, tile_id, ln_pre,
-                                                                  &lns_pre, xpre, ln_regs, lns_regs);
-    }
-    trace_mark(p, 4);
-}
-
-template <int BM, int BN, int NS, int PF>
+#define MDX_DENSE_SEG 0
+#include "dense_body.inc"
+#undef MDX_DENSE_SEG
+#define MDX_DENSE_SEG 1
+#include "dense_body.inc"
+#undef MDX_DENSE_SEG
+
+template <int BM, int BN, int NS, int PF, bool SEG = false>
 void launch_dense_one(const GemmParams& p, dim3 grid, hipStream_t st) {
     constexpr size_t ring = (size_t)NS * (BM + BN) * 64 * 2;
     constexpr size_t epi = (size_t)(BM > BN ? BM : BN) * ((BM > BN ? BN : BM) + 8) * 2 + 4096;
     constexpr size_t lds = ring > epi ? ring : epi;
     static MdxPerDeviceOnce attr_once;
-    if (attr_once.first())
-        (void)hipFuncSetAttribute(reinterpret_cast<const void*>(&dense_kernel<BM, BN, NS, PF>),
-                                  hipFuncAttributeMaxDynamicSharedMemorySize, (int)lds);
-    hipLaunchKernelGGL((dense_kernel<BM, BN, NS, PF>), grid, dim3(256), lds, st, p);
+    if constexpr (SEG) {
+        if (attr_once.first())
+            (void)hipFuncSetAttribute(reinterpret_cast<const void*>(&dense_seg_kernel<BM, BN, NS, PF>),
+                                      hipFuncAttributeMaxDynamicSharedMemorySize, (int)lds);
+        hipLaunchKernelGGL((dense_seg_kernel<BM, BN, NS, PF>), grid, dim3(256), lds, st, p);
+    } else {
+        if (attr_once.first())
+            (void)hipFuncSetAttribute(reinterpret_cast<const void*>(&dense_kernel<BM, BN, NS, PF>),
+                                      hipFuncAttributeMaxDynamicSharedMemorySize, (int)lds);
+        hipLaunchKernelGGL((dense_kernel<BM, BN, NS, PF>), grid, dim3(256), lds, st, p);
+    }
 }
 
 template <int BM, int NS>
@@ -600,8 +306,12 @@
     hipLaunchKernelGGL((dense_kernel<BM, 64, NS, 1, true>), grid, dim3(256), lds, st, p);
 }
 
-template <int BM, int BN, int NS>
+template <int BM, int BN, int NS, bool SEG = false>
 void launch_dense_pf(const GemmParams& p, int pf, dim3 grid, hipStream_t st) {
+    if constexpr (SEG) {
+        if (pf >= 1) return launch_dense_one<BM, BN, NS, 1, true>(p, grid, st);
+        return launch_dense_one<BM, BN, NS, 0, true>(p, grid, st);
+    }
     if constexpr (BM * BN < 128 * 128) {
         if (pf >= 3) return launch_dense_one<BM, BN, NS, 3>(p, grid, st);
         if (pf == 2) return launch_dense_one<BM, BN, NS, 2>(p, grid, st);
@@ -610,14 +320,14 @@
     launch_dense_one<BM, BN, NS, 0>(p, grid, st);
 }
 
-template <int BM, int BN>
+template <int BM, int BN, bool SEG = false>
 bool launch_dense_ns(const GemmParams& p, int ns, int pf, dim3 grid, hipStream_t st) {
     switch (ns) {
-        case 2: launch_dense_pf<BM, BN, 2>(p, pf, grid, st); return true;
-        case 3: launch_dense_pf<BM, BN, 3>(p, pf, grid, st); return true;
-        case 4: if constexpr (BM == 64 || BN == 64) { launch_dense_pf<BM, BN, 4>(p, pf, grid, st); return true; } return false;
-        case 5: if constexpr (BM == 64) { launch_dense_pf<BM, BN, 5>(p, pf, grid, st); return true; } return false;
-        case 6: if constexpr (BM == 64) { launch_dense_pf<BM, BN, 6>(p, pf, grid, st); return true; } return false;
+        case 2: launch_dense_pf<BM, BN, 2, SEG>(p, pf, grid, st); return true;
+        case 3: launch_dense_pf<BM, BN, 3, SEG>(p, pf, grid, st); return true;
+        case 4: if constexpr (BM == 64 || BN == 64) { launch_dense_pf<BM, BN, 4, SEG>(p, pf, grid, st); return true; } return false;
+        case 5: if constexpr (BM == 64) { launch_dense_pf<BM, BN, 5, SEG>(p, pf, grid, st); return true; } return false;
+        case 6: if constexpr (BM == 64) { launch_dense_pf<BM, BN, 6, SEG>(p, pf, grid, st); return true; } return false;
         default: return false;
     }
 }
@@ -626,7 +336,11 @@
 
 bool mdx_dense_takes_desc(const GemmParams& p, int bn) {
     if (!mdx_opt(MDX_OPT_GEMM_LEAN_DENSE) || !p.dense_issue) return false;
-    if (!(p.ksize == 1 && p.stride == 1 && !p.upsample && p.c2 == 0 && p.cin % 64 == 0 && p.out_mode == MDX_OUT_ROWMAJOR)) return false;
+    if (!(p.ksize == 1 && p.stride == 1 && !p.upsample && p.cin % 64 == 0 && p.out_mode == MDX_OUT_ROWMAJOR)) return false;
+    if (p.c2 != 0) {
+        if (p.c1 % 64 != 0 || p.c2 % 64 != 0 || bn == 160) return false;
+        if (p.epilogue != MDX_EPI_NONE || p.n_split || p.ln_stats || p.xa_k) return false;
+    }
     if (p.gn_cs || p.rowbias || p.out_bs || p.skip_w || p.d2s_c) return false;
     if (p.epilogue != MDX_EPI_NONE && p.epilogue != MDX_EPI_GEGLU) return false;
     if (p.xa_k && bn != 64) return false;
@@ -660,6 +374,12 @@
         if (ok && bm == 64) { if (ns == 2) launch_dense_xa<64, 2>(p, g, st); else if (ns == 3) launch_dense_xa<64, 3>(p, g, st); else launch_dense_xa<64, 4>(p, g, st); }
         if (ok && bm == 128) { if (ns == 2) launch_dense_xa<128, 2>(p, g, st); else if (ns == 3) launch_dense_xa<128, 3>(p, g, st); else launch_dense_xa<128, 4>(p, g, st); }
     }
+    else if (p.c2 != 0) {
+        if (bm == 64 && bn == 64) ok = launch_dense_ns<64, 64, true>(p, ns, pf, g, st);
+        else if (bm == 64 && bn == 128) ok = launch_dense_ns<64, 128, true>(p, ns, pf, g, st);
+        else if (bm == 128 && bn == 64) ok = launch_dense_ns<128, 64, true>(p, ns, pf, g, st);
+        else if (bm == 128 && bn == 128) ok = launch_dense_ns<128, 128, true>(p, ns, pf, g, st);
+    }
     else if (bm == 64 && bn == 64) ok = launch_dense_ns<64, 64>(p, ns, pf, g, st);
     else if (bm == 64 && bn == 128) ok = launch_dense_ns<64, 128>(p, ns, pf, g, st);
     else if (bm == 128 && bn == 64) ok = launch_dense_ns<128, 64>(p, ns, pf, g, st);
diff --git a/minddiffusion_amd/csrc/dense_body.inc b/minddiffusion_amd/csrc/dense_body.inc
--- /dev/null
+++ b/minddiffusion_amd/csrc/dense_body.inc
@@ -0,0 +1,327 @@
+#if MDX_DENSE_SEG
+template <int BM, int BN, int NS, int PF>
+__global__ __launch_bounds__(256, 2) void dense_seg_kernel(const GemmParams p) {
+    constexpr bool XA = false, SEG = true;
+#else
+template <int BM, int BN, int NS, int PF, bool XA = false>
+__global__ __launch_bounds__(256, 2) void dense_kernel(const GemmParams p) {
+    constexpr bool SEG = false;
+#endif
+    mdx_kernarg_touch<sizeof(GemmParams)>();
+    constexpr int NW = 4;
+    constexpr bool W41 = BN % 64 != 0;
+    static_assert(!W41 || (BM == 128 && BN % 32 == 0 && !XA && PF <= 1), "4 x 1 wave layout: 128-row tiles, prefetch level 0 / 1");
+    static_assert(!SEG || (!W41 && !XA && PF <= 1), "K-segmented A: the 2 x 2 wave layouts, no cross-attention epilogue, prefetch level 0 / 1");
+    constexpr int WROWS = W41 ? BM / 4 : BM / 2;
+    constexpr int TM = WROWS / 32;
+    constexpr int TN = W41 ? BN / 32 : BN / 64;
+    constexpr int ROWB = 128;
+    constexpr int KS = 4;
+    constexpr int A_BYTES = BM * ROWB;
+    constexpr int B_BYTES = BN * ROWB;
+    constexpr int STAGE = A_BYTES + B_BYTES;
+    constexpr int AJ = BM / 8 / NW;
+    constexpr int BJ = BN / 8 / NW;
+    constexpr int LPT = AJ + BJ;
+    extern __shared__ __attribute__((aligned(16))) char smem[];
+
+    const int tid = threadIdx.x;
+    const int lane = tid & 63;
+    const int wave = __builtin_amdgcn_readfirstlane(tid >> 6);
+    const int wm = W41 ? wave : wave >> 1, wn = W41 ? 0 : wave & 1;
+    const int hi = lane >> 5;
+    const int l31 = lane & 31;
+
+    const int ntiles = p.tiles_m * p.tiles_n;
+    const int tile_id = p.spread ? (int)blockIdx.x : (int)((blockIdx.x & 7) * p.tiles_per_xcd + (blockIdx.x >> 3));
+    if (tile_id >= ntiles) return;
+    trace_mark(p, 0);
+    int tile_m, tile_n;
+    if (p.n_fastest) {
+        tile_m = p.inv_tiles_n ? (int)__umulhi((unsigned)tile_id, p.inv_tiles_n) : tile_id;
+        tile_n = tile_id - tile_m * p.tiles_n;
+    } else {
+        tile_n = p.inv_tiles_m ? (int)__umulhi((unsigned)tile_id, p.inv_tiles_m) : tile_id;
+        tile_m = tile_id - tile_n * p.tiles_m;
+    }
+    const int m0 = tile_m * BM, n0 = tile_n * BN;
+    const int split = (int)blockIdx.y;
+    const int kt_begin = split * p.ktiles_per_split;
+    const int kt_end = min(p.ktiles, kt_begin + p.ktiles_per_split);
+    const int nt = kt_end - kt_begin;
+
+    const __amdgpu_buffer_rsrc_t rs_a = make_rsrc(p.a, p.a_bytes);
+    const __amdgpu_buffer_rsrc_t rs_w = make_rsrc(p.w, p.w_bytes);
+    [[maybe_unused]] const __amdgpu_buffer_rsrc_t rs_a2 = make_rsrc(SEG ? p.a2 : p.a, SEG ? p.a2_bytes : p.a_bytes);
+    [[maybe_unused]] const int kt1 = p.c1 >> 6;
+
+    const int lrow = lane >> 3, lchk = lane & 7;
+    const unsigned row_bytes = (unsigned)p.c1 * 2u;
+    unsigned a_voff[AJ], b_off[BJ];
+    [[maybe_unused]] unsigned a_voff2[SEG ? AJ : 1];
+#pragma unroll
+    for (int j = 0; j < AJ; ++j) {
+        const int row = (wave * AJ + j) * 8 + lrow;
+        const int m = m0 + row;
+        a_voff[j] = m < p.M ? (unsigned)m * row_bytes + (unsigned)((lchk ^ ((row >> 1) & 7)) * 16) : MDX_OOB;
+        if constexpr (SEG)
+            a_voff2[j] = m < p.M ? (unsigned)m * ((unsigned)p.c2 * 2u) + (unsigned)((lchk ^ ((row >> 1) & 7)) * 16) : MDX_OOB;
+    }
+#pragma unroll
+    for (int j = 0; j < BJ; ++j) {
+        const int row = (wave * BJ + j) * 8 + lrow;
+        if constexpr (W41) {
+            const int grow = n0 + row;
+            b_off[j] = (unsigned)(grow >> 6) * (unsigned)p.kt64 * 8192u + (unsigned)(((grow & 63) * 8 + lchk) * 16);
+        } else {
+            const int panel = (n0 >> 6) + (row >> 6);
+            b_off[j] = (unsigned)panel * (unsigned)p.kt64 * 8192u + (unsigned)(((row & 63) * 8 + lchk) * 16);
+        }
+    }
+    auto stage_tile = [&](int kt, int buf) {
+        char* sbase = smem + buf * STAGE;
+        if (SEG && kt >= kt1) {
+            if constexpr (SEG) {
+#pragma unroll
+                for (int j = 0; j < AJ; ++j) dma16s(rs_a2, sbase + (wave * AJ + j) * 1024, a_voff2[j], (unsigned)(kt - kt1) * 128u);
+            }
+        } else {
+#pragma unroll
+            for (int j = 0; j < AJ; ++j) dma16s(rs_a, sbase + (wave * AJ + j) * 1024, a_voff[j], (unsigned)kt * 128u);
+        }
+#pragma unroll
+        for (int j = 0; j < BJ; ++j) dma16s(rs_w, sbase + A_BYTES + (wave * BJ + j) * 1024, b_off[j], (unsigned)kt * 8192u);
+    };
+#pragma unroll
+    for (int i = 0; i < NS - 1; ++i)
+        if (i < nt) stage_tile(kt_begin + i, i);
+    __builtin_amdgcn_sched_barrier(0);
+    trace_mark(p, 1);
+
+    constexpr int CPR = BN / 8, RPP = 256 / CPR, PASSES = BM / RPP;
+    constexpr int NX = (PF >= 2 && !W41) ? (PASSES < 4 ? PASSES : 4) : 0;
+    constexpr int LNR = PF >= 3 ? LNR_MAX : 0;
+    constexpr int NT = PF == 1 || PF == 2 ? 2 : 0;
+    constexpr int NB = BN == 128 ? 4 : 2;
+    constexpr int E = NB + NX + LNR + (PF >= 2 ? 1 : 0) + NT;
+    const bool geglu = p.epilogue == MDX_EPI_GEGLU;
+    const __amdgpu_buffer_rsrc_t rs_bias = make_rsrc(p.bias, p.bias ? (unsigned)p.N * 4u : 0u);
+    const __amdgpu_buffer_rsrc_t rs_res = make_rsrc(p.residual, (p.residual && !geglu) ? p.res_bytes : 0u);
+    const bool ln_regs = PF >= 3 && p.ln_stats != nullptr && p.ln_nt <= LNR;
+    const bool lns_regs = PF >= 2 && p.ln_stats != nullptr;
+    const __amdgpu_buffer_rsrc_t rs_ln = make_rsrc(p.ln_stats, p.ln_stats ? (unsigned)p.M * (unsigned)p.ln_nt * 8u : 0u);
+    const __amdgpu_buffer_rsrc_t rs_lns = make_rsrc(p.ln_s, p.ln_stats ? (unsigned)p.N * 4u : 0u);
+    u32x4 braw[4] = {};
+    if constexpr (W41) {
+        const unsigned off = (tid < BN && n0 + tid < p.N) ? (unsigned)(n0 + tid) * 4u : MDX_OOB;
+        braw[0][0] = __builtin_amdgcn_raw_buffer_load_b32(rs_bias, off, 0, 0);
+        braw[1][0] = __builtin_amdgcn_raw_buffer_load_b32(rs_lns, off, 0, 0);
+    } else {
+        const int n = n0 + (geglu ? (tid & 7) : (tid % CPR)) * 8;
+        const unsigned off = n < p.N ? (unsigned)n * 4u : MDX_OOB;
+        braw[0] = __builtin_amdgcn_raw_buffer_load_b128(rs_bias, off, 0, 0);
+        braw[1] = __builtin_amdgcn_raw_buffer_load_b128(rs_bias, off, 16, 0);
+        if constexpr (NB == 4) {
+            const unsigned goff = geglu ? off : MDX_OOB;
+            braw[2] = __builtin_amdgcn_raw_buffer_load_b128(rs_bias, goff, 256, 0);
+            braw[3] = __builtin_amdgcn_raw_buffer_load_b128(rs_bias, goff, 272, 0);
+        }
+    }
+    u32x4 xraw[NX > 0 ? NX : 1];
+    if constexpr (NX > 0) {
+        const int n = n0 + (tid % CPR) * 8;
+#pragma unroll
+        for (int q = 0; q < NX; ++q) {
+            const int m = m0 + tid / CPR + q * RPP;
+            const unsigned off = (m < p.M && n < p.N) ? ((unsigned)m * (unsigned)p.residual_ld + (unsigned)n) * 2u : MDX_OOB;
+            xraw[q] = __builtin_amdgcn_raw_buffer_load_b128(rs_res, off, 0, 0);
+        }
+    }
+    u32x2 lnraw[LNR > 0 ? LNR : 1];
+    if constexpr (LNR > 0) {
+        const unsigned base = (tid < BM && m0 + tid < p.M) ? (unsigned)(m0 + tid) * (unsigned)p.ln_nt * 8u : MDX_OOB;
+#pragma unroll
+        for (int j = 0; j < LNR; ++j)
+            lnraw[j] = __builtin_amdgcn_raw_buffer_load_b64(rs_ln, (base != MDX_OOB && j < p.ln_nt) ? base : MDX_OOB, j * 8, 0);
+    }
+    unsigned lns_raw = 0u;
+    if constexpr (PF >= 2)
+        lns_raw = __builtin_amdgcn_raw_buffer_load_b32(rs_lns, (tid < BN && n0 + tid < p.N) ? (unsigned)(n0 + tid) * 4u : MDX_OOB, 0, 0);
+    unsigned touch[2] = {0u, 0u};
+    if constexpr (NT > 0) {
+        const int rows = min(BM, p.M - m0);
+        const unsigned bytes = (unsigned)rows * (unsigned)p.ln_nt * 8u;
+        const unsigned base = (unsigned)m0 * (unsigned)p.ln_nt * 8u;
+        touch[0] = __builtin_amdgcn_raw_buffer_load_b32(rs_ln, (unsigned)tid * 128u < bytes ? base + (unsigned)tid * 128u : MDX_OOB, 0, 0);
+        touch[1] = __builtin_amdgcn_raw_buffer_load_b32(rs_lns, (PF < 2 && tid < BN / 32 && n0 + tid * 32 < p.N) ? (unsigned)(n0 + tid * 32) * 4u : MDX_OOB, 0, 0);
+    }
+    __builtin_amdgcn_sched_barrier(0);
+
+    f32x16 acc[TM][TN];
+#pragma unroll
+    for (int i = 0; i < TM; ++i)
+#pragma unroll
+        for (int j = 0; j < TN; ++j)
+#pragma unroll
+            for (int r = 0; r < 16; ++r) acc[i][j][r] = 0.f;
+
+    const int swz = (l31 >> 1) & 7;
+    const int a_row_off = (wm * WROWS + l31) * ROWB;
+    const int b_row_off = A_BYTES + (wn * (BN / 2) + l31) * ROWB;
+
+    int rd = 0, wr = NS - 1;
+    for (int t = 0; t < nt; ++t) {
+        const int ahead = min(NS - 2, nt - 1 - t);
+        if (t == 0) {
+            if (NS >= 6 && ahead >= 4)
+                asm volatile("s_waitcnt vmcnt(%0)" ::"n"(4 * LPT + E) : "memory");
+            else if (NS >= 5 && ahead == 3)
+                asm volatile("s_waitcnt vmcnt(%0)" ::"n"(3 * LPT + E) : "memory");
+            else if (NS >= 4 && ahead == 2)
+                asm volatile("s_waitcnt vmcnt(%0)" ::"n"(2 * LPT + E) : "memory");
+            else if (NS >= 3 && ahead == 1)
+                asm volatile("s_waitcnt vmcnt(%0)" ::"n"(LPT + E) : "memory");
+            else
+                asm volatile("s_waitcnt vmcnt(%0)" ::"n"(E) : "memory");
+        } else if (NS >= 6 && ahead >= 4)
+            asm volatile("s_waitcnt vmcnt(%0)" ::"n"(4 * LPT) : "memory");
+        else if (NS >= 5 && ahead == 3)
+            asm volatile("s_waitcnt vmcnt(%0)" ::"n"(3 * LPT) : "memory");
+        else if (NS >= 4 && ahead == 2)
+            asm volatile("s_waitcnt vmcnt(%0)" ::"n"(2 * LPT) : "memory");
+        else if (NS >= 3 && ahead == 1)
+            asm volatile("s_waitcnt vmcnt(%0)" ::"n"(LPT) : "memory");
+        else
+            asm volatile("s_waitcnt vmcnt(0)" ::: "memory");
+        __builtin_amdgcn_s_barrier();
+        if (t == 0) trace_mark(p, 2);
+        const char* sb = smem + rd * STAGE;
+        constexpr bool ALLK = TM * TN <= 2;
+        constexpr int FD = ALLK ? KS : 2;
+        f16x8 af[FD][TM], bf[FD][TN];
+        auto rdfrag = [&](auto slot_c, const int ks) {
+            constexpr int slot = decltype(slot_c)::value;
+            const int coff = (((2 * ks + hi) ^ swz) << 4);
+#pragma unroll
+            for (int i = 0; i < TM; ++i) af[slot][i] = *reinterpret_cast<const f16x8*>(sb + a_row_off + i * 32 * ROWB + coff);
+#pragma unroll
+            for (int j = 0; j < TN; ++j) bf[slot][j] = *reinterpret_cast<const f16x8*>(sb + b_row_off + j * 32 * ROWB + coff);
+        };
+        auto mfmas = [&](auto slot_c) {
+            constexpr int slot = decltype(slot_c)::value;
+#pragma unroll
+            for (int i = 0; i < TM; ++i)
+#pragma unroll
+                for (int j = 0; j < TN; ++j)
+                    acc[i][j] = __builtin_amdgcn_mfma_f32_32x32x16_f16(bf[slot][j], af[slot][i], acc[i][j], 0, 0, 0);
+        };
+        using I0 = std::integral_constant<int, 0>;
+        using I1 = std::integral_constant<int, 1>;
+        if (t + NS - 1 < nt) stage_tile(kt_begin + t + NS - 1, wr);
+        __builtin_amdgcn_sched_barrier(0);
+        if constexpr (ALLK) {
+            using I2 = std::integral_constant<int, 2>;
+            using I3 = std::integral_constant<int, 3>;
+            rdfrag(I0{}, 0); rdfrag(I1{}, 1); rdfrag(I2{}, 2); rdfrag(I3{}, 3);
+            __builtin_amdgcn_sched_barrier(0);
+            mfmas(I0{}); mfmas(I1{}); mfmas(I2{}); mfmas(I3{});
+        } else {
+            rdfrag(I0{}, 0);
+            __builtin_amdgcn_sched_barrier(0);
+#pragma unroll
+            for (int ks = 0; ks < KS; ks += 2) {
+                rdfrag(I1{}, ks + 1);
+                __builtin_amdgcn_sched_barrier(0);
+                mfmas(I0{});
+                __builtin_amdgcn_sched_barrier(0);
+                if (ks + 2 < KS) {
+                    rdfrag(I0{}, ks + 2);
+                    __builtin_amdgcn_sched_barrier(0);
+                }
+                mfmas(I1{});
+                __builtin_amdgcn_sched_barrier(0);
+            }
+        }
+        rd = (rd + 1 == NS) ? 0 : rd + 1;
+        wr = (wr + 1 == NS) ? 0 : wr + 1;
+    }
+
+    __syncthreads();
+    trace_mark(p, 3);
+#pragma unroll
+    for (int q = 0; q < NB; ++q) asm volatile("" ::"v"(braw[q]));
+#pragma unroll
+    for (int q = 0; q < NX; ++q) asm volatile("" ::"v"(xraw[q]));
+#pragma unroll
+    for (int j = 0; j < LNR; ++j) asm volatile("" ::"v"(lnraw[j]));
+    if constexpr (PF >= 2) asm volatile("" ::"v"(lns_raw));
+#pragma unroll
+    for (int q = 0; q < NT; ++q) asm volatile("" ::"v"(touch[q]));
+    float bpre[16];
+#pragma unroll
+    for (int q = 0; q < 4; ++q) {
+        const f32x4 f = __builtin_bit_cast(f32x4, braw[q]);
+        bpre[4 * q] = f[0]; bpre[4 * q + 1] = f[1]; bpre[4 * q + 2] = f[2]; bpre[4 * q + 3] = f[3];
+    }
+    Row8Extras xpre[NX > 0 ? NX : 1];
+#pragma unroll
+    for (int q = 0; q < NX; ++q) xpre[q].res = __builtin_bit_cast(f16x8, xraw[q]);
+    float ln_pre[2];
+    {
+        float su = 0.f, sq = 0.f;
+#pragma unroll
+        for (int j = 0; j < LNR; ++j) {
+            const float2 v = __builtin_bit_cast(float2, lnraw[j]);
+            su += v.x;
+            sq += v.y;
+        }
+        const float inv = 1.0f / (float)p.K;
+        const float mean = su * inv;
+        float var = sq * inv - mean * mean;
+        var = var < 0.f ? 0.f : var;
+        ln_pre[0] = mean;
+        ln_pre[1] = rsqrtf(var + p.ln_eps);
+    }
+    const float lns_pre = __builtin_bit_cast(float, lns_raw);
+    if constexpr (XA) {
+        static_assert(BN == 64, "cross-attention epilogue: one 64-wide head per tile");
+        constexpr int XOFF = ((BM * 72 * 2 + 2 * BM * 4 + BN * 4 + 1023) / 1024) * 1024;
+        char* xs = smem + XOFF;
+        const int bsamp = m0 / p.HoWo, head = n0 >> 6;
+        const f16* kb = p.xa_k + (size_t)bsamp * p.xa_cap * p.N + head * 64;
+        const f16* vb = p.xa_vt + ((size_t)bsamp * p.N + head * 64) * p.xa_cap;
+        const __amdgpu_buffer_rsrc_t rs_k = make_rsrc(kb, (unsigned)(((size_t)(p.xa_len - 1) * p.N + 64) * 2));
+        const __amdgpu_buffer_rsrc_t rs_v = make_rsrc(vb, (unsigned)((size_t)64 * p.xa_cap * 2));
+        const int ntile = (p.xa_len + 63) >> 6;
+        auto stage_pair = [&](const int t0) {
+            const int t1 = t0 + 2 < ntile ? t0 + 2 : ntile;
+            for (int t = t0; t < t1; ++t) {
+                char* slot = xs + (t & 1) * 16384;
+#pragma unroll
+                for (int j = 0; j < 2; ++j) {
+                    const int inst = wave * 2 + j;
+                    const int krow = inst * 8 + (lane >> 3);
+                    const int kchunk = (lane & 7) ^ ((krow >> 1) & 7);
+                    const int key = t * 64 + krow;
+                    dma16(rs_k, slot + inst * 1024, key < p.xa_len ? (unsigned)(((size_t)key * p.N + kchunk * 8) * 2) : MDX_OOB);
+                    const int vrow = inst * 8 + (lane >> 3);
+                    const unsigned vchunk = (unsigned)((lane & 7) ^ ((vrow >> 1) & 7));
+                    const int kc = t * 64 + (int)vchunk * 8;
+                    dma16(rs_v, slot + 8192 + inst * 1024, kc < p.xa_cap ? (unsigned)(((size_t)vrow * p.xa_cap + kc) * 2) : MDX_OOB);
+                }
+            }
+        };
+        stage_pair(0);
+        gemm_epilogue<BM, BN, true, NW, LinearRows, NX, 3>(p, acc, smem, LinearRows{m0}, n0, split, bpre, tile_m, tile_id, ln_pre, &lns_pre, xpre,
+                                                           ln_regs, lns_regs);
+        asm volatile("s_waitcnt vmcnt(0)" ::: "memory");
+        __syncthreads();
+        xattn_tile_epilogue<BM>(p, smem, xs, m0, n0, stage_pair);
+    } else if constexpr (W41) {
+        epilogue_w41<BM, BN>(p, acc[0], smem, m0, n0, bpre[0], bpre[4]);
+    } else {
+        gemm_epilogue<BM, BN, true, NW, LinearRows, NX, LEAN_EPI ? 1 : 0>(p, acc, smem, LinearRows{m0}, n0, split, bpre, tile_m, tile_id, ln_pre,
+                                                                  &lns_pre, xpre, ln_regs, lns_regs);
+    }
+    trace_mark(p, 4);
+}
diff --git a/minddiffusion_amd/csrc/gemm_tuned.inc b/minddiffusion_amd/csrc/gemm_tuned.inc
--- a/minddiffusion_amd/csrc/gemm_tuned.inc
+++ b/minddiffusion_amd/csrc/gemm_tuned.inc
@@ -382,3 +382,7 @@
     {8192, 320, 2880, 3, 128, 64, 1, 129, 4},
     {8192, 320, 2880, 3, 128, 64, 1, 385, 4},
     {8192, 320, 5760, 3, 128, 64, 1, 641, 4},
+    {2048, 640, 3200, 1, 128, 128, 3, 258, 3},
+    {2048, 640, 3200, 1, 128, 64, 2, 386, 3},
+    {512, 1280, 6400, 1, 128, 64, 3, 258, 4},
+    {128, 1280, 6400, 1, 64, 64, 6, 258, 4},
diff --git a/minddiffusion_amd/ldm/modules/diffusionmodules/openaimodel.py b/minddiffusion_amd/ldm/modules/diffusionmodules/openaimodel.py
--- a/minddiffusion_amd/ldm/modules/diffusionmodules/openaimodel.py
+++ b/minddiffusion_amd/ldm/modules/diffusionmodules/openaimodel.py
@@ -332,6 +332,7 @@
         w["out.cb"] = L.vec(conv + ".bias", pad=self.cout_pad)
         self._frag_w = {}
         self._geglu80 = {}
+        self._ff_proj = {}
         self._plans = {}
         self._ctx_key = None
         self._ctx_ref = None
@@ -856,6 +857,18 @@
             d.bias, d.ln_s = g80[t + "ff1.cb"].data_ptr(), g80[t + "ff1.s"].data_ptr()
         else:
             d.bias = g80[t + "ff1.b"].data_ptr()
+
+    def ff_proj_weights(self, pre, t, ch, inner, n):
+        w, fp = self.w, self.net._ff_proj
+        thr = ops.get_option("unet_ff_proj_fuse")
+        if not thr or inner < thr or inner % 64 or self.B * n < 128:
+            return None
+        if t not in fp:
+            w_p = ops.unpack_gemm_weight(w[pre + "proj_out.w"], ch, inner)
+            w_f2 = ops.unpack_gemm_weight(w[t + "ff2.w"], inner, 4 * inner)
+            comp, bc = ops.compose_ff_proj(w_p, w[pre + "proj_out.b"], w_f2, w[t + "ff2.b"])
+            fp[t] = (ops.pack_gemm_weight(comp), bc)
+        return fp[t]
 
     def tail_rows(self, t, n, heads, dh):
         TC = self.TC
@@ -1048,6 +1061,12 @@
             else:
                 g = dense(tok3, B, n, inner, 8 * inner, w[t + "ff1.w"], epilogue=ops.EPI_GEGLU, **consumer(t + "ff1"))
             self.geglu_tile160(self.descs[-1], t, inner)
+            fpw = self.ff_proj_weights(pre, t, ch, inner, n) if last else None
+            if fpw is not None:
+                out = dense(g, B, n, 5 * inner, ch, fpw[0], bias=fpw[1], src2=tok3, c2=inner, residual=x)
+                self.meta[-1]["info"] += " (ff2 + proj_out fused)"
+                self.release(g, tok3, ln)
+                return out
             tok = dense(g, B, n, 4 * inner, inner, w[t + "ff2.w"], bias=w[t + "ff2.b"], residual=tok3,
                         stats_out=st if (fold1 and not last) else None)
             self.release(g, tok3, ln)
@@ -1103,7 +1122,8 @@
             if (c["x2"] is None and not c["film"] and L <= 64 and HW * L * 16 <= (64 << 10) and isinstance(d, ops.GemmDesc)
                     and d.N == C1
                     and d.out_ld == C1 and self.op_index.get(ctypes.addressof(d)) == c["meta"] - 1
-                    and ops.gemm_query(d)[2] > 1 and ops.groupnorm_from_splitk_ok(d)):
+                    and ops.gemm_query(d)[2] > 1 and ops.groupnorm_from_splitk_ok(d)
+                    and not (d.c2 and ops.gemm_query(d)[6])):
                 d.defer_reduce = 1
                 c["fs"] = d
                 self.meta[c["meta"] - 1]["launches"] = 1
diff --git a/minddiffusion_amd/ops.py b/minddiffusion_amd/ops.py
--- a/minddiffusion_amd/ops.py
+++ b/minddiffusion_amd/ops.py
@@ -27,6 +27,7 @@
             "unet_xattn_fuse": int(os.environ.get("MDX_UNET_XATTN_FUSE", "1")),
             "unet_cfg_dup": int(os.environ.get("MDX_UNET_CFG_DUP", "4")),
             "unet_cfg_dup_check": int(os.environ.get("MDX_UNET_CFG_DUP_CHECK", "0")),
+            "unet_ff_proj_fuse": int(os.environ.get("MDX_UNET_FF_PROJ_FUSE", "640")),
             "glide_qkv_merge": int(os.environ.get("MDX_GLIDE_QKV_MERGE", "1")),
             "glide_gn_qkv_fuse": int(os.environ.get("MDX_GLIDE_GN_QKV_FUSE", "0"))}
 
@@ -344,6 +345,13 @@
 
 def geglu_repack(t, unit_from, unit_to):
     return geglu_interleave(*geglu_deinterleave(t, unit_from), unit_to)
+
+
+def compose_ff_proj(w_p, b_p, w_f2, b_f2):
+    wp64 = w_p.to(torch.float64)
+    wc = (wp64 @ w_f2.to(torch.float64)).to(f16)
+    bc = (b_p.to(torch.float64) + wp64 @ b_f2.to(torch.float64)).to(f32)
+    return torch.cat([wc, w_p.to(f16)], 1).contiguous(), bc.contiguous()
 
 
 def make_gemm_desc(a, w, N, B, H, W, c1, out, out_ld, a2=None, c2=0, bias=None, rowbias=None, rowbias_ld=0,
```

Result: faster. 5.292 latents/s (median of 6 runs) (+1.7%).
